# neggles/neurosis

Hardware: AMD Instinct MI355X
Metric: train images/sec (node) SDXL 1024^2 (higher is better)
Workload: dtype bf16

## Files before the change

### include/neurosis_hip.h

```cpp
#ifndef NEUROSIS_HIP_H
#define NEUROSIS_HIP_H

#ifdef __cplusplus
extern "C" {
#endif

const char* nk_last_error(void);
int nk_abi_version(void);

int nk_linear_fwd(const void* x, const void* w, const float* bias, const void* residual, void* y,
                  int M, int N, int K, long ldx, long ldw, long ldr, long ldy, float alpha, void* stream);
int nk_linear_dgrad(const void* dy, const void* w, const void* dx_add, void* dx, int M, int N, int K,
                    long lddy, long ldw, long ldadd, long lddx, void* stream);
long nk_linear_fwd_geglu_ok(int M, int I, int K);
int nk_linear_fwd_geglu(const void* x, const void* w, const float* bias, void* u, void* h, int M, int I, int K, long ldx, long ldw, long ldu,
                        long ldh, void* stream);
int nk_linear_dgrad_geglu(const void* dy, const void* w, const void* u, void* du, int M, int N, int I, long lddy, long ldw, long ldu,
                          long lddu, void* stream);
int nk_linear_fwd_geglu_s(const void* x, const void* w, const float* bias, void* s, void* h, int M, int I, int K, long ldx, long ldw, long lds,
                          long ldh, void* stream);
int nk_linear_dgrad_geglu_s(const void* dy, const void* w, const void* s, void* du, int M, int N, int I, long lddy, long ldw, long lds,
                            long lddu, void* stream);
int nk_linear_wgrad(const void* dy, const void* x, float* dw, int M, int N, int K, long lddy, long ldx,
                    long lddw, int accumulate, void* stream);
int nk_linear_wgrad_bias(const void* dy, const void* x, float* dw, float* dbias, int M, int N, int K, long lddy, long ldx, long lddw,
                         int accumulate, void* stream);

int nk_gemm_sk_status(void);

int nk_health_status(void);
int nk_health_clear(void);
int nk_health_export(int* dst, void* stream);
int nk_health_import(const int* src, void* stream);
int nk_debug_raise_health(void* stream);
int nk_debug_stamp(unsigned long long* dst, void* stream);
int nk_debug_launch_log(int mode);
long nk_debug_launch_names(char* buf, long cap);

int nk_colsum_batched(const void* dy, float* out, float* ws, long M, int N, long ld, int nbatch, int accumulate, void* stream);

int nk_linear_fwd_batched(const void* const* x, const void* const* w, void* const* y, int count, int M, int N, int K,
                          long ldx, long ldw, long ldy, void* stream);

int nk_linear_wgrad_batched(const void* const* dy, const void* const* x, float* const* dw, float* const* dbias, int count, int M, int N,
                            int K, long lddy, long ldx, long lddw, int accumulate, void* stream);

typedef struct NkConvDesc {
  int N, H, W, Cin;
  int Cout, KH, KW;
  int stride;
  int pad_t, pad_l;
  int Ho, Wo;
  int upsample;
} NkConvDesc;
int nk_conv2d_fwd(const NkConvDesc* d, const void* x, const void* w, const float* bias, const void* rowvec,
                  const void* residual, void* y, void* stream);
long nk_conv2d_stats_tiles(const NkConvDesc* d, int stats_groups);
int nk_conv2d_fwd_stats(const NkConvDesc* d, const void* x, const void* w, const float* bias, const void* rowvec, const void* residual,
                        void* y, float* stats_part, int stats_groups, void* stream);
int nk_conv3x3_few_channels_fwd(const void* x, const void* w, const float* bias, void* y, int N, int H, int W, int Cout, int cin_real,
                                void* stream);
int nk_conv_weight_flip(const void* w, void* wt, int Cout, int Cin, int taps, void* stream);
long nk_conv2d_dgrad_flipped_ok(const NkConvDesc* d);
int nk_conv2d_dgrad_flipped(const NkConvDesc* d, const void* dy, const void* wt, void* dx, void* stream);
int nk_conv2d_dgrad(const NkConvDesc* d, const void* dy, const void* w, void* dx, void* stream);
int nk_conv2d_wgrad(const NkConvDesc* d, const void* dy, const void* x, float* dw, int accumulate, void* stream);
int nk_conv2d_wgrad_bias(const NkConvDesc* d, const void* dy, const void* x, float* dw, float* dbias, int accumulate, void* stream);

typedef struct NkAttnDesc {
  int B, H, Lq, Lk, D;
  long sq, sk, sv, so;
  long bq, bk, bv, bo;
  long sdq, sdk, sdv, sdo;
  long bdq, bdk, bdv, bdo;
  float scale;
  int causal;
} NkAttnDesc;
int nk_attention_fwd(const NkAttnDesc* d, const void* q, const void* k, const void* v, void* o, float* lse,
                     void* stream);
long nk_attention_bwd_ws_floats(const NkAttnDesc* d);
int nk_attention_bwd(const NkAttnDesc* d, const void* q, const void* k, const void* v, const void* o,
                     const float* lse, const void* d_o, void* dq, void* dk, void* dv, float* delta_ws, void* stream);
int nk_attention_bwd_causal(const NkAttnDesc* d, const void* q, const void* k, const void* v, const void* o,
                            const float* lse, const void* d_o, void* dq, void* dk, void* dv, void* stream);
int nk_softmax_rows(void* s, long M, int L, void* stream);

long nk_groupnorm_ws_floats(int N, int HW, int C, int G);
int nk_groupnorm_fwd(const void* x, const float* gamma, const float* beta, void* y, float* mean, float* rstd,
                     float* ws, int N, int HW, int C, int G, float eps, int silu, void* stream);
int nk_groupnorm_sums(const void* x, float* sums, float* ws, int N, int HW, int C, int G, void* stream);
long nk_groupnorm_sums_ws_floats(int N, int nparts, int G);
int nk_groupnorm_sums_from_parts(const float* part, float* sums, float* ws, int N, int nparts, int G, void* stream);
int nk_groupnorm_apply(const void* x, const float* sums, const float* gamma, const float* beta, void* y, float* mean, float* rstd,
                       int N, int HW, int C, int G, float eps, int silu, void* stream);
int nk_groupnorm_bwd(const void* dy, const void* x, const float* gamma, const float* beta, const float* mean,
                     const float* rstd, const void* dx_add, void* dx, float* dgamma, float* dbeta, float* ws,
                     int N, int HW, int C, int G, int silu, int accumulate, void* stream);

int nk_layernorm_fwd(const void* x, const float* gamma, const float* beta, void* y, float* mean, float* rstd,
                     int M, int C, float eps, void* stream);
long nk_layernorm_ws_floats(int M, int C);
int nk_layernorm_bwd(const void* dy, const void* x, const float* gamma, const float* mean, const float* rstd,
                     const void* dx_add, void* dx, float* dgamma, float* dbeta, float* ws, int M, int C, int accumulate, void* stream);
#define NK_COLPART_MAX 32
typedef struct NkColpartBatch {
  const float* part[NK_COLPART_MAX];
  float* dgamma[NK_COLPART_MAX];
  float* dbeta[NK_COLPART_MAX];
  int nrows[NK_COLPART_MAX];
  int C[NK_COLPART_MAX];
  int accumulate[NK_COLPART_MAX];
  int n;
} NkColpartBatch;
long nk_layernorm_part_rows(int M);
int nk_layernorm_bwd_rows(const void* dy, const void* x, const float* gamma, const float* mean, const float* rstd,
                          const void* dx_add, void* dx, float* part, int M, int C, void* stream);
int nk_colpart_reduce_batch(const NkColpartBatch* b, void* stream);
int nk_layernorm_bwd_dx(const void* dy, const void* x, const float* gamma, const float* mean, const float* rstd,
                        const void* dx_add, void* dx, int M, int C, void* stream);
int nk_layernorm_bwd_params(const void* dy, const void* x, const float* mean, const float* rstd, float* dgamma,
                            float* dbeta, float* ws, int M, int C, int accumulate, void* stream);

int nk_geglu_fwd(const void* u, void* y, long M, int I, void* stream);
int nk_geglu_bwd(const void* dy, const void* u, void* du, long M, int I, void* stream);
int nk_geglu_fwd_s(const void* u, void* y, void* s, long M, int I, void* stream);
int nk_geglu_bwd_s(const void* dy, const void* s, void* du, long M, int I, void* stream);

int nk_silu_fwd(const void* x, void* y, long n, void* stream);
int nk_silu_bwd(const void* dy, const void* x, void* dx, long n, void* stream);

int nk_add(const void* a, const void* b, void* out, long n, void* stream);

int nk_cat_channels(const void* a, const void* b, void* out, long rows, int Ca, int Cb, void* stream);
int nk_split_channels(const void* src, void* a, void* b, long rows, int Ca, int Cb, void* stream);

int nk_upsample2x_bwd(const void* dup, void* dx, int N, int H, int W, int C, void* stream);

int nk_nchw_to_nhwc(const void* src, int src_is_f32, void* dst, int N, int C, int HW, int Cpad, float scale,
                    void* stream);
int nk_nhwc_to_nchw(const void* src, void* dst, int dst_is_f32, int N, int C, int HW, int Cpad, void* stream);
int nk_cast_f32_to_bf16(const float* src, void* dst, long n, void* stream);
int nk_cast_bf16_to_f32(const void* src, float* dst, long n, void* stream);

long nk_colsum_ws_floats(long M, int N);
int nk_colsum(const void* dy, float* out, float* ws, long M, int N, long ld, int accumulate, void* stream);

int nk_softmax_rows_bwd(const void* p, void* dp, long M, int L, float scale, void* stream);

int nk_leaky_relu_fwd(const void* x, void* y, long n, float slope, void* stream);
int nk_leaky_relu_bwd(const void* dy, const void* y, void* dx, long n, float slope, void* stream);
long nk_batchnorm_ws_floats(long M, int C);
int nk_batchnorm_fwd(const void* x, const float* gamma, const float* beta, void* y, float* mean, float* rstd, float* running_mean,
                     float* running_var, float* ws, long M, int C, float eps, float momentum, float slope, void* stream);
int nk_batchnorm_bwd(const void* dy, const void* x, const void* y, const float* gamma, const float* mean, const float* rstd, void* dx,
                     float* dgamma, float* dbeta, float* ws, long M, int C, float slope, int accumulate, void* stream);
int nk_batchnorm_eval(const void* x, const float* gamma, const float* beta, const float* running_mean, const float* running_var, void* y,
                      float* ws, long M, int C, float eps, float slope, void* stream);

int nk_maxpool2x2_fwd(const void* x, void* y, int N, int H, int W, int C, void* stream);
int nk_maxpool2x2_bwd(const void* dy, const void* x, void* dx, int N, int H, int W, int C, void* stream);
int nk_maxpool_fwd(const void* x, void* y, int N, int H, int W, int C, int k, int s, void* stream);
int nk_maxpool_bwd(const void* dy, const void* x, void* dx, int N, int H, int W, int C, int k, int s, void* stream);
long nk_lpips_layer_ws_floats(int N, int HW);
int nk_lpips_layer_fwd(const void* f0, const void* f1, const float* w, float* out, float* ws, int N, int HW, int C, float eps,
                       int accumulate, void* stream);
int nk_lpips_layer_bwd(const void* f0, const void* f1, const float* w, const float* upstream, void* df1, int N, int HW, int C,
                       float eps, void* stream);

int nk_gelu_fwd(const void* x, void* y, long n, int mode, void* stream);
int nk_gelu_bwd(const void* dy, const void* x, void* dx, long n, int mode, void* stream);
#define NK_EMBEDDING_BWD_MAX_TOKENS 8192
int nk_embedding_bwd(const long long* ids, const void* dx, long ldx, float* dtable, float* dpos, int B, int L, int V, int P, int C,
                     int accumulate, void* stream);
int nk_gather_rows_bwd(const void* dsel, long ldsel, const long long* idx, void* dx, int B, int L, int C, void* stream);
int nk_wgrad_few_rows(const void* x, long ldx, const void* dy, long lddy, float* dw, long lddw, int M, int K, int N, int accumulate, void* stream);

int nk_timestep_embedding(const float* t, void* out, int B, int dim, float max_period, void* stream);

int nk_edm_prepare(const float* x, const float* eps, const float* sigma, const float* c_in, float* zt, void* net_in,
                   int B, int C, int HW, int Cpad, void* stream);
int nk_edm_loss(const void* net_out, const float* zt, const float* target, const float* c_out, const float* c_skip,
                const float* w, float* loss, void* dnet, int B, int C, int HW, int Cpad, float upstream, void* stream);

int nk_sample_prepare(const float* x, const float* c_in, void* net_in, int B, int C, int HW, int Cpad, int rep, void* stream);
int nk_sample_denoise(const void* net_out, const float* x, const float* c_skip, const float* c_out, float scale,
                      float* denoised, int B, int C, int HW, int Cpad, int rep, void* stream);
int nk_sample_euler_step(const void* net_out, const float* x, const float* c_skip, const float* c_out, const float* sigma_hat,
                         const float* sigma_next, float scale, float* x_next, float* denoised, int B, int C, int HW, int Cpad,
                         int rep, void* stream);

int nk_adamw_flat(float* p, const float* g, float* m, float* v, void* shadow, long n, float lr, float beta1,
                  float beta2, float eps, float weight_decay, int step, float grad_scale, void* stream);

typedef struct NkAdafactorArgs {
  float* master; const float* grad; void* shadow; float* state; float* ws;
  const void* tensors; const void* items;
  float* u2_part; float* p2_part; float* mean_row; float* scale; float* lr_t;
  int item_lo, item_hi, tensor_lo, tensor_hi;
  float beta2t, eps1, eps2, clip_threshold, rel_step, weight_decay, grad_scale;
  int scale_parameter;
  unsigned* counters;
  int has_matrix;
  int reserved;
} NkAdafactorArgs;
long nk_adafactor_tensor_bytes(void);
int nk_adafactor_init(const NkAdafactorArgs* args, void* stream);
int nk_adafactor_chunk(const NkAdafactorArgs* args, void* stream);

typedef struct NkCameArgs {
  float* master; const float* grad; void* shadow; float* state; float* ws;
  const void* tensors; const void* items;
  float* u2_part;
  float* mean_row;
  float* denom;
  unsigned* counters;
  int item_lo, item_hi, tensor_lo, tensor_hi;
  float beta1, beta2, beta3;
  float one_minus_beta1, one_minus_beta2, one_minus_beta3;
  float eps1, eps2, clip_threshold, lr, decay, grad_scale;
  int has_matrix;
// ... 23 lines not shown
```

### neurosis_amd/csrc/conv_wgrad_halo.h

```cpp
#pragma once

#define WH_TH 4
#define WH_TW 32
#define WH_HS 48
#define WH_X_BYTES ((WH_TH + 2) * WH_HS * 128)
#define WH_DY_BYTES (WH_TH * WH_TW * 256)
#define WH_STAGE (WH_X_BYTES + WH_DY_BYTES)
#define WH_SMEM (2 * WH_STAGE)
#define WH_BCO 128
#define WH_BCI 64

typedef __attribute__((address_space(3))) char* wh_lds;
typedef __attribute__((address_space(3))) short4_t* wh_lds4;

__device__ __forceinline__ int wh_swz_x(int slot) { return (((slot >> 1) & 1) << 2) | ((slot >> 2) & 3); }
__device__ __forceinline__ int wh_swz_dy(int px) { return ((px & 3) << 2) | ((px >> 2) & 3); }

__device__ __forceinline__ bf16x8_t wh_read(wh_lds lo, wh_lds hi) {
  const short4_t a = __builtin_amdgcn_ds_read_tr16_b64_v4i16((wh_lds4)lo);
  const short4_t b = __builtin_amdgcn_ds_read_tr16_b64_v4i16((wh_lds4)hi);
  short8_t r;
  r[0] = a[0]; r[1] = a[1]; r[2] = a[2]; r[3] = a[3];
  r[4] = b[0]; r[5] = b[1]; r[6] = b[2]; r[7] = b[3];
  return __builtin_bit_cast(bf16x8_t, r);
}

struct WhStager {
  int xd, xe, dd, de;
  int n, ty, tx;

  __device__ __forceinline__ void init(const NkGemmParams& p, int t, int txn, int tyn, int lane) {
    const int per_img = txn * tyn;
    n = t / per_img;
    const int rem = t - n * per_img;
    ty = rem / txn;
    tx = rem - ty * txn;
    const int l8 = lane >> 3, l16 = lane >> 4;
    xd = (lane & 7) ^ ((((l8 >> 1) & 1) << 2) | (l8 >> 2));
    xe = l8 * p.gb.C;
    dd = (lane & 15) ^ (l16 << 2);
    de = l16 * (int)p.lda;
  }
  __device__ __forceinline__ void issue(const NkGemmParams& p, char* stage, int txn, int tyn, int cb, int ib, int wave, int lane) {
    const NkGather& g = p.gb;
    const int h0 = ty * WH_TH, w0 = tx * WH_TW;
    const bf16_t* xo = p.B + (((long)n * g.H + h0 - 1) * g.W + (w0 - 1)) * g.C + ib * WH_BCI;
    const bf16_t* dyo = p.A + (((long)n * g.H + h0) * g.W + w0) * p.lda + cb * WH_BCO;
    const bf16_t* zp = (const bf16_t*)nk_zero_page;
    int l8 = lane >> 3, l16 = lane >> 4, xd_ = xd, xe_ = xe, dd_ = dd, de_ = de;
    asm volatile("" : "+v"(l8), "+v"(l16), "+v"(xd_), "+v"(xe_), "+v"(dd_), "+v"(de_));
#pragma unroll
    for (int i = 0; i < 8; ++i) {
      const int pc = wave + 8 * i;
      if (pc < 30) {
        const int hr = pc / 5, pg = pc - hr * 5;
        const bool row_ok = (unsigned)(h0 - 1 + hr) < (unsigned)g.H;
        const int slot = pg * 8 + l8;
        const bool v = row_ok && slot < WH_TW + 2 && (unsigned)(w0 - 1 + slot) < (unsigned)g.W;
        const int off = (hr * g.W + pg * 8) * g.C + xe_ + ((xd_ ^ ((pg & 1) << 1)) << 3);
        __builtin_amdgcn_global_load_lds((nk_gptr)(v ? xo + off : zp), (nk_lptr)(stage + (hr * WH_HS + pg * 8) * 128), 16, 0, 0);
      } else if (pc < 62) {
        const int q = pc - 30;
        const bool row_ok = h0 + (q >> 3) < g.H;
        const int chunk = dd_ ^ (q & 3);
        const bool v = row_ok && w0 + (q & 7) * 4 + l16 < g.W && cb * WH_BCO + chunk * 8 < p.M;
        const int off = ((q >> 3) * g.W + (q & 7) * 4) * (int)p.lda + de_ + (chunk << 3);
        __builtin_amdgcn_global_load_lds((nk_gptr)(v ? dyo + off : zp), (nk_lptr)(stage + WH_X_BYTES + q * 1024), 16, 0, 0);
      }
    }
    if (++tx == txn) { tx = 0; if (++ty == tyn) { ty = 0; ++n; } }
  }
};

template <int BIAS>
__global__ __launch_bounds__(512, 2) void nk_conv3x3_wgrad_halo_kernel(const NkGemmParams p) {
  extern __shared__ __attribute__((aligned(16))) char smem[];
  const int tid = threadIdx.x, lane = tid & 63;
  const int wave = __builtin_amdgcn_readfirstlane(tid >> 6);
  const int cs = wave & 3, is = wave >> 2;
  const NkGather& g = p.gb;
  const int Cin = g.C, Cout = p.M;
  const int nci = Cin / WH_BCI;
  const int nblk = ((Cout + WH_BCO - 1) / WH_BCO) * nci;
  const int blk = blockIdx.x % nblk, split = blockIdx.x / nblk;
  const int cb = blk / nci, ib = blk - cb * nci;
  const int txn = (g.W + WH_TW - 1) / WH_TW, tyn = (g.H + WH_TH - 1) / WH_TH;
  const int T = p.halo_nb * txn * tyn;
  const int t0 = split * p.ksplit_len, t1 = min(T, t0 + p.ksplit_len);

  float16_t acc[9];
#pragma unroll
  for (int t = 0; t < 9; ++t)
#pragma unroll
    for (int r = 0; r < 16; ++r) acc[t][r] = 0.f;
  float bsum = 0.f;

  const int h = lane >> 5, g1 = (lane >> 4) & 1, q4 = (lane & 15) >> 2, pp = lane & 3;
  unsigned xo[3][2], dyo[2];
#pragma unroll
  for (int j = 0; j < 2; ++j) {
#pragma unroll
    for (int a = 0; a < 3; ++a) {
      const int row = a + 4 * h + q4 + 8 * j;
      xo[a][j] = (unsigned)(row * 128 + (((4 * is + 2 * g1 + (pp >> 1)) ^ wh_swz_x(row)) << 4) + 8 * (pp & 1));
    }
    const int row = 4 * h + q4 + 8 * j;
    dyo[j] = (unsigned)(WH_X_BYTES + row * 256 + (((4 * cs + 2 * g1 + (pp >> 1)) ^ wh_swz_dy(row)) << 4) + 8 * (pp & 1));
  }
  const wh_lds sm = (wh_lds)smem;

  WhStager stg;
  stg.init(p, t0 < t1 ? t0 : 0, txn, tyn, lane);
  if (t0 < t1) stg.issue(p, smem, txn, tyn, cb, ib, wave, lane);
  for (int t = t0; t < t1; ++t) {
    const int st = (t - t0) & 1;
    asm volatile("s_waitcnt vmcnt(0)" ::: "memory");
    __syncthreads();
    if (t + 1 < t1) stg.issue(p, smem + (st ^ 1) * WH_STAGE, txn, tyn, cb, ib, wave, lane);
    const wh_lds base = sm + st * WH_STAGE;
#pragma unroll
    for (int kg = 0; kg < 8; ++kg) {
      const int r = kg >> 1, c = (kg & 1) * 16;
      const bf16x8_t af = wh_read(base + dyo[0] + kg * 4096, base + dyo[1] + kg * 4096);
      if constexpr (BIAS) {
        const short8_t raw = __builtin_bit_cast(short8_t, af);
#pragma unroll
        for (int e = 0; e < 8; ++e) bsum += bf2f((bf16_t)raw[e]);
      }
#pragma unroll
      for (int kh = 0; kh < 3; ++kh)
#pragma unroll
        for (int kw = 0; kw < 3; ++kw) {
          const int off = ((r + kh) * WH_HS + c) * 128;
          const bf16x8_t xf = wh_read(base + xo[kw][0] + off, base + xo[kw][1] + off);
          acc[kh * 3 + kw] = __builtin_amdgcn_mfma_f32_32x32x16_bf16(af, xf, acc[kh * 3 + kw], 0, 0, 0);
        }
    }
  }

  float* dw = (float*)p.C;
  const int ci = ib * WH_BCI + is * 32 + (lane & 31);
  const int co_base = cb * WH_BCO + cs * 32 + 4 * h;
  const bool atomic = gridDim.x > (unsigned)nblk || p.accumulate == 1;
#pragma unroll
  for (int t = 0; t < 9; ++t)
#pragma unroll
    for (int r = 0; r < 16; ++r) {
      const int co = co_base + (r & 3) + 8 * (r >> 2);
      if (co < Cout) {
        float* dst = dw + (long)co * p.ldc + t * Cin + ci;
        const float v = acc[t][r] * p.alpha;
        if (atomic) unsafeAtomicAdd(dst, v);
        else *dst = v;
      }
    }
  if constexpr (BIAS) {
    if (ib == 0 && is == 0) {
      bsum += __shfl_xor(bsum, 32);
      const int co = cb * WH_BCO + cs * 32 + (lane & 31);
      if (lane < 32 && co < Cout) {
        if (atomic) unsafeAtomicAdd(p.dbias + co, bsum * p.alpha);
        else p.dbias[co] = bsum * p.alpha;
      }
    }
  }
}

static bool wgrad_halo_shape_ok(const NkGemmParams& p) {
  const NkGather& g = p.gb;
  if (!p.halo_nb || g.KW != 3 || p.N != 9 * g.C || g.rs != 1 || g.ks != 1 || g.div != 1 || g.off_h != -1 || g.off_w != -1) return false;
  if (g.Ho != g.H || g.Wo != g.W || (g.C % WH_BCI) || (p.M & 7) || p.nbatch || p.ldc != p.N || p.lda != p.M) return false;
  if (p.K != (long)p.halo_nb * g.H * g.W) return false;
  const long cover = (long)((g.W + WH_TW - 1) / WH_TW) * WH_TW * ((g.H + WH_TH - 1) / WH_TH) * WH_TH;
  return cover * 100 <= (long)g.H * g.W * 125;
}
static int wgrad_halo_splits(const NkGemmParams& p, int& per) {
  const NkGather& g = p.gb;
  const long T = (long)p.halo_nb * ((g.W + WH_TW - 1) / WH_TW) * ((g.H + WH_TH - 1) / WH_TH);
  const long nblk = (long)((p.M + WH_BCO - 1) / WH_BCO) * (g.C / WH_BCI);
  const double dw_bytes = (double)p.M * p.N * 4.0;
  double best = 1e30;
  int best_s = 1;
  for (int s = 1; s <= 64 && s <= T; ++s) {
    const long tiles = (T + s - 1) / s;
    const long rounds = (nblk * s + 255) / 256;
    const double cost = (double)rounds * (tiles * 3.0e-6 + 4.0e-6) + (s > 1 ? s * dw_bytes / 1.3e12 : dw_bytes / 4.0e12);
    if (cost < best * 0.97) { best = cost; best_s = s; }
  }
  per = (int)((T + best_s - 1) / best_s);
  return (int)((T + per - 1) / per);
}
static bool use_wgrad_halo(const NkGemmParams& p, int amode, int bmode, int out_f32) {
  if (amode != OP_MC || bmode != OP_MCG || !out_f32) return false;
  int mode = 1;
  if (const char* e = getenv("NK_CONV_WGRAD_HALO")) mode = atoi(e);
  if (!mode || !wgrad_halo_shape_ok(p)) return false;
  if (mode == 2) return true;
  if (p.M < 64) return false;
  const long nblk = (long)((p.M + WH_BCO - 1) / WH_BCO) * (p.gb.C / WH_BCI);
  return p.K >= 16384 || nblk >= 180;
}
static int launch_wgrad_halo(NkGemmParams& p, hipStream_t stream) {
  int per = 0;
  const int S = wgrad_halo_splits(p, per);
  const long nblk = (long)((p.M + WH_BCO - 1) / WH_BCO) * (p.gb.C / WH_BCI);
  if (S > 1 && p.accumulate == 0) {
    const size_t n = (size_t)p.M * p.N;
    const unsigned blocks = (unsigned)((n / 4 + 255) / 256 > 2048 ? 2048 : (n / 4 + 255) / 256);
    hipLaunchKernelGGL(nk_zero_f32_kernel, dim3(blocks ? blocks : 1), dim3(256), 0, stream, (float*)p.C, n);
    if (p.dbias) hipLaunchKernelGGL(nk_zero_f32_kernel, dim3(1), dim3(256), 0, stream, p.dbias, (size_t)p.M);
    if (hipGetLastError() != hipSuccess) return NK_ERR_LAUNCH;
  }
  p.accumulate = p.accumulate == 1 ? 1 : 0;
  p.ksplit_len = per;
  auto kern = p.dbias ? nk_conv3x3_wgrad_halo_kernel<1> : nk_conv3x3_wgrad_halo_kernel<0>;
  nk_optin_lds((const void*)kern, WH_SMEM);
  hipLaunchKernelGGL(kern, dim3((unsigned)(nblk * S)), dim3(512), WH_SMEM, stream, p);
  return nk_check_launch(p.dbias ? "nk_conv3x3_wgrad_halo_kernel<bias=1>" : "nk_conv3x3_wgrad_halo_kernel<bias=0>");
}
```

### neurosis_amd/csrc/gemm.hip

```cpp
#include "nk_common.h"
#include "nk_gemm.h"
#include <stdlib.h>

#define BM 128
#define BN 128
#define BK 64
#define NTHREADS 256
#define GROUP_M 8
#define KC_IMAGE_BYTES (128 * 128)
#define MC_ROW_BYTES (128 * 2 + 16)
#define MC_IMAGE_BYTES (BK * MC_ROW_BYTES)
#define OPND_BYTES MC_IMAGE_BYTES
#define STAGE_BYTES (2 * OPND_BYTES)
#define CS_LD 132
#define SMEM_BYTES (2 * STAGE_BYTES)

static_assert(SMEM_BYTES >= BM * CS_LD * 4, "epilogue staging must fit");

enum { OP_KC = 0, OP_KCG = 1, OP_MC = 2, OP_MCT = 3, OP_MCG = 4 };

__device__ __forceinline__ bool is_kc(int mode) { return mode == OP_KC || mode == OP_KCG; }

__device__ __forceinline__ long gather_offset(const NkGather& g, int n, int bh, int bw, int kh, int kw,
                                              int c, bool& valid) {
  int hn = bh + kh * g.ks;
  int wn = bw + kw * g.ks;
  bool ok = (hn >= 0) & (wn >= 0);
  ok &= (((hn | wn) & g.need_even) == 0);
  const int sh = g.div >> 1;
  int h = hn >> sh, w = wn >> sh;
  ok &= (h < g.H) & (w < g.W);
  valid = valid && ok;
  return (((long)n * g.H + h) * g.W + w) * g.C + c;
}

template <int OUT_F32, int TBM = BM, int TNT = NTHREADS, int NJ = 4>
__device__ __forceinline__ void nk_gemm_epilogue(const NkGemmParams& p, char* smem, float4_t (&acc)[4][NJ], int m0, int n0, int tid,
                                                 int lane, int wm, int wn) {
  float* cs = (float*)smem;
  constexpr int GIT = OUT_F32 ? 1 : (TBM * BN / 8) / TNT;
  uint4_t gu_a[GIT], gu_g[GIT];
  const bool geglu = !OUT_F32 && p.geglu_u != nullptr && (p.N & 7) == 0;
  if constexpr (!OUT_F32) {
    if (geglu) {
#pragma unroll
      for (int it = 0; it < GIT; ++it) {
        const int idx = tid + it * TNT;
        const int m = m0 + (idx >> 4), n = n0 + (idx & 15) * 8;
        const bool ok = m < p.M && n < p.N;
        const bf16_t* up = p.geglu_u + (long)(ok ? m : 0) * p.ld_u + (ok ? n : 0);
        gu_a[it] = *(const uint4_t*)up;
        gu_g[it] = *(const uint4_t*)(up + p.N);
      }
    }
  }
#pragma unroll
  for (int i = 0; i < 4; ++i)
#pragma unroll
    for (int j = 0; j < NJ; ++j)
#pragma unroll
      for (int r = 0; r < 4; ++r) {
        int row = wm * 64 + i * 16 + (lane >> 4) * 4 + r;
        int col = wn * (NJ * 16) + j * 16 + (lane & 15);
        cs[row * CS_LD + col] = acc[i][j][r];
      }
  __syncthreads();

  if constexpr (!OUT_F32) {
    if (geglu) {
      bf16_t* C = (bf16_t*)p.C;
#pragma unroll
      for (int it = 0; it < GIT; ++it) {
        const int idx = tid + it * TNT;
        const int row = idx >> 4, cc = idx & 15;
        const int m = m0 + row, n = n0 + cc * 8;
        if (m >= p.M || n >= p.N) continue;
        const float4_t c0 = *(const float4_t*)(cs + row * CS_LD + cc * 8);
        const float4_t c1 = *(const float4_t*)(cs + row * CS_LD + cc * 8 + 4);
        float v[8] = {c0[0], c0[1], c0[2], c0[3], c1[0], c1[1], c1[2], c1[3]};
        if (p.alpha != 1.0f) {
#pragma unroll
          for (int e = 0; e < 8; ++e) v[e] *= p.alpha;
        }
        float a[8], g[8], da[8], dg[8];
        unpack8(gu_a[it], a);
        unpack8(gu_g[it], g);
        if (p.geglu_save) {
#pragma unroll
          for (int e = 0; e < 8; ++e) { da[e] = v[e] * a[e]; dg[e] = v[e] * g[e]; }
        } else {
#pragma unroll
          for (int e = 0; e < 8; ++e) {
            float cdf, pdf;
            normal_cdf_pdf(g[e], cdf, pdf);
            da[e] = v[e] * (g[e] * cdf);
            dg[e] = v[e] * a[e] * (cdf + g[e] * pdf);
          }
        }
        *(uint4_t*)(C + (long)m * p.ldc + n) = pack8(da);
        *(uint4_t*)(C + (long)m * p.ldc + p.N + n) = pack8(dg);
      }
      return;
    }
  }

  if constexpr (OUT_F32) {
    float* C = (float*)(p.nbatch ? p.Cb[blockIdx.z] : p.C);
    if (!p.accumulate && (p.N & 3) == 0 && (p.ldc & 3) == 0) {
      for (int it = 0; it < (TBM * BN / 4) / TNT; ++it) {
        int idx = tid + it * TNT;
        int row = idx >> 5, c4 = (idx & 31) * 4;
        int m = m0 + row, n = n0 + c4;
        if (m < p.M && n < p.N) {
          float4_t v = *(const float4_t*)(cs + row * CS_LD + c4);
          v *= p.alpha;
          *(float4_t*)(C + (long)m * p.ldc + n) = v;
        }
      }
      return;
    }
    for (int it = 0; it < (TBM * BN) / TNT; ++it) {
      int idx = tid + it * TNT;
      int row = idx >> 7, col = idx & 127;
      int m = m0 + row, n = n0 + col;
      if (m < p.M && n < p.N) {
        float v = cs[row * CS_LD + col] * p.alpha;
        float* dst = C + (long)m * p.ldc + n;
        if (p.accumulate) unsafeAtomicAdd(dst, v);
        else *dst = v;
      }
    }
  } else {
    bf16_t* C = (bf16_t*)(p.nbatch ? p.Cb[blockIdx.z] : p.C);
    const bool vec = (p.N & 7) == 0;
#pragma unroll 2
    for (int it = 0; it < (TBM * BN / 8) / TNT; ++it) {
      int idx = tid + it * TNT;
      int row = idx >> 4, cc = idx & 15;
      int m = m0 + row, n = n0 + cc * 8;
      if (m >= p.M || n >= p.N) continue;
      float v[8];
      const float4_t c0 = *(const float4_t*)(cs + row * CS_LD + cc * 8);
      const float4_t c1 = *(const float4_t*)(cs + row * CS_LD + cc * 8 + 4);
      v[0] = c0[0]; v[1] = c0[1]; v[2] = c0[2]; v[3] = c0[3];
      v[4] = c1[0]; v[5] = c1[1]; v[6] = c1[2]; v[7] = c1[3];
      if (p.alpha != 1.0f) {
#pragma unroll
        for (int e = 0; e < 8; ++e) v[e] *= p.alpha;
      }
      if (vec) {
        if (p.bias) {
          const float4_t b0 = *(const float4_t*)(p.bias + n);
          const float4_t b1 = *(const float4_t*)(p.bias + n + 4);
          v[0] += b0[0]; v[1] += b0[1]; v[2] += b0[2]; v[3] += b0[3];
          v[4] += b1[0]; v[5] += b1[1]; v[6] += b1[2]; v[7] += b1[3];
        }
        if (p.rowvec) {
          unsigned b = fdiv((unsigned)m, p.fRowsPerBatch);
          float t[8];
          unpack8(*(const uint4_t*)(p.rowvec + (long)b * p.ld_rowvec + n), t);
#pragma unroll
          for (int e = 0; e < 8; ++e) v[e] += t[e];
        }
        if (p.residual) {
          float t[8];
          unpack8(*(const uint4_t*)(p.residual + (long)m * p.ldr + n), t);
#pragma unroll
          for (int e = 0; e < 8; ++e) v[e] += t[e];
        }
        *(uint4_t*)(C + (long)m * p.ldc + n) = pack8(v);
      } else {
        for (int e = 0; e < 8 && n + e < p.N; ++e) {
          float x = v[e];
          if (p.bias) x += p.bias[n + e];
          if (p.rowvec) x += bf2f(p.rowvec[(long)fdiv((unsigned)m, p.fRowsPerBatch) * p.ld_rowvec + n + e]);
          if (p.residual) x += bf2f(p.residual[(long)m * p.ldr + n + e]);
          C[(long)m * p.ldc + n + e] = f2bf(x);
        }
      }
    }
  }
}

__device__ __attribute__((aligned(64))) unsigned int nk_zero_page[16];

typedef __attribute__((address_space(1))) const void* nk_gptr;
typedef __attribute__((address_space(3))) void* nk_lptr;

#define V2_OPND_BYTES 16384
#define V2_STAGE_BYTES (2 * V2_OPND_BYTES)
#define V2_SMEM_BYTES (BM * CS_LD * 4)

__device__ __forceinline__ int mc_swz(int k) { return ((k & 3) | (((k >> 3) & 1) << 2)) << 1; }

template <int MODE, int NP = 4>
struct OperandDMA {
  const bf16_t* P;
  long ld;
  int R, r0, wave, lane;
  int pn[NP], pbh[NP], pbw[NP];
  int tkh0, tkh1, tkw0, tkw1, tc0, tc1;
  bool rvalid[NP < 2 ? 2 : NP];

  __device__ __forceinline__ int kc_row(int i) const { return wave * (NP * 8) + i * 8 + (lane >> 3); }
  __device__ __forceinline__ int kc_chunk() const { return (lane & 7) ^ (lane >> 3); }
  __device__ __forceinline__ int mc_k(int i) const { return (wave * NP + i) * 4 + (lane >> 4); }
  __device__ __forceinline__ int mc_var(int i) const { return (((wave * NP + i) * 4) >> 3) & 1; }
  __device__ __forceinline__ bool mc_valid(int v) const { return v ? rvalid[1] : rvalid[0]; }
  __device__ __forceinline__ int sel(int a0, int a1, int v) const { return v ? a1 : a0; }
  __device__ __forceinline__ int mc_chunk(int v) const { return (lane & 15) ^ (((lane >> 4) | (v << 2)) << 1); }

  __device__ __forceinline__ void init(const bf16_t* p, long ld_, int R_, int r0_, int tid, const NkGather& g) {
    P = p; ld = ld_; R = R_; r0 = r0_; wave = tid >> 6; lane = tid & 63;
    if constexpr (MODE == OP_KC || MODE == OP_KCG) {
#pragma unroll
      for (int i = 0; i < NP; ++i) {
        int r = r0 + kc_row(i);
        rvalid[i] = r < R;
        if constexpr (MODE == OP_KCG) {
          unsigned p_ = rvalid[i] ? (unsigned)r : 0u;
          unsigned n = fdiv(p_, g.fHoWo);
          unsigned rem = p_ - n * g.fHoWo.d;
          unsigned ph = fdiv(rem, g.fWo);
          unsigned pw = rem - ph * g.fWo.d;
          pn[i] = (int)n;
          pbh[i] = (int)ph * g.rs + g.off_h;
          pbw[i] = (int)pw * g.rs + g.off_w;
          if (g.div == 1 && (g.C & 63) == 0) pn[i] = ((pn[i] * g.H + pbh[i]) * g.W + pbw[i]) * g.C + kc_chunk() * 8;
        }
      }
    } else {
#pragma unroll
      for (int v = 0; v < 2; ++v) {
        int r = r0 + mc_chunk(v) * 8;
        rvalid[v] = r < R;
        if constexpr (MODE == OP_MCG) {
          unsigned rr = rvalid[v] ? (unsigned)r : 0u;
          unsigned tap = fdiv(rr, g.fC);
          const int c_ = (int)(rr - tap * g.fC.d);
          unsigned kh = fdiv(tap, g.fKW);
          const int kw_ = (int)(tap - kh * g.fKW.d);
          if (v == 0) { tc0 = c_; tkh0 = (int)kh; tkw0 = kw_; }
          else { tc1 = c_; tkh1 = (int)kh; tkw1 = kw_; }
        }
      }
    }
  }

  __device__ __forceinline__ void issue(int k0, int kend, char* img, const NkGather& g, const NkTapW& tw) const {
    const bf16_t* src[NP];
    sources(k0, kend, src, g, tw);
#pragma unroll
    for (int i = 0; i < NP; ++i) fire(i, src[i], img);
  }
  __device__ __forceinline__ void fire(int i, const bf16_t* s, char* img) const {
    __builtin_amdgcn_global_load_lds((nk_gptr)s, (nk_lptr)(img + (wave * NP + i) * 1024), 16, 0, 0);
  }
  __device__ __forceinline__ void sources(int k0, int kend, const bf16_t* (&src)[NP], const NkGather& g, const NkTapW& tw) const {
    const bf16_t* zp = (const bf16_t*)nk_zero_page;
    if constexpr (MODE == OP_KC) {
      int k = k0 + kc_chunk() * 8;
      bool kv = k < kend;
#pragma unroll
      for (int i = 0; i < NP; ++i) src[i] = (kv && rvalid[i]) ? P + (long)(r0 + kc_row(i)) * ld + k : zp;
    } else if constexpr (MODE == OP_KCG) {
      int k = k0 + kc_chunk() * 8;
      bool kv = k < kend;
      unsigned tap, kh;
      int c, kw;
      if (((g.C | k0) & 63) == 0) {
        const unsigned k0u = (unsigned)k0;
        tap = fdiv(k0u, g.fC);
        const int c0 = (int)(k0u - tap * g.fC.d);
        c = c0 + kc_chunk() * 8;
        kh = fdiv(tap, g.fKW);
        kw = (int)(tap - kh * g.fKW.d);
        if (g.div == 1) {
          const int dh = (int)kh * g.ks, dw = kw * g.ks;
          const int tapoff = (dh * g.W + dw) * g.C + c0;
#pragma unroll
          for (int i = 0; i < NP; ++i) {
            const bool ok = kv && rvalid[i] && (unsigned)(pbh[i] + dh) < (unsigned)g.H && (unsigned)(pbw[i] + dw) < (unsigned)g.W;
// ... 34 lines not shown
    } else if constexpr (MODE == OP_MCT) {
      if (((tw.fCout.d | (unsigned)k0) & 63) == 0) {
        const unsigned k0u = (unsigned)k0;
        const unsigned tap = fdiv(k0u, tw.fCout);
        const unsigned co0 = k0u - tap * tw.fCout.d;
        const bf16_t* base = P + (long)co0 * tw.co_stride + (long)tap * tw.tap_stride + r0;
#pragma unroll
        for (int i = 0; i < NP; ++i) {
          const int v = mc_var(i);
          const bool ok = k0 + mc_k(i) < kend && mc_valid(v);
          src[i] = ok ? base + (long)mc_k(i) * tw.co_stride + mc_chunk(v) * 8 : zp;
        }
      } else {
#pragma unroll
        for (int i = 0; i < NP; ++i) {
          int k = k0 + mc_k(i);
          const int v = mc_var(i);
          bool ok = k < kend && mc_valid(v);
          unsigned kk = ok ? (unsigned)k : 0u;
          unsigned tap = fdiv(kk, tw.fCout);
          unsigned co = kk - tap * tw.fCout.d;
          src[i] = ok ? P + (long)co * tw.co_stride + (long)tap * tw.tap_stride + r0 + mc_chunk(v) * 8 : zp;
        }
      }
    } else {
#pragma unroll
      for (int i = 0; i < NP; ++i) {
        int k = k0 + mc_k(i);
        const int v = mc_var(i);
        bool ok = (k < kend) && mc_valid(v);
        unsigned p_ = ok ? (unsigned)k : 0u;
        unsigned n = fdiv(p_, g.fHoWo);
        unsigned rem = p_ - n * g.fHoWo.d;
        unsigned ph = fdiv(rem, g.fWo);
        unsigned pw = rem - ph * g.fWo.d;
        long off = gather_offset(g, (int)n, (int)ph * g.rs + g.off_h, (int)pw * g.rs + g.off_w, sel(tkh0, tkh1, v), sel(tkw0, tkw1, v), sel(tc0, tc1, v), ok);
        src[i] = ok ? P + off : zp;
      }
    }
  }

  int kcur;
  const bf16_t* rp[NP];
  int mh[NP], mw[NP], moff[NP];
  bool mplain;
  __device__ __forceinline__ void start(int k_begin, const NkGather& g) {
    start(k_begin);
    if constexpr (MODE == OP_MCG) {
      const int q = (int)fdiv(64u, g.fWo);
      mplain = g.div == 1 && q + 1 < g.Ho;
      if (mplain) {
#pragma unroll
        for (int i = 0; i < NP; ++i) {
          const int v = mc_var(i);
          const unsigned p_ = (unsigned)(k_begin + mc_k(i));
          const unsigned n = fdiv(p_, g.fHoWo);
          const unsigned rem = p_ - n * g.fHoWo.d;
          const unsigned ph = fdiv(rem, g.fWo);
          const unsigned pw = rem - ph * g.fWo.d;
          mh[i] = (int)ph * g.rs + g.off_h + sel(tkh0, tkh1, v) * g.ks;
          mw[i] = (int)pw * g.rs + g.off_w + sel(tkw0, tkw1, v) * g.ks;
          moff[i] = (((int)n * g.H + mh[i]) * g.W + mw[i]) * g.C + sel(tc0, tc1, v);
        }
      }
    }
  }
  __device__ __forceinline__ void start(int k_begin) {
    kcur = k_begin;
    if constexpr (MODE == OP_KC) {
#pragma unroll
      for (int i = 0; i < NP; ++i) rp[i] = P + (long)(r0 + kc_row(i)) * ld + (k_begin + kc_chunk() * 8);
    } else if constexpr (MODE == OP_MC) {
#pragma unroll
      for (int i = 0; i < NP; ++i) rp[i] = P + (long)(k_begin + mc_k(i)) * ld + r0 + mc_chunk(mc_var(i)) * 8;
    }
  }
  __device__ __forceinline__ void next_sources(int kend, const bf16_t* (&src)[NP], const NkGather& g, const NkTapW& tw) {
    if constexpr (MODE == OP_KC || MODE == OP_MC) {
      const bf16_t* zp = (const bf16_t*)nk_zero_page;
#pragma unroll
      for (int i = 0; i < NP; ++i) {
        bool ok;
        if constexpr (MODE == OP_KC) ok = (kcur + kc_chunk() * 8 < kend) && rvalid[i];
        else ok = (kcur + mc_k(i) < kend) && mc_valid(mc_var(i));
        src[i] = ok ? rp[i] : zp;
        rp[i] += MODE == OP_KC ? (long)BK : (long)BK * ld;
      }
    } else if constexpr (MODE == OP_MCG) {
      if (mplain) {
        const bf16_t* zp = (const bf16_t*)nk_zero_page;
        const int q = (int)fdiv(64u, g.fWo);
        const int rm = 64 - q * g.Wo;
        const int wspan = g.Wo * g.rs, hspan = g.Ho * g.rs;
        const int A = (q * g.rs * g.W + rm * g.rs) * g.C, Bc = (g.rs * g.W - wspan) * g.C, Ci = (g.H - hspan) * g.W * g.C;
#pragma unroll
        for (int i = 0; i < NP; ++i) {
          const int v = mc_var(i);
          const bool ok = (kcur + mc_k(i) < kend) && mc_valid(v) && (unsigned)mh[i] < (unsigned)g.H && (unsigned)mw[i] < (unsigned)g.W;
          src[i] = ok ? P + (long)moff[i] : zp;
          const int dw = sel(tkw0, tkw1, v) * g.ks + g.off_w, dh = sel(tkh0, tkh1, v) * g.ks + g.off_h;
          int w = mw[i] + rm * g.rs;
          const bool c1 = w - dw >= wspan;
          w -= c1 ? wspan : 0;
          int h = mh[i] + (q + (c1 ? 1 : 0)) * g.rs;
          const bool c2 = h - dh >= hspan;
          h -= c2 ? hspan : 0;
          mw[i] = w; mh[i] = h;
          moff[i] += A + (c1 ? Bc : 0) + (c2 ? Ci : 0);
        }
      } else {
        sources(kcur, kend, src, g, tw);
      }
    } else {
      sources(kcur, kend, src, g, tw);
    }
    kcur += BK;
  }
  __device__ __forceinline__ void issue_next(int kend, char* img, const NkGather& g, const NkTapW& tw) {
    const bf16_t* src[NP];
    next_sources(kend, src, g, tw);
#pragma unroll
    for (int i = 0; i < NP; ++i) fire(i, src[i], img);
  }

  static __device__ __forceinline__ bf16x8_t frag(const char* img, int sub, int ks, int lane) {
    if constexpr (MODE == OP_KC || MODE == OP_KCG) {
      int row = sub + (lane & 15);
      int chunk = ks * 4 + (lane >> 4);
      int byte = row * 128 + ((chunk ^ (row & 7)) << 4);
      return *(const bf16x8_t*)(img + byte);
    } else {
      int g = lane >> 4, i = lane & 15;
      int q = i >> 2, p = i & 3;
      int k = ks * 32 + 8 * g + q;
      int col = sub + 4 * p;
      int byte_lo = k * 256 + (((col >> 3) ^ mc_swz(k)) << 4) + (col & 7) * 2;
      int k2 = k + 4;
      int byte_hi = k2 * 256 + (((col >> 3) ^ mc_swz(k2)) << 4) + (col & 7) * 2;
      typedef __attribute__((address_space(3))) short4_t* lds_p;
      short4_t lo = __builtin_amdgcn_ds_read_tr16_b64_v4i16((lds_p)(img + byte_lo));
      short4_t hi = __builtin_amdgcn_ds_read_tr16_b64_v4i16((lds_p)(img + byte_hi));
      short8_t r;
      r[0] = lo[0]; r[1] = lo[1]; r[2] = lo[2]; r[3] = lo[3];
      r[4] = hi[0]; r[5] = hi[1]; r[6] = hi[2]; r[7] = hi[3];
      return __builtin_bit_cast(bf16x8_t, r);
    }
  }
};

__device__ __forceinline__ bf16x8_t nk_ones_frag() {
  const short8_t o = {0x3F80, 0x3F80, 0x3F80, 0x3F80, 0x3F80, 0x3F80, 0x3F80, 0x3F80};
  return __builtin_bit_cast(bf16x8_t, o);
}
__device__ __forceinline__ void nk_store_bias_rows(float* db, const float4_t& a, int row0, int M, float alpha, int mode, int lane) {
  if (lane & 15) return;
#pragma unroll
  for (int r = 0; r < 4; ++r) {
    const int m = row0 + (lane >> 4) * 4 + r;
    if (m < M) {
      const float v = a[r] * alpha;
      if (mode == 2) unsafeAtomicAdd(db + m, v);
      else db[m] = mode == 1 ? db[m] + v : v;
    }
  }
}

template <int AMODE, int BMODE, int OUT_F32, int NW>
__global__ __launch_bounds__(NW * 64, NW / 2) void nk_gemm_dma_kernel(const NkGemmParams p) {
  extern __shared__ __attribute__((aligned(16))) char smem[];
  constexpr int NJ = NW == 4 ? 4 : 2;
  constexpr int NP = 16 / NW;
  const int tid = threadIdx.x;
  const int lane = tid & 63;
  const int wave = tid >> 6;
  const int wm = NW == 4 ? (wave >> 1) : (wave >> 2), wn = NW == 4 ? (wave & 1) : (wave & 3);

  const int nwg = gridDim.x;
  const int bid = blockIdx.x;
  const int q8 = nwg >> 3, r8 = nwg & 7, xcd = bid & 7;
  const int wg = (xcd < r8 ? xcd * (q8 + 1) : r8 * (q8 + 1) + (xcd - r8) * q8) + (bid >> 3);
  const int ntn = (p.N + BN - 1) / BN;
  const int ntm = (p.M + BM - 1) / BM;
  const int GMv = p.group_m;
  const int per_group = GMv * ntn;
  const int group = wg / per_group;
  const int first_m = group * GMv;
  const int gm = min(GMv, ntm - first_m);
  const int in_group = wg - group * per_group;
  const int nt = in_group / gm;
  const int mt = first_m + (in_group - nt * gm);
  const int m0 = mt * BM, n0 = nt * BN;

  const int kbeg = blockIdx.y * p.ksplit_len;
  const int kend = min(p.K, kbeg + p.ksplit_len);
  const int nk = (kend - kbeg + BK - 1) / BK;

  OperandDMA<AMODE, NP> opa;
  OperandDMA<BMODE, NP> opb;
  opa.init(p.nbatch ? p.Ab[blockIdx.z] : p.A, p.lda, p.M, m0, tid, p.ga);
  opb.init(p.nbatch ? p.Bb[blockIdx.z] : p.B, p.ldb, p.N, n0, tid, p.gb);

  float4_t acc[4][NJ];
#pragma unroll
  for (int i = 0; i < 4; ++i)
#pragma unroll
    for (int j = 0; j < NJ; ++j) acc[i][j] = (float4_t){0.f, 0.f, 0.f, 0.f};
  constexpr bool CAN_BIAS = AMODE == OP_MC && OUT_F32 == 1;
  constexpr int NWN = NW == 4 ? 2 : 4, BPW = 4 / NWN;
  float* const dbias = CAN_BIAS ? (p.nbatch ? p.dbias_b[blockIdx.z] : p.dbias) : nullptr;
  const bool do_bias = CAN_BIAS && dbias != nullptr && nt == 0;
  const int wn_s = __builtin_amdgcn_readfirstlane(wn);
  float4_t accb[BPW];
#pragma unroll
  for (int u = 0; u < BPW; ++u) accb[u] = (float4_t){0.f, 0.f, 0.f, 0.f};

  constexpr bool CAN_ROT = AMODE == OP_KC || AMODE == OP_KCG || (AMODE == OP_MC && BMODE == OP_MC);
  const int s0 = CAN_ROT && p.k_rotate ? (xcd * nk) >> 3 : 0;
  opa.start(kbeg + s0 * BK, p.ga);
  opb.start(kbeg + s0 * BK, p.gb);
  if (nk > 0) {
    opa.issue_next(kend, smem, p.ga, p.tw);
    opb.issue_next(kend, smem + V2_OPND_BYTES, p.gb, p.tw);
  }
  for (int kt = 0; kt < nk; ++kt) {
    asm volatile("s_waitcnt vmcnt(0)" ::: "memory");
    __syncthreads();
    const char* cur = smem + (kt & 1) * V2_STAGE_BYTES;
    bf16x8_t af[2][4], bfr[2][NJ];
#pragma unroll
    for (int ks = 0; ks < 2; ++ks) {
#pragma unroll
      for (int i = 0; i < 4; ++i) af[ks][i] = OperandDMA<AMODE>::frag(cur, wm * 64 + i * 16, ks, lane);
#pragma unroll
      for (int j = 0; j < NJ; ++j) bfr[ks][j] = OperandDMA<BMODE>::frag(cur + V2_OPND_BYTES, wn * (NJ * 16) + j * 16, ks, lane);
    }
    __builtin_amdgcn_sched_barrier(0);
    if (kt + 1 < nk) {
      char* nxt = smem + ((kt + 1) & 1) * V2_STAGE_BYTES;
      if constexpr (CAN_ROT) {
        if (kt + 1 == nk - s0) {
          opa.start(kbeg, p.ga);
          opb.start(kbeg, p.gb);
        }
      }
      opa.issue_next(kend, nxt, p.ga, p.tw);
      opb.issue_next(kend, nxt + V2_OPND_BYTES, p.gb, p.tw);
    }
    __builtin_amdgcn_sched_barrier(0);
#pragma unroll
    for (int ks = 0; ks < 2; ++ks)
#pragma unroll
      for (int i = 0; i < 4; ++i)
#pragma unroll
        for (int j = 0; j < NJ; ++j)
          acc[i][j] = __builtin_amdgcn_mfma_f32_16x16x32_bf16(af[ks][i], bfr[ks][j], acc[i][j], 0, 0, 0);
    if constexpr (CAN_BIAS) {
      if (do_bias) {
        const bf16x8_t ones = nk_ones_frag();
#pragma unroll
        for (int u = 0; u < BPW; ++u) {
          switch (wn_s * BPW + u) {
            case 0: accb[u] = __builtin_amdgcn_mfma_f32_16x16x32_bf16(af[0][0], ones, accb[u], 0, 0, 0); accb[u] = __builtin_amdgcn_mfma_f32_16x16x32_bf16(af[1][0], ones, accb[u], 0, 0, 0); break;
            case 1: accb[u] = __builtin_amdgcn_mfma_f32_16x16x32_bf16(af[0][1], ones, accb[u], 0, 0, 0); accb[u] = __builtin_amdgcn_mfma_f32_16x16x32_bf16(af[1][1], ones, accb[u], 0, 0, 0); break;
            case 2: accb[u] = __builtin_amdgcn_mfma_f32_16x16x32_bf16(af[0][2], ones, accb[u], 0, 0, 0); accb[u] = __builtin_amdgcn_mfma_f32_16x16x32_bf16(af[1][2], ones, accb[u], 0, 0, 0); break;
            default: accb[u] = __builtin_amdgcn_mfma_f32_16x16x32_bf16(af[0][3], ones, accb[u], 0, 0, 0); accb[u] = __builtin_amdgcn_mfma_f32_16x16x32_bf16(af[1][3], ones, accb[u], 0, 0, 0); break;
          }
        }
      }
    }
  }
  if constexpr (CAN_BIAS) {
    if (do_bias) {
      const int mode = gridDim.y > 1 ? 2 : (p.accumulate ? 1 : 0);
#pragma unroll
      for (int u = 0; u < BPW; ++u) nk_store_bias_rows(dbias, accb[u], m0 + wm * 64 + (wn * BPW + u) * 16, p.M, p.alpha, mode, lane);
    }
  }
  __syncthreads();
  nk_gemm_epilogue<OUT_F32, BM, NW * 64, NJ>(p, smem, acc, m0, n0, tid, lane, wm, wn);
}

#define RING_NS 4
#define RING_SMEM_BYTES (RING_NS * V2_STAGE_BYTES)

template <int MODE>
__device__ __forceinline__ bf16x8_t ring_frag(const char* img, int sub, int ks, int lane) {
  if constexpr (MODE == OP_KC || MODE == OP_KCG) {
    return OperandDMA<MODE>::frag(img, sub, ks, lane);
  } else {
    int g = lane >> 4, i = lane & 15;
    int q = i >> 2, p = i & 3;
    int k = ks * 32 + 8 * g + q;
    int col = sub + 4 * p;
    int byte_lo = k * 256 + (((col >> 3) ^ mc_swz(k)) << 4) + (col & 7) * 2;
    int k2 = k + 4;
    int byte_hi = k2 * 256 + (((col >> 3) ^ mc_swz(k2)) << 4) + (col & 7) * 2;
    typedef __attribute__((address_space(3))) const char* lds_c;
    const unsigned a_lo = (unsigned)(size_t)(lds_c)(img + byte_lo), a_hi = (unsigned)(size_t)(lds_c)(img + byte_hi);
    short4_t lo, hi;
    asm volatile("ds_read_b64_tr_b16 %0, %1" : "=v"(lo) : "v"(a_lo));
    asm volatile("ds_read_b64_tr_b16 %0, %1" : "=v"(hi) : "v"(a_hi));
    short8_t r;
    r[0] = lo[0]; r[1] = lo[1]; r[2] = lo[2]; r[3] = lo[3];
    r[4] = hi[0]; r[5] = hi[1]; r[6] = hi[2]; r[7] = hi[3];
    return __builtin_bit_cast(bf16x8_t, r);
  }
}

template <int AMODE, int BMODE, int OUT_F32>
__global__ __launch_bounds__(512, 2) void nk_gemm_ring_kernel(const NkGemmParams p) {
  extern __shared__ __attribute__((aligned(16))) char smem[];
  constexpr int NJ = 2, NP = 2;
  const int tid = threadIdx.x;
  const int lane = tid & 63;
  const int wave = tid >> 6;
  const int wm = wave >> 2, wn = wave & 3;

  const int nwg = gridDim.x;
  const int bid = blockIdx.x;
  const int q8 = nwg >> 3, r8 = nwg & 7, xcd = bid & 7;
  const int wg = (xcd < r8 ? xcd * (q8 + 1) : r8 * (q8 + 1) + (xcd - r8) * q8) + (bid >> 3);
  const int ntn = (p.N + BN - 1) / BN;
  const int ntm = (p.M + BM - 1) / BM;
  const int GMv = p.group_m;
  const int per_group = GMv * ntn;
  const int group = wg / per_group;
  const int first_m = group * GMv;
  const int gm = min(GMv, ntm - first_m);
  const int in_group = wg - group * per_group;
  const int nt = in_group / gm;
  const int mt = first_m + (in_group - nt * gm);
  const int m0 = mt * BM, n0 = nt * BN;

  const int kbeg = blockIdx.y * p.ksplit_len;
  const int kend = min(p.K, kbeg + p.ksplit_len);
  const int nk = (kend - kbeg + BK - 1) / BK;

  OperandDMA<AMODE, NP> opa;
  OperandDMA<BMODE, NP> opb;
  opa.init(p.A, p.lda, p.M, m0, tid, p.ga);
  opb.init(p.B, p.ldb, p.N, n0, tid, p.gb);

  float4_t acc[4][NJ];
#pragma unroll
  for (int i = 0; i < 4; ++i)
#pragma unroll
    for (int j = 0; j < NJ; ++j) acc[i][j] = (float4_t){0.f, 0.f, 0.f, 0.f};

  constexpr bool CAN_BIAS = AMODE == OP_MC && OUT_F32 == 1;
  const bool do_bias = CAN_BIAS && p.dbias != nullptr && nt == 0;
  float4_t accb = (float4_t){0.f, 0.f, 0.f, 0.f};

  opa.start(kbeg, p.ga);
  opb.start(kbeg, p.gb);
#pragma unroll
  for (int t = 0; t < RING_NS - 1; ++t)
    if (t < nk) {
      opa.issue_next(kend, smem + t * V2_STAGE_BYTES, p.ga, p.tw);
      opb.issue_next(kend, smem + t * V2_STAGE_BYTES + V2_OPND_BYTES, p.gb, p.tw);
    }
  int cur_stage = 0;
  for (int kt = 0; kt < nk; ++kt) {
    const int later = min(nk - 1 - kt, RING_NS - 2);
    if (later >= 2) asm volatile("s_waitcnt vmcnt(8)" ::: "memory");
    else if (later == 1) asm volatile("s_waitcnt vmcnt(4)" ::: "memory");
    else asm volatile("s_waitcnt vmcnt(0)" ::: "memory");
    __builtin_amdgcn_s_barrier();
    const char* cur = smem + cur_stage * V2_STAGE_BYTES;
    bf16x8_t af[2][4], bfr[2][NJ];
#pragma unroll
    for (int ks = 0; ks < 2; ++ks) {
#pragma unroll
      for (int i = 0; i < 4; ++i) af[ks][i] = ring_frag<AMODE>(cur, wm * 64 + i * 16, ks, lane);
#pragma unroll
      for (int j = 0; j < NJ; ++j) bfr[ks][j] = ring_frag<BMODE>(cur + V2_OPND_BYTES, wn * (NJ * 16) + j * 16, ks, lane);
    }
    __builtin_amdgcn_sched_barrier(0);
    if (kt + RING_NS - 1 < nk) {
      int ns = cur_stage + RING_NS - 1; if (ns >= RING_NS) ns -= RING_NS;
      opa.issue_next(kend, smem + ns * V2_STAGE_BYTES, p.ga, p.tw);
      opb.issue_next(kend, smem + ns * V2_STAGE_BYTES + V2_OPND_BYTES, p.gb, p.tw);
    }
    asm volatile("s_waitcnt lgkmcnt(0)"
                 : "+v"(af[0][0]), "+v"(af[0][1]), "+v"(af[0][2]), "+v"(af[0][3]), "+v"(af[1][0]), "+v"(af[1][1]), "+v"(af[1][2]),
                   "+v"(af[1][3]), "+v"(bfr[0][0]), "+v"(bfr[0][1]), "+v"(bfr[1][0]), "+v"(bfr[1][1]));
    __builtin_amdgcn_sched_barrier(0);
#pragma unroll
    for (int ks = 0; ks < 2; ++ks)
#pragma unroll
      for (int i = 0; i < 4; ++i)
#pragma unroll
        for (int j = 0; j < NJ; ++j)
          acc[i][j] = __builtin_amdgcn_mfma_f32_16x16x32_bf16(af[ks][i], bfr[ks][j], acc[i][j], 0, 0, 0);
    if constexpr (CAN_BIAS) {
      if (do_bias) {
        const bf16x8_t ones = nk_ones_frag();
        switch (__builtin_amdgcn_readfirstlane(wn)) {
          case 0: accb = __builtin_amdgcn_mfma_f32_16x16x32_bf16(af[0][0], ones, accb, 0, 0, 0); accb = __builtin_amdgcn_mfma_f32_16x16x32_bf16(af[1][0], ones, accb, 0, 0, 0); break;
          case 1: accb = __builtin_amdgcn_mfma_f32_16x16x32_bf16(af[0][1], ones, accb, 0, 0, 0); accb = __builtin_amdgcn_mfma_f32_16x16x32_bf16(af[1][1], ones, accb, 0, 0, 0); break;
          case 2: accb = __builtin_amdgcn_mfma_f32_16x16x32_bf16(af[0][2], ones, accb, 0, 0, 0); accb = __builtin_amdgcn_mfma_f32_16x16x32_bf16(af[1][2], ones, accb, 0, 0, 0); break;
          default: accb = __builtin_amdgcn_mfma_f32_16x16x32_bf16(af[0][3], ones, accb, 0, 0, 0); accb = __builtin_amdgcn_mfma_f32_16x16x32_bf16(af[1][3], ones, accb, 0, 0, 0); break;
        }
      }
    }
    if (++cur_stage == RING_NS) cur_stage = 0;
  }
  if constexpr (CAN_BIAS) {
    if (do_bias) nk_store_bias_rows(p.dbias, accb, m0 + wm * 64 + wn * 16, p.M, p.alpha, gridDim.y > 1 ? 2 : (p.accumulate ? 1 : 0), lane);
  }
  __syncthreads();
  nk_gemm_epilogue<OUT_F32, BM, 512, NJ>(p, smem, acc, m0, n0, tid, lane, wm, wn);
}

#define R64_NS 8
#define R64_OPND 8192
#define R64_STAGE (2 * R64_OPND)
#define R64_SMEM (R64_NS * R64_STAGE)
#define R64_CS_LD 68
__global__ __launch_bounds__(512, 2) void nk_gemm_ring64_kernel(const NkGemmParams p) {
  extern __shared__ __attribute__((aligned(16))) char smem[];
  const int tid = threadIdx.x, lane = tid & 63, wave = tid >> 6;
  const int wm = wave >> 2, wn = wave & 3;
  const int nwg = gridDim.x, bid = blockIdx.x;
  const int q8 = nwg >> 3, r8 = nwg & 7, xcd = bid & 7;
  const int wg = (xcd < r8 ? xcd * (q8 + 1) : r8 * (q8 + 1) + (xcd - r8) * q8) + (bid >> 3);
  const int ntm = (p.M + 63) >> 6;
  const int nt = wg / ntm, mt = wg - nt * ntm;
  const int m0 = mt * 64, n0 = nt * 64;
  const int kend = p.K, nk = (p.K + BK - 1) / BK;

  OperandDMA<OP_KC, 1> opa, opb;
  opa.init(p.A, p.lda, p.M, m0, tid, p.ga);
  opb.init(p.B, p.ldb, p.N, n0, tid, p.gb);
  float4_t acc[2] = {(float4_t){0.f, 0.f, 0.f, 0.f}, (float4_t){0.f, 0.f, 0.f, 0.f}};
  opa.start(0);
  opb.start(0);
#pragma unroll
  for (int t = 0; t < R64_NS - 1; ++t)
    if (t < nk) {
      opa.issue_next(kend, smem + t * R64_STAGE, p.ga, p.tw);
      opb.issue_next(kend, smem + t * R64_STAGE + R64_OPND, p.gb, p.tw);
    }
  int cur_stage = 0;
  for (int kt = 0; kt < nk; ++kt) {
    switch (min(nk - 1 - kt, R64_NS - 2)) {
      case 6: asm volatile("s_waitcnt vmcnt(12)" ::: "memory"); break;
      case 5: asm volatile("s_waitcnt vmcnt(10)" ::: "memory"); break;
      case 4: asm volatile("s_waitcnt vmcnt(8)" ::: "memory"); break;
      case 3: asm volatile("s_waitcnt vmcnt(6)" ::: "memory"); break;
      case 2: asm volatile("s_waitcnt vmcnt(4)" ::: "memory"); break;
      case 1: asm volatile("s_waitcnt vmcnt(2)" ::: "memory"); break;
      default: asm volatile("s_waitcnt vmcnt(0)" ::: "memory"); break;
    }
    __builtin_amdgcn_s_barrier();
    const char* cur = smem + cur_stage * R64_STAGE;
    bf16x8_t af[2][2], bfr[2];
#pragma unroll
    for (int ks = 0; ks < 2; ++ks) {
#pragma unroll
      for (int i = 0; i < 2; ++i) af[ks][i] = ring_frag<OP_KC>(cur, wm * 32 + i * 16, ks, lane);
      bfr[ks] = ring_frag<OP_KC>(cur + R64_OPND, wn * 16, ks, lane);
    }
    __builtin_amdgcn_sched_barrier(0);
    if (kt + R64_NS - 1 < nk) {
      int ns = cur_stage + R64_NS - 1; if (ns >= R64_NS) ns -= R64_NS;
      opa.issue_next(kend, smem + ns * R64_STAGE, p.ga, p.tw);
      opb.issue_next(kend, smem + ns * R64_STAGE + R64_OPND, p.gb, p.tw);
    }
    asm volatile("s_waitcnt lgkmcnt(0)" : "+v"(af[0][0]), "+v"(af[0][1]), "+v"(af[1][0]), "+v"(af[1][1]), "+v"(bfr[0]), "+v"(bfr[1]));
    __builtin_amdgcn_sched_barrier(0);
#pragma unroll
    for (int ks = 0; ks < 2; ++ks)
#pragma unroll
      for (int i = 0; i < 2; ++i) acc[i] = __builtin_amdgcn_mfma_f32_16x16x32_bf16(af[ks][i], bfr[ks], acc[i], 0, 0, 0);
    if (++cur_stage == R64_NS) cur_stage = 0;
  }
  __syncthreads();
  float* cs = (float*)smem;
#pragma unroll
  for (int i = 0; i < 2; ++i)
#pragma unroll
    for (int r = 0; r < 4; ++r) cs[(wm * 32 + i * 16 + (lane >> 4) * 4 + r) * R64_CS_LD + wn * 16 + (lane & 15)] = acc[i][r];
  __syncthreads();
  const int row = tid >> 3, cc = tid & 7;
  const int m = m0 + row, n = n0 + cc * 8;
  if (m >= p.M || n >= p.N) return;
  bf16_t* C = (bf16_t*)p.C;
  const float4_t c0 = *(const float4_t*)(cs + row * R64_CS_LD + cc * 8), c1 = *(const float4_t*)(cs + row * R64_CS_LD + cc * 8 + 4);
  float v[8] = {c0[0] * p.alpha, c0[1] * p.alpha, c0[2] * p.alpha, c0[3] * p.alpha, c1[0] * p.alpha, c1[1] * p.alpha, c1[2] * p.alpha, c1[3] * p.alpha};
  if ((p.N & 7) == 0) {
    if (p.bias) {
      const float4_t b0 = *(const float4_t*)(p.bias + n), b1 = *(const float4_t*)(p.bias + n + 4);
      v[0] += b0[0]; v[1] += b0[1]; v[2] += b0[2]; v[3] += b0[3];
      v[4] += b1[0]; v[5] += b1[1]; v[6] += b1[2]; v[7] += b1[3];
    }
    if (p.rowvec) {
      float t[8];
      unpack8(*(const uint4_t*)(p.rowvec + (long)fdiv((unsigned)m, p.fRowsPerBatch) * p.ld_rowvec + n), t);
#pragma unroll
      for (int e = 0; e < 8; ++e) v[e] += t[e];
    }
    if (p.residual) {
      float t[8];
      unpack8(*(const uint4_t*)(p.residual + (long)m * p.ldr + n), t);
#pragma unroll
      for (int e = 0; e < 8; ++e) v[e] += t[e];
    }
    *(uint4_t*)(C + (long)m * p.ldc + n) = pack8(v);
  } else {
    for (int e = 0; e < 8 && n + e < p.N; ++e) {
      float x = v[e];
      if (p.bias) x += p.bias[n + e];
      if (p.rowvec) x += bf2f(p.rowvec[(long)fdiv((unsigned)m, p.fRowsPerBatch) * p.ld_rowvec + n + e]);
      if (p.residual) x += bf2f(p.residual[(long)m * p.ldr + n + e]);
      C[(long)m * p.ldc + n + e] = f2bf(x);
    }
  }
}
static bool use_ring64(const NkGemmParams& p, int amode, int bmode, int out_f32) {
  if (amode != OP_KC || bmode != OP_KC || out_f32 || p.nbatch || p.geglu_u || p.geglu_h || p.stats_part) return false;
  if (const char* e = getenv("NK_GEMM_R64")) if (e[0] == '0') return false;
  if (p.M > 512 || p.K < 4 * BK) return false;
  const long t64 = (long)((p.M + 63) / 64) * ((p.N + 63) / 64);
  return t64 <= 256;
}
static int launch_ring64(const NkGemmParams& p, hipStream_t stream) {
  nk_optin_lds((const void*)nk_gemm_ring64_kernel, R64_SMEM);
  const unsigned tiles = (unsigned)(((p.M + 63) >> 6) * ((p.N + 63) >> 6));
  hipLaunchKernelGGL(nk_gemm_ring64_kernel, dim3(tiles), dim3(512), R64_SMEM, stream, p);
  return nk_check_launch("nk_gemm_ring64_kernel");
}

#define SK_NT 512
#define SK_SMEM_BYTES (2 * V2_STAGE_BYTES)
#define SK_MAX_GRID 512
#define SK_TILE_FLOATS (BM * BN)

__device__ __forceinline__ void sk_decode(const NkGemmParams& p, int t, int ntm, int ntn, int& m0, int& n0, int& z) {
  const int per = ntm * ntn;
  z = p.nbatch ? t / per : 0;
  const int wg = t - z * per;
  const int per_group = GROUP_M * ntn;
  const int group = wg / per_group;
  const int first_m = group * GROUP_M;
  const int gm = min(GROUP_M, ntm - first_m);
  const int in_group = wg - group * per_group;
  const int nt = in_group / gm;
  m0 = (first_m + (in_group - nt * gm)) * BM;
  n0 = nt * BN;
}

template <int MI>
__device__ __forceinline__ void residual_prefetch_64x32(const NkGemmParams& p, uint4_t (&r)[MI], int mbase, int nbase, int lane) {
  const int g = lane >> 4;
  const int n = nbase + (g & 1) * 16 + (g >> 1) * 8;
  const int mrow = mbase + (lane & 15);
#pragma unroll
  for (int i = 0; i < MI; ++i) {
    const int m = mrow + i * 16;
    r[i] = (n < p.N && m < p.M) ? *(const uint4_t*)(p.residual + (long)m * p.ldr + n) : (uint4_t){0u, 0u, 0u, 0u};
  }
// ... 391 lines not shown
    X2_NEXT(op, s_, g, cnt, ke);                            \
    op.fire(0, s_[0], img); op.fire(1, s_[1], img);         \
  } while (0)
  float4_t acc[8][4];
#pragma unroll
  for (int i = 0; i < 8; ++i)
#pragma unroll
    for (int j = 0; j < 4; ++j) acc[i][j] = (float4_t){0.f, 0.f, 0.f, 0.f};

  bf16x8_t ar[8], bc0[4], bc1[4];
  typedef __attribute__((address_space(3))) const char* lds_c;
  const unsigned lds0 = (unsigned)(size_t)(lds_c)smem;
  const unsigned x0 = (unsigned)(((lane >> 4) ^ (lane & 7)) << 4);
  const unsigned arow = lds0 + (unsigned)(wm * 128 + (lane & 15)) * 128u;
  const unsigned brow = lds0 + 32768u + (unsigned)(wn * 64 + (lane & 15)) * 128u;
  const unsigned a_k0 = arow + x0, a_k1 = arow + (x0 ^ 64u), b_k0 = brow + x0, b_k1 = brow + (x0 ^ 64u);
#define X2_RD1(f, addr, OFF) asm volatile("ds_read_b128 %0, %1 offset:%2" : "=v"(f) : "v"(addr), "n"((OFF)))
#define X2_RDA(half)                                                                                             \
  X2_RD1(ar[0], ca0, (half) * 8192); X2_RD1(ar[1], ca0, (half) * 8192 + 2048); X2_RD1(ar[2], ca0, (half) * 8192 + 4096);    \
  X2_RD1(ar[3], ca0, (half) * 8192 + 6144); X2_RD1(ar[4], ca1, (half) * 8192); X2_RD1(ar[5], ca1, (half) * 8192 + 2048);    \
  X2_RD1(ar[6], ca1, (half) * 8192 + 4096); X2_RD1(ar[7], ca1, (half) * 8192 + 6144)
#define X2_RDB(f, half)                                                                                          \
  X2_RD1(f[0], cb0, (half) * 4096); X2_RD1(f[1], cb0, (half) * 4096 + 2048); X2_RD1(f[2], cb1, (half) * 4096);              \
  X2_RD1(f[3], cb1, (half) * 4096 + 2048)
#define X2_BAR() __builtin_amdgcn_sched_barrier(0); __builtin_amdgcn_s_barrier(); __builtin_amdgcn_sched_barrier(0)
#define X2_MM(rb, cb, bf, PREP)                                                                                  \
  asm volatile("s_waitcnt lgkmcnt(0)" ::: "memory");                                                             \
  __builtin_amdgcn_sched_barrier(0);                                                                             \
  __builtin_amdgcn_s_setprio(1);                                                                                 \
  PREP;               \
  _Pragma("unroll") for (int ks = 0; ks < 2; ++ks)                                                               \
    _Pragma("unroll") for (int i = 0; i < 4; ++i)                                                                \
      _Pragma("unroll") for (int j = 0; j < 2; ++j)                                                              \
        acc[(rb) + i][(cb) + j] = __builtin_amdgcn_mfma_f32_16x16x32_bf16(bf[ks * 2 + j], ar[ks * 4 + i], acc[(rb) + i][(cb) + j], 0, 0, 0); \
  __builtin_amdgcn_s_setprio(0)

  const bf16_t* sa0[2];
  const bf16_t* sa1[2];
  const bf16_t* sb0[2];
  const bf16_t* sb1[2];
  if (nk > 0) {
    X2_ISSUE(a0, smem, p.ga, na0, ka0);
    X2_ISSUE(a1, smem + 16384, p.ga, na1, ka1);
    X2_ISSUE(b0, smem + 32768, p.gb, nb0, kb0);
    X2_ISSUE(b1, smem + 49152, p.gb, nb1, kb1);
    X2_ISSUE(b0, smem + XL_STAGE_BYTES + 32768, p.gb, nb0, kb0);
    X2_ISSUE(b1, smem + XL_STAGE_BYTES + 49152, p.gb, nb1, kb1);
    asm volatile("s_waitcnt vmcnt(4)" ::: "memory");
  }
  X2_NEXT(a1, sa1, p.ga, na1, ka1);
  X2_BAR();
  if (wm == 1) { X2_BAR(); }
  for (int t = 0; t < nk; ++t) {
    const unsigned so = (unsigned)(t & 1) * XL_STAGE_BYTES;
    char* cur = smem + so;
    char* oth = smem + (so ^ XL_STAGE_BYTES);
    const unsigned ca0 = a_k0 + so, ca1 = a_k1 + so, cb0 = b_k0 + so, cb1 = b_k1 + so;
    __builtin_amdgcn_sched_barrier(0);
    X2_RDB(bc0, 0);
    X2_RDA(0);
    a1.fire(0, sa1[0], oth + 16384);
    a1.fire(1, sa1[1], oth + 16384);
    X2_BAR();
    X2_MM(0, 0, bc0, X2_NEXT(a0, sa0, p.ga, na0, ka0));
    X2_BAR();
    X2_RDB(bc1, 1);
    a0.fire(0, sa0[0], oth);
    a0.fire(1, sa0[1], oth);
    X2_BAR();
    X2_MM(0, 2, bc1, (void)0);
    X2_BAR();
    X2_RDA(1);
    X2_BAR();
    X2_MM(4, 2, bc1, X2_NEXT(b0, sb0, p.gb, nb0, kb0); X2_NEXT(b1, sb1, p.gb, nb1, kb1));
    X2_BAR();
    b0.fire(0, sb0[0], cur + 32768);
    b0.fire(1, sb0[1], cur + 32768);
    b1.fire(0, sb1[0], cur + 49152);
    b1.fire(1, sb1[1], cur + 49152);
    asm volatile("s_waitcnt vmcnt(4)" ::: "memory");
    X2_BAR();
    X2_MM(4, 0, bc0, X2_NEXT(a1, sa1, p.ga, na1, ka1));
    X2_BAR();
  }
  if (wm == 0) { X2_BAR(); }
  asm volatile("s_waitcnt vmcnt(0)" ::: "memory");
#undef X2_NEXT
#undef X2_ISSUE
#undef X2_RD1
#undef X2_RDA
#undef X2_RDB
#undef X2_BAR
#undef X2_MM
  if constexpr (GEGLU) {
    const int I = p.N >> 1;
    const int abase = (n0 >> 1) + wn * 32;
    const int cl = (lane >> 4) * 4;
    float4_t ba[2], bg[2];
#pragma unroll
    for (int q = 0; q < 2; ++q) {
      ba[q] = p.bias ? *(const float4_t*)(p.bias + abase + q * 16 + cl) : (float4_t){0.f, 0.f, 0.f, 0.f};
      bg[q] = p.bias ? *(const float4_t*)(p.bias + I + abase + q * 16 + cl) : (float4_t){0.f, 0.f, 0.f, 0.f};
    }
    NkGemmParams ph = p;
    ph.N = I; ph.ldc = p.ld_h; ph.bias = nullptr;
    NkGemmParams ps = p;
    ps.bias = nullptr;
#pragma unroll
    for (int ib = 0; ib < 2; ++ib) {
      float4_t pa[4][2], pg[4][2], phh[4][2];
#pragma unroll
      for (int i = 0; i < 4; ++i)
#pragma unroll
        for (int q = 0; q < 2; ++q) {
          pa[i][q] = acc[ib * 4 + i][2 * q];
          pg[i][q] = acc[ib * 4 + i][2 * q + 1];
#pragma unroll
          for (int r = 0; r < 4; ++r) {
            const float av = bf2f(f2bf(pa[i][q][r] + ba[q][r])), gv = bf2f(f2bf(pg[i][q][r] + bg[q][r]));
            float cdf, pdf;
            normal_cdf_pdf(gv, cdf, pdf);
            const float ge = gv * cdf;
            phh[i][q][r] = av * ge;
            if (p.geglu_save) {
              pa[i][q][r] = ge;
              pg[i][q][r] = av * (cdf + gv * pdf);
            }
          }
        }
      const int mb = m0 + wm * 128 + ib * 64;
      if (p.geglu_save) {
        reg_epilogue_64x32<0>(ps, p.C, pa, mb, abase, lane);
        reg_epilogue_64x32<0>(ps, p.C, pg, mb, I + abase, lane);
      } else {
        reg_epilogue_64x32<0>(p, p.C, pa, mb, abase, lane);
        reg_epilogue_64x32<0>(p, p.C, pg, mb, I + abase, lane);
      }
      reg_epilogue_64x32<0>(ph, p.geglu_h, phh, mb, abase, lane);
    }
    return;
  }
#pragma unroll
  for (int ib = 0; ib < 2; ++ib)
#pragma unroll
    for (int half = 0; half < 2; ++half) {
      float4_t pair[4][2];
#pragma unroll
      for (int i = 0; i < 4; ++i) { pair[i][0] = acc[ib * 4 + i][2 * half]; pair[i][1] = acc[ib * 4 + i][2 * half + 1]; }
      reg_epilogue_64x32<0>(p, p.C, pair, m0 + wm * 128 + ib * 64, n0 + wn * 64 + half * 32, lane);
    }
}

static bool use_xl(const NkGemmParams& p, int amode, int bmode, int out_f32, int splitk);
__global__ void nk_zero_f32_kernel(float* __restrict__ dst, size_t n);
#include "gemm_g2.h"
#include "gemm_w160.h"
#include "conv_halo.h"
#include "conv_wgrad_halo.h"

static bool use_xl(const NkGemmParams& p, int amode, int bmode, int out_f32, int splitk) {
  static int on = -1;
  if (on < 0) { const char* e = getenv("NK_GEMM_XL"); on = (e && e[0] == '0') ? 0 : 1; }
  if (!on || p.nbatch || out_f32 || splitk != 1 || bmode != OP_KC || !(amode == OP_KC || amode == OP_KCG)) return false;
  const long ntn = (p.N + XL_BN - 1) / XL_BN;
  const long tiles = (long)((p.M + XL_BM - 1) / XL_BM) * ntn;
  const long rounds = (tiles + 255) / 256;
  return tiles >= 224 && tiles * 10 >= rounds * 256 * 8 && ntn * XL_BN * 100 <= (long)p.N * 112 && p.K >= 4 * BK;
}
template <int AMODE, int WM, int WN>
static int launch_xl_as(const NkGemmParams& p, hipStream_t stream) {
  auto kern = nk_gemm_xl_kernel<AMODE, WM, WN>;
  nk_optin_lds((const void*)kern, XL_SMEM_BYTES);
  dim3 grid(((p.M + XL_BM - 1) / XL_BM) * ((p.N + XL_BN - 1) / XL_BN), 1, 1);
  hipLaunchKernelGGL(kern, grid, dim3((XL_BM / WM) * (XL_BN / WN) * 64), XL_SMEM_BYTES, stream, p);
  return nk_check_launch("nk_gemm_xl_kernel");
}
template <int AMODE>
static int launch_xl(const NkGemmParams& p_in, hipStream_t stream) {
  if (AMODE == OP_KC) {
    auto kern = nk_gemm_xl2g_kernel<OP_KC, 0>;
    auto kerng = nk_gemm_xl2g_kernel<OP_KC, 1>;
    nk_optin_lds((const void*)kern, XL_SMEM_BYTES);
    nk_optin_lds((const void*)kerng, XL_SMEM_BYTES);
    NkGemmParams p = p_in;
    p.k_rotate = k_rotate_on(p.K) ? 1 : 0;
    dim3 grid(((p.M + XL_BM - 1) / XL_BM) * ((p.N + XL_BN - 1) / XL_BN), 1, 1);
    if (p.geglu_h) hipLaunchKernelGGL(kerng, grid, dim3(512), XL_SMEM_BYTES, stream, p);
    else hipLaunchKernelGGL(kern, grid, dim3(512), XL_SMEM_BYTES, stream, p);
    return nk_check_launch(p.geglu_h ? "nk_gemm_xl2g_kernel<geglu=1>" : "nk_gemm_xl2g_kernel<geglu=0>");
  }
  return launch_xl_as<AMODE, 64, 64>(p_in, stream);
}

template <int AMODE, int BMODE, int OUT_F32>
static int launch(const NkGemmParams& p_in, int splitk, hipStream_t stream) {
  NkGemmParams p2 = p_in;
  const NkGemmParams& p = p2;
  auto kern8 = nk_gemm_dma_kernel<AMODE, BMODE, OUT_F32, 8>;
  auto kernr = nk_gemm_ring_kernel<AMODE, BMODE, OUT_F32>;
  nk_optin_lds((const void*)kern8, V2_SMEM_BYTES);
  nk_optin_lds((const void*)kernr, RING_SMEM_BYTES);
  int ntm = (p.M + BM - 1) / BM, ntn = (p.N + BN - 1) / BN;
  dim3 grid(ntm * ntn, splitk, p.nbatch ? p.nbatch : 1);
  {
    int per_xcd = (ntm * ntn + 7) / 8, g = 1;
    while ((g + 1) * (g + 1) <= per_xcd) ++g;
    p2.group_m = g > GROUP_M ? GROUP_M : g;
  }
  p2.k_rotate = k_rotate_on(splitk > 1 ? p.ksplit_len : p.K) ? 1 : 0;
  if (!p.nbatch && (long)ntm * ntn * splitk <= 256) {
    hipLaunchKernelGGL(kernr, grid, dim3(512), RING_SMEM_BYTES, stream, p);
    return nk_check_launch("nk_gemm_ring_kernel");
  }
  hipLaunchKernelGGL(kern8, grid, dim3(512), V2_SMEM_BYTES, stream, p);
  return nk_check_launch("nk_gemm_dma_kernel");
}


#include <mutex>
#include <unordered_map>
struct SkWorkspace {
  unsigned* counter = nullptr;
  unsigned* flags = nullptr;
  float* ws = nullptr;
};
static std::mutex sk_mutex;
static std::unordered_map<void*, SkWorkspace> sk_spaces;

static bool use_sk(const NkGemmParams& p, int out_f32) {
  int mode = 4;
  if (const char* e = getenv("NK_GEMM_SK")) mode = atoi(e);
  if (mode == 0) return false;
  if (mode == 1) return true;
  if (mode == 2) return out_f32 != 0;
  if (mode == 4 && out_f32) return false;
  const long tiles = (long)((p.M + BM - 1) / BM) * ((p.N + BN - 1) / BN) * (p.nbatch ? p.nbatch : 1);
  const long nk = (p.K + BK - 1) / BK;
  const long rounds = (tiles + 511) / 512;
  const double fill = (double)tiles / (double)(rounds * 512);
  if (tiles >= 1024 && fill >= 0.8) return false;
  if (tiles >= 512 && fill >= 0.95) return false;
  return nk >= 24;
}

static int sk_prepare(NkGemmParams& p, int grid, hipStream_t stream) {
  std::lock_guard<std::mutex> lock(sk_mutex);
  SkWorkspace& w = sk_spaces[(void*)stream];
  if (!w.ws) {
    hipStreamCaptureStatus capturing = hipStreamCaptureStatusNone;
    if (hipStreamIsCapturing(stream, &capturing) == hipSuccess && capturing != hipStreamCaptureStatusNone) {
      nk_set_error(__FILE__, __LINE__, "stream-K workspace requested while the stream is capturing: run the launch once on this stream before capturing it");
      return NK_ERR_LAUNCH;
    }
    char* raw = nullptr;
    const size_t ws_bytes = (size_t)SK_MAX_GRID * SK_TILE_FLOATS * sizeof(float);
    if (hipMalloc((void**)&raw, ws_bytes + (SK_MAX_GRID + 64) * sizeof(unsigned)) != hipSuccess) {
      nk_set_error(__FILE__, __LINE__, "hipMalloc of the stream-K workspace failed");
      return NK_ERR_LAUNCH;
    }
    w.ws = (float*)raw;
    w.flags = (unsigned*)(raw + ws_bytes);
    w.counter = w.flags + SK_MAX_GRID;
    if (hipMemsetAsync(w.flags, 0, (SK_MAX_GRID + 64) * sizeof(unsigned), stream) != hipSuccess) return NK_ERR_LAUNCH;
  }
  p.sk_health = nk_health_word();
  if (!p.sk_health) { nk_set_error(__FILE__, __LINE__, "health word allocation failed"); return NK_ERR_LAUNCH; }
  p.sk_counter = w.counter;
  p.sk_flags = w.flags;
  p.sk_ws = w.ws;
  p.sk_base = 0;
  p.sk_epoch = 0;
  return NK_OK;
}

int nk_gemm_sk_reset(void) {
  std::lock_guard<std::mutex> lock(sk_mutex);
  for (auto& kv : sk_spaces)
    if (kv.second.flags && hipMemset(kv.second.flags, 0, (SK_MAX_GRID + 64) * sizeof(unsigned)) != hipSuccess) return NK_ERR_LAUNCH;
  return NK_OK;
}

extern "C" int nk_gemm_sk_status(void) {
  std::lock_guard<std::mutex> lock(sk_mutex);
  if (hipDeviceSynchronize() != hipSuccess) return -1;
  int bad = 0;
  for (auto& kv : sk_spaces) {
    unsigned v = 0;
    if (kv.second.flags && hipMemcpy(&v, kv.second.flags + SK_MAX_GRID + 1, sizeof(v), hipMemcpyDeviceToHost) == hipSuccess && v) bad = 1;
  }
  return bad;
}

template <int AMODE, int BMODE, int OUT_F32>
static int launch_sk(NkGemmParams& p, hipStream_t stream) {
  auto kern = nk_gemm_sk_kernel<AMODE, BMODE, OUT_F32>;
  nk_optin_lds((const void*)kern, SK_SMEM_BYTES);
  const long ntm = (p.M + BM - 1) / BM, ntn = (p.N + BN - 1) / BN, nk = (p.K + BK - 1) / BK;
  const long T = ntm * ntn * (p.nbatch ? p.nbatch : 1), W = T * nk;
  const int max_grid = SK_MAX_GRID & ~7, min_iters = 4;
  long grid = (W / min_iters) & ~7l;
  if (grid > max_grid) grid = max_grid;
  if (grid < 8) grid = 8;
  p.sk_chunked = T >= 64;
  { const char* d = getenv("NK_SK_DEBUG"); p.sk_debug = d ? atoi(d) & 2 : 0; }
  if (int e = sk_prepare(p, (int)grid, stream)) return e;
  hipLaunchKernelGGL(kern, dim3((unsigned)grid), dim3(SK_NT), SK_SMEM_BYTES, stream, p);
  return nk_check_launch("nk_gemm_sk_kernel");
}

__global__ __launch_bounds__(256) void nk_zero_f32_kernel(float* __restrict__ dst, size_t n) {
  const size_t n4 = n / 4, stride = (size_t)gridDim.x * 256;
  float4_t* d4 = (float4_t*)dst;
  for (size_t i = (size_t)blockIdx.x * 256 + threadIdx.x; i < n4; i += stride) d4[i] = (float4_t){0.f, 0.f, 0.f, 0.f};
  if (blockIdx.x == 0 && threadIdx.x < (n & 3)) dst[n4 * 4 + threadIdx.x] = 0.f;
}

static int pick_splitk(int M, int N, int K, int max_split) {
  int tiles = ((M + BM - 1) / BM) * ((N + BN - 1) / BN);
  int nk = (K + BK - 1) / BK;
  const int lo = 96, hi = 192;
  if (tiles >= lo && tiles * 2 <= 512 && nk >= 256 && max_split >= 2) return 2;
  if (tiles >= lo) return 1;
  int s = 1;
  while (s < max_split && tiles * s < hi && nk / (s * 2) >= 8) s *= 2;
  return s;
}

static void set_split(NkGemmParams& p, int splitk) {
  int nk = (p.K + BK - 1) / BK;
  int per = (nk + splitk - 1) / splitk;
  p.ksplit_len = per * BK;
}

static int zero_split_outputs(const NkGemmParams& p, hipStream_t stream) {
  for (int z = 0; z < (p.nbatch ? p.nbatch : 1); ++z) {
    const size_t n = (size_t)p.M * p.N;
    float* dst = (float*)(p.nbatch ? p.Cb[z] : p.C);
    const unsigned blocks = (unsigned)((n / 4 + 255) / 256 > 2048 ? 2048 : (n / 4 + 255) / 256);
    hipLaunchKernelGGL(nk_zero_f32_kernel, dim3(blocks ? blocks : 1), dim3(256), 0, stream, dst, n);
    float* db = p.nbatch ? p.dbias_b[z] : p.dbias;
    if (db) hipLaunchKernelGGL(nk_zero_f32_kernel, dim3(1), dim3(256), 0, stream, db, (size_t)p.M);
  }
  return hipGetLastError() != hipSuccess ? NK_ERR_LAUNCH : NK_OK;
}

int nk_gemm_dispatch(NkGemmParams& p, int amode, int bmode, int out_f32, int allow_splitk,
                     hipStream_t stream) {
  NK_CHECK_ARG(p.M > 0 && p.N > 0 && p.K > 0);
  if (!p.nbatch) NK_CHECK_ARG(((uintptr_t)p.A & 15) == 0 && ((uintptr_t)p.B & 15) == 0 && ((uintptr_t)p.C & 15) == 0);
  for (int z = 0; z < p.nbatch; ++z) NK_CHECK_ARG(((uintptr_t)p.Ab[z] & 15) == 0 && ((uintptr_t)p.Bb[z] & 15) == 0 && ((uintptr_t)p.Cb[z] & 15) == 0);
  if (amode == OP_KC) NK_CHECK_ARG((p.K & 7) == 0 && (p.lda & 7) == 0);
  if (bmode == OP_KC) NK_CHECK_ARG((p.K & 7) == 0 && (p.ldb & 7) == 0);
  if (amode == OP_KCG) NK_CHECK_ARG((p.ga.C & 7) == 0);
  if (amode == OP_MC) NK_CHECK_ARG((p.M & 7) == 0 && (p.lda & 7) == 0);
  if (bmode == OP_MC) NK_CHECK_ARG((p.N & 7) == 0 && (p.ldb & 7) == 0);
  if (bmode == OP_MCT) NK_CHECK_ARG((p.N & 7) == 0 && (p.tw.co_stride & 7) == 0 && (p.tw.tap_stride & 7) == 0);
  if (bmode == OP_MCG) NK_CHECK_ARG((p.gb.C & 7) == 0);
  if (p.residual) NK_CHECK_ARG(((uintptr_t)p.residual & 15) == 0 && ((p.ldr & 7) == 0 || (p.N & 7) != 0));
  if (!out_f32) NK_CHECK_ARG((p.ldc & 7) == 0 || (p.N & 7) != 0);
  if (p.fRowsPerBatch.d == 0) p.fRowsPerBatch = make_fastdiv(1);

  if (p.dbias || (p.nbatch && p.dbias_b[0])) NK_CHECK_ARG(amode == OP_MC && out_f32);
  if (p.geglu_h) {
    NK_CHECK_ARG(amode == OP_KC && bmode == OP_KC && !out_f32 && !p.nbatch && (p.N & 255) == 0 && (p.ld_h & 7) == 0 && !p.rowvec && !p.residual && p.alpha == 1.0f);
    NK_CHECK_ARG(((uintptr_t)p.geglu_h & 15) == 0 && (!p.bias || ((uintptr_t)p.bias & 15) == 0));
    if (!use_xl(p, amode, bmode, out_f32, 1)) {
      nk_set_error(__FILE__, __LINE__, "fused GEGLU forward on a shape the 256 x 256 kernel does not take (ask nk_linear_fwd_geglu_ok first)");
      return NK_ERR_ARG;
    }
    set_split(p, 1);
    return launch_xl<OP_KC>(p, stream);
  }
  if (p.geglu_u) {
    NK_CHECK_ARG(amode == OP_KC && bmode == OP_MC && !out_f32 && !p.nbatch && (p.N & 7) == 0 && (p.ld_u & 7) == 0 && !p.bias && !p.rowvec && !p.residual);
    set_split(p, 1);
    return launch<OP_KC, OP_MC, 0>(p, 1, stream);
  }
  if (use_halo(p, amode, bmode, out_f32)) return launch_halo(p, stream);
  if (use_wgrad_halo(p, amode, bmode, out_f32)) return launch_wgrad_halo(p, stream);
  if (p.stats_part) {
    nk_set_error(__FILE__, __LINE__, "statistics epilogue on a convolution the halo-tile kernel does not take (ask nk_conv2d_stats_tiles first)");
    return NK_ERR_ARG;
  }

  {
    const W160Plan wp = w160_plan(p, amode, bmode, out_f32, allow_splitk);
    if (wp.bn) {
      set_split(p, wp.splitk);
      if (wp.splitk > 1 && p.accumulate == 0) {
        NK_CHECK_ARG(p.ldc == p.N);
        if (int rc = zero_split_outputs(p, stream)) return rc;
        p.accumulate = 1;
      } else if (p.accumulate == 2) {
        p.accumulate = wp.splitk > 1 ? 1 : 0;
      }
      p.k_rotate = k_rotate_on(wp.splitk > 1 ? p.ksplit_len : p.K) ? 1 : 0;
      return wp.bn == 160 ? launch_w160_as<160>(p, wp.splitk, stream) : launch_w160_as<128>(p, wp.splitk, stream);
    }
  }
  if (use_ring64(p, amode, bmode, out_f32)) return launch_ring64(p, stream);
  if ((!p.nbatch || p.nbatch <= NK_MAX_BATCH) && use_g2(p, amode, bmode, out_f32, 1) && (g2_mode() == 2 || !use_xl(p, amode, bmode, out_f32, 1))) {
    if (p.accumulate == 2) p.accumulate = 0;
    if (amode == OP_KC && bmode == OP_KC) return out_f32 ? launch_g2<OP_KC, OP_KC, 1>(p, stream) : launch_g2<OP_KC, OP_KC, 0>(p, stream);
    if (amode == OP_KC && bmode == OP_MC) return out_f32 ? launch_g2<OP_KC, OP_MC, 1>(p, stream) : launch_g2<OP_KC, OP_MC, 0>(p, stream);
    if (amode == OP_KCG && bmode == OP_KC) return out_f32 ? launch_g2<OP_KCG, OP_KC, 1>(p, stream) : launch_g2<OP_KCG, OP_KC, 0>(p, stream);
    if (amode == OP_KCG && bmode == OP_MCT) return out_f32 ? launch_g2<OP_KCG, OP_MCT, 1>(p, stream) : launch_g2<OP_KCG, OP_MCT, 0>(p, stream);
    return out_f32 ? launch_g2<OP_MC, OP_MC, 1>(p, stream) : launch_g2<OP_MC, OP_MC, 0>(p, stream);
  }

  bool has_dbias = p.dbias != nullptr;
  for (int z = 0; z < p.nbatch && z < NK_MAX_BATCH; ++z) has_dbias = has_dbias || p.dbias_b[z] != nullptr;
  if (!has_dbias && use_sk(p, out_f32)) {
    const long ntm_ = (p.M + BM - 1) / BM, ntn_ = (p.N + BN - 1) / BN, nk_ = (p.K + BK - 1) / BK;
    if (ntm_ * ntn_ * (p.nbatch ? p.nbatch : 1) * nk_ < (1l << 22)) {
      if (p.accumulate == 2) p.accumulate = 0;
#define NK_SK_CASE(A_, B_)                                                        \
      if (amode == A_ && bmode == B_) return out_f32 ? launch_sk<A_, B_, 1>(p, stream) : launch_sk<A_, B_, 0>(p, stream);
      NK_SK_CASE(OP_KC, OP_KC)
      NK_SK_CASE(OP_KC, OP_MC)
      NK_SK_CASE(OP_MC, OP_MC)
      NK_SK_CASE(OP_KCG, OP_KC)
      NK_SK_CASE(OP_KCG, OP_MCT)
      NK_SK_CASE(OP_MC, OP_MCG)
#undef NK_SK_CASE
    }
  }
  int splitk = 1;
  if (out_f32 && allow_splitk) splitk = pick_splitk(p.M * (p.nbatch ? p.nbatch : 1), p.N, p.K, 32);
  if (p.nbatch) NK_CHECK_ARG(p.nbatch <= NK_MAX_BATCH);
  set_split(p, splitk);
  if (out_f32 && splitk > 1 && p.accumulate == 0) {
    NK_CHECK_ARG(p.ldc == p.N);
    if (int rc = zero_split_outputs(p, stream)) return rc;
    p.accumulate = 1;
  } else if (p.accumulate == 2) {
    p.accumulate = splitk > 1 ? 1 : 0;
  }

  if (use_xl(p, amode, bmode, out_f32, splitk))
    return amode == OP_KC ? launch_xl<OP_KC>(p, stream) : launch_xl<OP_KCG>(p, stream);

#define NK_CASE(A_, B_)                                                          \
  if (amode == A_ && bmode == B_) {                                              \
    return out_f32 ? launch<A_, B_, 1>(p, splitk, stream) : launch<A_, B_, 0>(p, splitk, stream); \
  }
  NK_CASE(OP_KC, OP_KC)
  NK_CASE(OP_KC, OP_MC)
  NK_CASE(OP_MC, OP_MC)
  NK_CASE(OP_KCG, OP_KC)
  NK_CASE(OP_KCG, OP_MCT)
  NK_CASE(OP_MC, OP_MCG)
#undef NK_CASE
  nk_set_error(__FILE__, __LINE__, "unsupported operand mode combination");
  return NK_ERR_ARG;
}

int nk_halo_bn(int N) { return halo_bn(N); }
int nk_halo_tiles_per_image(const NkGemmParams& p) {
  if (!use_halo(p, OP_KCG, OP_KC, 0)) return 0;
  return halo_tiles_per_image(p);
}


int nk_geglu_fwd_fusable(const NkGemmParams& p) {
  return (p.N & 255) == 0 && use_xl(p, OP_KC, OP_KC, 0, 1) ? 1 : 0;
}
```

### neurosis_amd/csrc/gemm_w160.h

```cpp
#pragma once

#define W160_BM 160
#define W160_NS 3
#ifdef NK_W160_STAMPS
__device__ unsigned long long nk_w160_stamp_buf[12 * 4096];
#define W160_STAMP(slot) do { if (tid == 0 && blockIdx.x < 4096 && blockIdx.z == 0 && blockIdx.y == 0) nk_w160_stamp_buf[blockIdx.x * 12 + (slot)] = __builtin_amdgcn_s_memtime(); } while (0)
#define W160_STAMP_RT(slot) do { if (tid == 0 && blockIdx.x < 4096 && blockIdx.z == 0 && blockIdx.y == 0) nk_w160_stamp_buf[blockIdx.x * 12 + (slot)] = __builtin_amdgcn_s_memrealtime(); } while (0)
#define W160_PSTAMP_DECL unsigned long long ps_fire = 0, ps_wait = 0, ps_bar = 0, ps_t = 0
#define W160_PSTAMP_T() (ps_t = __builtin_amdgcn_s_memtime())
#define W160_PSTAMP_ADD(acc) do { const unsigned long long n_ = __builtin_amdgcn_s_memtime(); acc += n_ - ps_t; ps_t = n_; } while (0)
#define W160_PSTAMP_OUT() do { if (tid == 256 && blockIdx.x < 4096 && blockIdx.z == 0 && blockIdx.y == 0) { nk_w160_stamp_buf[blockIdx.x * 12 + 6] = ps_fire; nk_w160_stamp_buf[blockIdx.x * 12 + 7] = ps_wait; nk_w160_stamp_buf[blockIdx.x * 12 + 8] = ps_bar; } } while (0)
#else
#define W160_STAMP(slot)
#define W160_STAMP_RT(slot)
#define W160_PSTAMP_DECL
#define W160_PSTAMP_T()
#define W160_PSTAMP_ADD(acc)
#define W160_PSTAMP_OUT()
#endif

template <int BN_>
struct W160Cfg {
  static constexpr int NJ = BN_ / 32;
  static constexpr int A_BYTES = W160_BM * 128;
// ... 115 lines not shown
      oa.advance(); ob.advance();
      if (kslab == nk) { kslab = 0; oa.rewind(nk); ob.rewind(nk); }
    };
    fire_next(smem);
    fire_next(smem + Cfg::STAGE);
    asm volatile("s_waitcnt vmcnt(%0)" ::"n"(PPS) : "memory");
    W160_BAR();
    unsigned sn = 2 * Cfg::STAGE;
    W160_PSTAMP_DECL;
    W160_PSTAMP_T();
    for (int t = 0; t < nk; ++t) {
      fire_next(smem + sn);
      W160_PSTAMP_ADD(ps_fire);
      asm volatile("s_waitcnt vmcnt(%0)" ::"n"(PPS) : "memory");
      W160_PSTAMP_ADD(ps_wait);
      W160_BAR();
      W160_PSTAMP_ADD(ps_bar);
      sn += Cfg::STAGE; if (sn == W160_NS * Cfg::STAGE) sn = 0;
    }
    W160_PSTAMP_OUT();
    asm volatile("s_waitcnt vmcnt(0)" ::: "memory");
    if (gridDim.y > 1) { W160_BAR(); }
    return;
  }

  __builtin_amdgcn_s_setprio(1);
  const int wr = wave >> 1, wc = wave & 1;
  typedef __attribute__((address_space(3))) const char* lds_c;
  const unsigned lds0 = (unsigned)(size_t)(lds_c)smem;
  FragG2<OP_MC, W160_BM, 5> fa;
  FragG2<OP_MC, BN_, NJ> fb;
  fa.init(lds0, wr * 80, lane);
  fb.init(lds0 + Cfg::A_BYTES, wc * (BN_ / 2), lane);

  float4_t acc[5][NJ];
#pragma unroll
  for (int i = 0; i < 5; ++i)
#pragma unroll
    for (int j = 0; j < NJ; ++j) acc[i][j] = (float4_t){0.f, 0.f, 0.f, 0.f};
  float* const dbias = p.nbatch ? p.dbias_b[blockIdx.z] : p.dbias;
  unsigned bmask = 0;
  if (dbias != nullptr && wc == 0) {
    for (int rb = nt; rb < 10; rb += ntn) bmask |= 1u << rb;
    bmask = (bmask >> (5 * wr)) & 31u;
  }
  bmask = __builtin_amdgcn_readfirstlane(bmask);
  float4_t accb[5];
#pragma unroll
  for (int i = 0; i < 5; ++i) accb[i] = (float4_t){0.f, 0.f, 0.f, 0.f};

  short4_t alo[2][5], ahi[2][5], blo[2][NJ], bhi[2][NJ];
  unsigned aa[5], ba[NJ];
  auto set_stage = [&](unsigned so) {
#pragma unroll
    for (int i = 0; i < 5; ++i) aa[i] = fa.a[i] + so;
#pragma unroll
    for (int j = 0; j < NJ; ++j) ba[j] = fb.a[j] + so;
  };
  auto frag = [](const short4_t& lo, const short4_t& hi) {
    short8_t r;
    r[0] = lo[0]; r[1] = lo[1]; r[2] = lo[2]; r[3] = lo[3]; r[4] = hi[0]; r[5] = hi[1]; r[6] = hi[2]; r[7] = hi[3];
    return __builtin_bit_cast(bf16x8_t, r);
  };

  auto substep = [&](auto cur_tag, auto nks_tag, auto barrier_tag, auto bias_tag, unsigned so_next) {
    constexpr int CUR = decltype(cur_tag)::value, NKS = decltype(nks_tag)::value;
    constexpr bool BARRIER = decltype(barrier_tag)::value, BIAS = decltype(bias_tag)::value;
    constexpr int NXT = 1 - CUR;
    if constexpr (NJ == 5)
      asm volatile("s_waitcnt lgkmcnt(8)" : "+v"(blo[CUR][0]), "+v"(bhi[CUR][0]), "+v"(blo[CUR][1]), "+v"(bhi[CUR][1]), "+v"(blo[CUR][2]), "+v"(bhi[CUR][2]),
                   "+v"(blo[CUR][3]), "+v"(bhi[CUR][3]), "+v"(blo[CUR][4]), "+v"(bhi[CUR][4]), "+v"(alo[CUR][0]), "+v"(ahi[CUR][0]));
    else
      asm volatile("s_waitcnt lgkmcnt(8)" : "+v"(blo[CUR][0]), "+v"(bhi[CUR][0]), "+v"(blo[CUR][1]), "+v"(bhi[CUR][1]), "+v"(blo[CUR][2]), "+v"(bhi[CUR][2]),
                   "+v"(blo[CUR][3]), "+v"(bhi[CUR][3]), "+v"(alo[CUR][0]), "+v"(ahi[CUR][0]));
    __builtin_amdgcn_sched_barrier(0);
    bf16x8_t bf[NJ];
#pragma unroll
    for (int j = 0; j < NJ; ++j) bf[j] = frag(blo[CUR][j], bhi[CUR][j]);
    {
      const bf16x8_t a0 = frag(alo[CUR][0], ahi[CUR][0]);
#pragma unroll
      for (int j = 0; j < NJ; ++j) acc[0][j] = __builtin_amdgcn_mfma_f32_16x16x32_bf16(bf[j], a0, acc[0][j], 0, 0, 0);
      if constexpr (BIAS) {
        if (bmask & 1u) accb[0] = __builtin_amdgcn_mfma_f32_16x16x32_bf16(nk_ones_frag(), a0, accb[0], 0, 0, 0);
      }
    }
    if constexpr (BARRIER) {
      W160_BAR();
      set_stage(so_next);
    }
    __builtin_amdgcn_sched_barrier(0);
    constexpr int GAPS = 4 * NJ;
    auto row = [&](auto i_tag) {
      constexpr int i = decltype(i_tag)::value;
      constexpr int issued = ((i - 1) * NJ * NRD + GAPS - 1) / GAPS;
      constexpr int allow = 2 * (4 - i) + issued;
      asm volatile("s_waitcnt lgkmcnt(%2)" : "+v"(alo[CUR][i]), "+v"(ahi[CUR][i]) : "n"(allow > 15 ? 15 : allow));
      __builtin_amdgcn_sched_barrier(0);
      const bf16x8_t ai = frag(alo[CUR][i], ahi[CUR][i]);
      auto gap = [&](auto j_tag) {
        constexpr int j = decltype(j_tag)::value;
        constexpr int g = (i - 1) * NJ + j;
        constexpr int r0 = (g * NRD + GAPS - 1) / GAPS, r1 = ((g + 1) * NRD + GAPS - 1) / GAPS;
        acc[i][j] = __builtin_amdgcn_mfma_f32_16x16x32_bf16(bf[j], ai, acc[i][j], 0, 0, 0);
        if constexpr (r1 > r0) w160_issue_read<BN_, NKS, r0>(alo[NXT], ahi[NXT], blo[NXT], bhi[NXT], aa, ba);
        if constexpr (r1 > r0 + 1) w160_issue_read<BN_, NKS, r0 + 1>(alo[NXT], ahi[NXT], blo[NXT], bhi[NXT], aa, ba);
        __builtin_amdgcn_sched_barrier(0);
      };
      gap(std::integral_constant<int, 0>{}); gap(std::integral_constant<int, 1>{}); gap(std::integral_constant<int, 2>{}); gap(std::integral_constant<int, 3>{});
      if constexpr (NJ == 5) gap(std::integral_constant<int, 4>{});
      if constexpr (BIAS) {
        if (bmask & (1u << i)) accb[i] = __builtin_amdgcn_mfma_f32_16x16x32_bf16(nk_ones_frag(), ai, accb[i], 0, 0, 0);
      }
    };
    row(std::integral_constant<int, 1>{}); row(std::integral_constant<int, 2>{}); row(std::integral_constant<int, 3>{}); row(std::integral_constant<int, 4>{});
  };

  W160_BAR();
  W160_STAMP(1); W160_STAMP_RT(4);
  set_stage(0);
  {
    auto rd = [&](auto r_tag) { w160_issue_read<BN_, 0, decltype(r_tag)::value>(alo[0], ahi[0], blo[0], bhi[0], aa, ba); };
    rd(std::integral_constant<int, 0>{}); rd(std::integral_constant<int, 1>{}); rd(std::integral_constant<int, 2>{}); rd(std::integral_constant<int, 3>{});
    rd(std::integral_constant<int, 4>{}); rd(std::integral_constant<int, 5>{}); rd(std::integral_constant<int, 6>{}); rd(std::integral_constant<int, 7>{});
    rd(std::integral_constant<int, 8>{}); rd(std::integral_constant<int, 9>{}); rd(std::integral_constant<int, 10>{}); rd(std::integral_constant<int, 11>{});
    rd(std::integral_constant<int, 12>{}); rd(std::integral_constant<int, 13>{}); rd(std::integral_constant<int, 14>{}); rd(std::integral_constant<int, 15>{});
    rd(std::integral_constant<int, 16>{}); rd(std::integral_constant<int, 17>{});
    if constexpr (NRD == 20) { rd(std::integral_constant<int, 18>{}); rd(std::integral_constant<int, 19>{}); }
  }
  if constexpr (NJ == 5)
    asm volatile("s_waitcnt lgkmcnt(0)" : "+v"(blo[0][0]), "+v"(bhi[0][0]), "+v"(blo[0][1]), "+v"(bhi[0][1]), "+v"(blo[0][2]), "+v"(bhi[0][2]), "+v"(blo[0][3]),
                 "+v"(bhi[0][3]), "+v"(blo[0][4]), "+v"(bhi[0][4]), "+v"(alo[0][0]), "+v"(ahi[0][0]), "+v"(alo[0][1]), "+v"(ahi[0][1]), "+v"(alo[0][2]),
                 "+v"(ahi[0][2]), "+v"(alo[0][3]), "+v"(ahi[0][3]), "+v"(alo[0][4]), "+v"(ahi[0][4]));
  else
    asm volatile("s_waitcnt lgkmcnt(0)" : "+v"(blo[0][0]), "+v"(bhi[0][0]), "+v"(blo[0][1]), "+v"(bhi[0][1]), "+v"(blo[0][2]), "+v"(bhi[0][2]), "+v"(blo[0][3]),
                 "+v"(bhi[0][3]), "+v"(alo[0][0]), "+v"(ahi[0][0]), "+v"(alo[0][1]), "+v"(ahi[0][1]), "+v"(alo[0][2]), "+v"(ahi[0][2]), "+v"(alo[0][3]),
                 "+v"(ahi[0][3]), "+v"(alo[0][4]), "+v"(ahi[0][4]));
  __builtin_amdgcn_sched_barrier(0);
  auto k_loop = [&](auto bias_tag) {
    unsigned so = 0;
    for (int t = 0; t < nk; ++t) {
      unsigned son = so + Cfg::STAGE; if (son == W160_NS * Cfg::STAGE) son = 0;
      substep(std::integral_constant<int, 0>{}, std::integral_constant<int, 1>{}, std::false_type{}, bias_tag, 0u);
      substep(std::integral_constant<int, 1>{}, std::integral_constant<int, 0>{}, std::true_type{}, bias_tag, son);
      so = son;
    }
  };
  if (bmask) k_loop(std::true_type{}); else k_loop(std::false_type{});
  asm volatile("s_waitcnt lgkmcnt(0)" ::: "memory");
  __builtin_amdgcn_s_setprio(0);
  W160_STAMP(2); W160_STAMP_RT(5);

  const int mb = m0 + wr * 80, nb = n0 + wc * (BN_ / 2);
  const int mode = gridDim.y > 1 ? 2 : (p.accumulate ? 1 : 0);
  if (dbias != nullptr && bmask) {
#pragma unroll
    for (int i = 0; i < 5; ++i) {
      if ((bmask & (1u << i)) && lane < 16) {
        const int m = mb + i * 16 + lane;
        if (m < p.M) {
          const float v = accb[i][0] * p.alpha;
          if (mode == 2) unsafeAtomicAdd(dbias + m, v);
          else dbias[m] = mode == 1 ? dbias[m] + v : v;
        }
      }
    }
  }
  float* const Cp = (float*)(p.nbatch ? p.Cb[blockIdx.z] : p.C);
  if (mode == 2) {
    W160_BAR();
    constexpr int BW = BN_ / 2, LDW = BW + 4;
    static_assert(4 * 80 * LDW * 4 <= Cfg::SMEM, "the four waves' staging images fit the ring");
    float* img = (float*)smem + wave * (80 * LDW);
#pragma unroll
    for (int i = 0; i < 5; ++i)
#pragma unroll
      for (int j = 0; j < NJ; ++j) {
        float4_t v = acc[i][j];
        v *= p.alpha;
        *(float4_t*)(img + (i * 16 + (lane & 15)) * LDW + j * 16 + (lane >> 4) * 4) = v;
      }
    for (int e = lane; e < 80 * BW; e += 64) {
      const int m = e / BW, n = e - m * BW;
      if (mb + m < p.M && nb + n < p.N) unsafeAtomicAdd(Cp + (long)(mb + m) * p.ldc + nb + n, img[m * LDW + n]);
    }
    return;
  }
#pragma unroll
  for (int half = 0; half < NJ / 2; ++half) {
    float4_t pair[5][2];
#pragma unroll
    for (int i = 0; i < 5; ++i) { pair[i][0] = acc[i][2 * half]; pair[i][1] = acc[i][2 * half + 1]; }
    reg_epilogue_64x32<1, 5>(p, Cp, pair, mb, nb + half * 32, lane);
  }
  if constexpr (NJ & 1) {
    float4_t last[5];
#pragma unroll
    for (int i = 0; i < 5; ++i) last[i] = acc[i][NJ - 1];
    reg_epilogue_col16<1, 5>(p, Cp, last, mb, nb + (NJ - 1) * 16, lane);
  }
#ifdef NK_W160_STAMPS
  asm volatile("s_waitcnt vmcnt(0)" ::: "memory");
  W160_STAMP(3);
#endif
}
#ifdef NK_W160_STAMPS
extern "C" int nk_debug_w160_stamps(unsigned long long* host_out, int nwg) {
  return hipMemcpyFromSymbol(host_out, HIP_SYMBOL(nk_w160_stamp_buf), (size_t)nwg * 12 * sizeof(unsigned long long)) == hipSuccess ? 0 : 1;
}
#endif

static int w160_mode() {
  int mode = 1;
  if (const char* e = getenv("NK_GEMM_W160")) mode = atoi(e);
  return mode;
}
struct W160Plan { int bn, splitk; };
static W160Plan w160_plan(const NkGemmParams& p, int amode, int bmode, int out_f32, int allow_splitk) {
  const int mode = w160_mode();
  if (!mode || amode != OP_MC || bmode != OP_MC || !out_f32) return {0, 0};
  if (p.nbatch > NK_MAX_BATCH) return {0, 0};
  const int nb = p.nbatch ? p.nbatch : 1;
  const long nk = (p.K + BK - 1) / BK;
  if (mode == 2) {
    int sk = 1;
    if (const char* e = getenv("NK_GEMM_W160_SPLIT")) sk = atoi(e);
    if (sk < 1 || !allow_splitk || nk < 2 * sk) sk = 1;
    return {p.N % 160 == 0 || p.N % 128 != 0 ? 160 : 128, sk};
  }
  if (p.M % W160_BM) return {0, 0};
  if (nk < 32) return {0, 0};
  W160Plan best = {0, 0};
  double best_us = 1e30;
  for (int bn = 160; bn >= 128; bn -= 32) {
    const long ntn = (p.N + bn - 1) / bn;
    if (ntn * bn * 100 > (long)p.N * 104) continue;
    const long tiles = (long)(p.M / W160_BM) * ntn * nb;
    for (int sk = 1; sk <= 8; ++sk) {
      if (sk > 1 && (!allow_splitk || nk / sk < 32)) break;
      const long wgs = tiles * sk, rounds = (wgs + 255) / 256;
      if ((double)wgs < 0.85 * (double)(rounds * 256)) continue;
      const double us = (double)rounds * (double)((nk + sk - 1) / sk) * 0.66 * bn / 160.0 + (sk > 1 ? sk * (double)p.M * p.N * nb * 4.0 / 0.6e6 : 0.0);
      if (us < best_us) { best_us = us; best = {bn, sk}; }
    }
  }
  return best;
}
template <int BN_>
static int launch_w160_as(NkGemmParams& p, int splitk, hipStream_t stream) {
  auto kern = nk_gemm_w160_kernel<BN_>;
  nk_optin_lds((const void*)kern, W160Cfg<BN_>::SMEM);
  dim3 grid(((p.M + W160_BM - 1) / W160_BM) * ((p.N + BN_ - 1) / BN_), splitk, p.nbatch ? p.nbatch : 1);
  hipLaunchKernelGGL(kern, grid, dim3(512), W160Cfg<BN_>::SMEM, stream, p);
  return nk_check_launch(BN_ == 160 ? "nk_gemm_w160_kernel<160>" : "nk_gemm_w160_kernel<128>");
}
```

### neurosis_amd/csrc/nk_gemm.h

```cpp
#pragma once
#include "nk_common.h"

struct NkGather {
  int H, W, C;
  int Ho, Wo;
  int KW;
  int rs, ks;
  int off_h, off_w;
  int div;
  int need_even;
  FastDiv fWo, fHoWo, fC, fKW;
};

struct NkTapW {
  long co_stride, tap_stride;
  FastDiv fCout;
};

struct NkGemmParams {
  const bf16_t* A;
  const bf16_t* B;
  long lda, ldb;
  int M, N, K;
  NkGather ga, gb;
  NkTapW tw;
  void* C;
  long ldc;
  float alpha;
  const float* bias;
  const bf16_t* residual;
  long ldr;
  const bf16_t* rowvec;
  long ld_rowvec;
  FastDiv fRowsPerBatch;
  int ksplit_len;
  int group_m;
  int accumulate;
  int lean_src;
  int k_rotate;
  int nbatch;
  const bf16_t* Ab[8];
  const bf16_t* Bb[8];
  void* Cb[8];
  unsigned* sk_counter;
  unsigned sk_base;
  unsigned* sk_flags;
  unsigned sk_epoch;
  float* sk_ws;
  int sk_chunked;
  int sk_debug;
  unsigned* sk_health;
  float* dbias;
  float* dbias_b[8];
  const bf16_t* geglu_u;
  long ld_u;
  bf16_t* geglu_h;
  long ld_h;
  int geglu_save;
  int halo_nb;
  float* stats_part;
  int stats_groups;
};
#define NK_MAX_BATCH 8

enum { NK_OP_KC = 0, NK_OP_KCG = 1, NK_OP_MC = 2, NK_OP_MCT = 3, NK_OP_MCG = 4 };

int nk_gemm_dispatch(NkGemmParams& p, int amode, int bmode, int out_f32, int allow_splitk, hipStream_t stream);
int nk_halo_tiles_per_image(const NkGemmParams& p);
int nk_halo_bn(int N);
int nk_geglu_fwd_fusable(const NkGemmParams& p);
```

### neurosis_amd/csrc/ops_gemm.hip

```cpp
#include "../../include/neurosis_hip.h"
#include "nk_gemm.h"
#include <string.h>

static NkGemmParams zero_params() {
  NkGemmParams p;
  memset(&p, 0, sizeof(p));
  p.alpha = 1.0f;
  p.fRowsPerBatch = make_fastdiv(1);
  p.ga.fWo = p.ga.fHoWo = p.ga.fC = p.ga.fKW = make_fastdiv(1);
  p.gb.fWo = p.gb.fHoWo = p.gb.fC = p.gb.fKW = make_fastdiv(1);
  p.tw.fCout = make_fastdiv(1);
  return p;
}

extern "C" int nk_linear_fwd(const void* x, const void* w, const float* bias, const void* residual, void* y,
                             int M, int N, int K, long ldx, long ldw, long ldr, long ldy, float alpha,
                             void* stream) {
  NkGemmParams p = zero_params();
  p.A = (const bf16_t*)x; p.lda = ldx;
  p.B = (const bf16_t*)w; p.ldb = ldw;
  p.M = M; p.N = N; p.K = K;
  p.C = y; p.ldc = ldy;
  p.bias = bias;
  p.residual = (const bf16_t*)residual; p.ldr = ldr;
  p.alpha = alpha;
  return nk_gemm_dispatch(p, NK_OP_KC, NK_OP_KC, 0, 0, (hipStream_t)stream);
}

extern "C" int nk_linear_fwd_batched(const void* const* x, const void* const* w, void* const* y, int count, int M, int N, int K,
                                     long ldx, long ldw, long ldy, void* stream) {
  NK_CHECK_ARG(x && w && y && count >= 1 && count <= NK_MAX_BATCH);
  NkGemmParams p = zero_params();
  p.lda = ldx; p.ldb = ldw;
  p.M = M; p.N = N; p.K = K;
  p.ldc = ldy;
  p.nbatch = count;
  for (int i = 0; i < count; ++i) {
    p.Ab[i] = (const bf16_t*)x[i];
    p.Bb[i] = (const bf16_t*)w[i];
    p.Cb[i] = y[i];
  }
  p.A = p.Ab[0]; p.B = p.Bb[0]; p.C = p.Cb[0];
  return nk_gemm_dispatch(p, NK_OP_KC, NK_OP_KC, 0, 0, (hipStream_t)stream);
}

extern "C" int nk_linear_dgrad(const void* dy, const void* w, const void* dx_add, void* dx, int M, int N, int K,
                               long lddy, long ldw, long ldadd, long lddx, void* stream) {
  NkGemmParams p = zero_params();
  p.A = (const bf16_t*)dy; p.lda = lddy;
  p.B = (const bf16_t*)w; p.ldb = ldw;
  p.M = M; p.N = K; p.K = N;
  p.C = dx; p.ldc = lddx;
  p.residual = (const bf16_t*)dx_add; p.ldr = ldadd;
  return nk_gemm_dispatch(p, NK_OP_KC, NK_OP_MC, 0, 0, (hipStream_t)stream);
}

static NkGemmParams geglu_fwd_params(const void* x, const void* w, const float* bias, void* u, void* h, int M, int I, int K, long ldx, long ldw,
                                      long ldu, long ldh) {
  NkGemmParams p = zero_params();
  p.A = (const bf16_t*)x; p.lda = ldx;
  p.B = (const bf16_t*)w; p.ldb = ldw;
  p.M = M; p.N = 2 * I; p.K = K;
  p.C = u; p.ldc = ldu;
  p.bias = bias;
  p.geglu_h = (bf16_t*)h; p.ld_h = ldh;
  return p;
}
extern "C" long nk_linear_fwd_geglu_ok(int M, int I, int K) {
  if (M <= 0 || I <= 0 || K <= 0 || (I & 127) || (K & 7)) return 0;
  NkGemmParams p = geglu_fwd_params(nullptr, nullptr, nullptr, nullptr, (void*)16, M, I, K, K, K, 2l * I, I);
  return nk_geglu_fwd_fusable(p);
}
extern "C" int nk_linear_fwd_geglu(const void* x, const void* w, const float* bias, void* u, void* h, int M, int I, int K, long ldx, long ldw,
                                   long ldu, long ldh, void* stream) {
  NK_CHECK_ARG(x && w && u && h && M > 0 && I > 0 && K > 0);
  NkGemmParams p = geglu_fwd_params(x, w, bias, u, h, M, I, K, ldx, ldw, ldu, ldh);
  return nk_gemm_dispatch(p, NK_OP_KC, NK_OP_KC, 0, 0, (hipStream_t)stream);
}

extern "C" int nk_linear_fwd_geglu_s(const void* x, const void* w, const float* bias, void* s, void* h, int M, int I, int K, long ldx, long ldw,
                                     long lds, long ldh, void* stream) {
  NK_CHECK_ARG(x && w && s && h && M > 0 && I > 0 && K > 0);
  NkGemmParams p = geglu_fwd_params(x, w, bias, s, h, M, I, K, ldx, ldw, lds, ldh);
  p.geglu_save = 1;
  return nk_gemm_dispatch(p, NK_OP_KC, NK_OP_KC, 0, 0, (hipStream_t)stream);
}

static int dgrad_geglu(const void* dy, const void* w, const void* u, void* du, int M, int N, int I, long lddy, long ldw, long ldu, long lddu, int save,
                       void* stream) {
  NK_CHECK_ARG(dy && w && u && du && I > 0 && (I & 7) == 0);
  NkGemmParams p = zero_params();
  p.A = (const bf16_t*)dy; p.lda = lddy;
  p.B = (const bf16_t*)w; p.ldb = ldw;
  p.M = M; p.N = I; p.K = N;
  p.C = du; p.ldc = lddu;
  p.geglu_u = (const bf16_t*)u; p.ld_u = ldu;
  p.geglu_save = save;
  return nk_gemm_dispatch(p, NK_OP_KC, NK_OP_MC, 0, 0, (hipStream_t)stream);
}
extern "C" int nk_linear_dgrad_geglu_s(const void* dy, const void* w, const void* s, void* du, int M, int N, int I, long lddy, long ldw,
                                       long lds, long lddu, void* stream) {
  return dgrad_geglu(dy, w, s, du, M, N, I, lddy, ldw, lds, lddu, 1, stream);
}

extern "C" int nk_linear_dgrad_geglu(const void* dy, const void* w, const void* u, void* du, int M, int N, int I, long lddy, long ldw,
                                     long ldu, long lddu, void* stream) {
  return dgrad_geglu(dy, w, u, du, M, N, I, lddy, ldw, ldu, lddu, 0, stream);
}

static int linear_wgrad(const void* dy, const void* x, float* dw, float* dbias, int M, int N, int K, long lddy, long ldx, long lddw,
                        int accumulate, void* stream) {
  NkGemmParams p = zero_params();
  p.A = (const bf16_t*)dy; p.lda = lddy;
  p.B = (const bf16_t*)x; p.ldb = ldx;
  p.M = N; p.N = K; p.K = M;
  p.C = dw; p.ldc = lddw;
  p.accumulate = accumulate;
  p.dbias = dbias;
  return nk_gemm_dispatch(p, NK_OP_MC, NK_OP_MC, 1, lddw == K, (hipStream_t)stream);
}
extern "C" int nk_linear_wgrad(const void* dy, const void* x, float* dw, int M, int N, int K, long lddy,
                               long ldx, long lddw, int accumulate, void* stream) {
  return linear_wgrad(dy, x, dw, nullptr, M, N, K, lddy, ldx, lddw, accumulate, stream);
}
extern "C" int nk_linear_wgrad_bias(const void* dy, const void* x, float* dw, float* dbias, int M, int N, int K, long lddy,
                                    long ldx, long lddw, int accumulate, void* stream) {
  NK_CHECK_ARG(dbias != nullptr);
  return linear_wgrad(dy, x, dw, dbias, M, N, K, lddy, ldx, lddw, accumulate, stream);
}

extern "C" int nk_linear_wgrad_batched(const void* const* dy, const void* const* x, float* const* dw, float* const* dbias, int count, int M,
                                       int N, int K, long lddy, long ldx, long lddw, int accumulate, void* stream) {
  NK_CHECK_ARG(dy && x && dw && count >= 1 && count <= NK_MAX_BATCH);
  NkGemmParams p = zero_params();
  p.lda = lddy; p.ldb = ldx;
  p.M = N; p.N = K; p.K = M;
  p.ldc = lddw;
  p.accumulate = accumulate;
  p.nbatch = count;
  for (int i = 0; i < count; ++i) {
    p.Ab[i] = (const bf16_t*)dy[i];
    p.Bb[i] = (const bf16_t*)x[i];
    p.Cb[i] = dw[i];
    p.dbias_b[i] = dbias ? dbias[i] : nullptr;
  }
  p.A = p.Ab[0]; p.B = p.Bb[0]; p.C = p.Cb[0];
  return nk_gemm_dispatch(p, NK_OP_MC, NK_OP_MC, 1, lddw == K, (hipStream_t)stream);
}

static int check_conv(const NkConvDesc* d) {
  NK_CHECK_ARG(d != nullptr);
  NK_CHECK_ARG(d->N > 0 && d->H > 0 && d->W > 0 && d->Cin > 0 && d->Cout > 0);
  NK_CHECK_ARG(d->KH > 0 && d->KW > 0 && (d->stride == 1 || d->stride == 2 || d->stride == 4));
  NK_CHECK_ARG((d->Cin & 7) == 0 && (d->Cout & 7) == 0);
  NK_CHECK_ARG(!(d->upsample && d->stride != 1));
  const int Hin = d->upsample ? 2 * d->H : d->H, Win = d->upsample ? 2 * d->W : d->W;
  NK_CHECK_ARG(d->Ho > 0 && d->Wo > 0);
  NK_CHECK_ARG((d->Ho - 1) * d->stride - d->pad_t < Hin && (d->Wo - 1) * d->stride - d->pad_l < Win);
  NK_CHECK_ARG((long)d->N * Hin * Win * (long)d->Cin < (1l << 31) && (long)d->N * d->Ho * d->Wo * (long)d->Cout < (1l << 31));
  return NK_OK;
}

static NkGather fwd_gather(const NkConvDesc* d) {
  NkGather g;
  memset(&g, 0, sizeof(g));
  g.H = d->H; g.W = d->W; g.C = d->Cin;
  g.Ho = d->Ho; g.Wo = d->Wo; g.KW = d->KW;
  g.rs = d->stride; g.ks = 1;
  g.off_h = -d->pad_t; g.off_w = -d->pad_l;
  g.div = d->upsample ? 2 : 1;
  g.need_even = 0;
  g.fWo = make_fastdiv(d->Wo); g.fHoWo = make_fastdiv(d->Ho * d->Wo);
  g.fC = make_fastdiv(d->Cin); g.fKW = make_fastdiv(d->KW);
  return g;
}

static NkGemmParams conv_fwd_params(const NkConvDesc* d, const void* x, const void* w, const float* bias, const void* rowvec,
                                    const void* residual, void* y) {
  NkGemmParams p = zero_params();
  p.A = (const bf16_t*)x;
  p.ga = fwd_gather(d);
  p.B = (const bf16_t*)w; p.ldb = (long)d->KH * d->KW * d->Cin;
  p.M = d->N * d->Ho * d->Wo; p.N = d->Cout; p.K = d->KH * d->KW * d->Cin;
  p.C = y; p.ldc = d->Cout;
  p.bias = bias;
  p.rowvec = (const bf16_t*)rowvec; p.ld_rowvec = d->Cout;
  p.fRowsPerBatch = make_fastdiv(d->Ho * d->Wo);
  p.residual = (const bf16_t*)residual; p.ldr = d->Cout;
  p.halo_nb = (d->KH == 3 && d->KW == 3) ? d->N : 0;
  return p;
}

extern "C" int nk_conv2d_fwd(const NkConvDesc* d, const void* x, const void* w, const float* bias,
                             const void* rowvec, const void* residual, void* y, void* stream) {
  if (int e = check_conv(d)) return e;
  NkGemmParams p = conv_fwd_params(d, x, w, bias, rowvec, residual, y);
  return nk_gemm_dispatch(p, NK_OP_KCG, NK_OP_KC, 0, 0, (hipStream_t)stream);
}

extern "C" long nk_conv2d_stats_tiles(const NkConvDesc* d, int stats_groups) {
  if (check_conv(d)) return 0;
  if (stats_groups < 0 || stats_groups > 32) return 0;
  if (stats_groups) {
    if (d->Cout % stats_groups) return 0;
    const int bn = nk_halo_bn(d->Cout), cpg = d->Cout / stats_groups;
    if (bn % cpg) return 0;
  }
  NkGemmParams p = conv_fwd_params(d, nullptr, nullptr, nullptr, nullptr, nullptr, nullptr);
  return nk_halo_tiles_per_image(p);
}

extern "C" int nk_conv2d_fwd_stats(const NkConvDesc* d, const void* x, const void* w, const float* bias, const void* rowvec,
                                   const void* residual, void* y, float* stats_part, int stats_groups, void* stream) {
  if (int e = check_conv(d)) return e;
  NK_CHECK_ARG(stats_part && stats_groups > 0);
  NK_CHECK_ARG(nk_conv2d_stats_tiles(d, stats_groups) > 0);
  NkGemmParams p = conv_fwd_params(d, x, w, bias, rowvec, residual, y);
  p.stats_part = stats_part; p.stats_groups = stats_groups;
  return nk_gemm_dispatch(p, NK_OP_KCG, NK_OP_KC, 0, 0, (hipStream_t)stream);
}

extern "C" int nk_conv2d_dgrad(const NkConvDesc* d, const void* dy, const void* w, void* dx, void* stream) {
  if (int e = check_conv(d)) return e;
  const int Hin = d->upsample ? 2 * d->H : d->H, Win = d->upsample ? 2 * d->W : d->W;
  NkGemmParams p = zero_params();
  NkGather g;
  memset(&g, 0, sizeof(g));
  g.H = d->Ho; g.W = d->Wo; g.C = d->Cout;
  g.Ho = Hin; g.Wo = Win; g.KW = d->KW;
  g.rs = 1; g.ks = -1;
  g.off_h = d->pad_t; g.off_w = d->pad_l;
  g.div = d->stride; g.need_even = d->stride - 1;
  g.fWo = make_fastdiv(Win); g.fHoWo = make_fastdiv(Hin * Win);
  g.fC = make_fastdiv(d->Cout); g.fKW = make_fastdiv(d->KW);
  p.A = (const bf16_t*)dy; p.ga = g;
  p.B = (const bf16_t*)w;
  p.tw.co_stride = (long)d->KH * d->KW * d->Cin;
  p.tw.tap_stride = d->Cin;
  p.tw.fCout = make_fastdiv(d->Cout);
  p.M = d->N * Hin * Win; p.N = d->Cin; p.K = d->KH * d->KW * d->Cout;
  p.C = dx; p.ldc = d->Cin;
  return nk_gemm_dispatch(p, NK_OP_KCG, NK_OP_MCT, 0, 0, (hipStream_t)stream);
}

extern "C" long nk_conv2d_dgrad_flipped_ok(const NkConvDesc* d) {
  if (check_conv(d) || d->KH != 3 || d->KW != 3 || d->stride != 1 || d->pad_t != 1 || d->pad_l != 1) return 0;
  const int Hin = d->upsample ? 2 * d->H : d->H, Win = d->upsample ? 2 * d->W : d->W;
  if (d->Ho != Hin || d->Wo != Win) return 0;
  NkConvDesc t = *d;
  t.H = Hin; t.W = Win; t.Cin = d->Cout; t.Cout = d->Cin; t.upsample = 0;
  NkGemmParams p = conv_fwd_params(&t, nullptr, nullptr, nullptr, nullptr, nullptr, nullptr);
  return nk_halo_tiles_per_image(p) > 0;
}

extern "C" int nk_conv2d_dgrad_flipped(const NkConvDesc* d, const void* dy, const void* wt, void* dx, void* stream) {
  NK_CHECK_ARG(nk_conv2d_dgrad_flipped_ok(d) == 1);
  const int Hin = d->upsample ? 2 * d->H : d->H, Win = d->upsample ? 2 * d->W : d->W;
  NkConvDesc t = *d;
  t.H = Hin; t.W = Win; t.Cin = d->Cout; t.Cout = d->Cin; t.upsample = 0;
  NkGemmParams p = conv_fwd_params(&t, dy, wt, nullptr, nullptr, nullptr, dx);
  return nk_gemm_dispatch(p, NK_OP_KCG, NK_OP_KC, 0, 0, (hipStream_t)stream);
}

static int conv_wgrad(const NkConvDesc* d, const void* dy, const void* x, float* dw, float* dbias, int accumulate, void* stream) {
  if (int e = check_conv(d)) return e;
  NkGemmParams p = zero_params();
  p.A = (const bf16_t*)dy; p.lda = d->Cout;
  p.B = (const bf16_t*)x; p.gb = fwd_gather(d);
  p.M = d->Cout; p.N = d->KH * d->KW * d->Cin; p.K = d->N * d->Ho * d->Wo;
  p.C = dw; p.ldc = p.N;
  p.accumulate = accumulate;
  p.dbias = dbias;
  p.halo_nb = (d->KH == 3 && d->KW == 3) ? d->N : 0;
  return nk_gemm_dispatch(p, NK_OP_MC, NK_OP_MCG, 1, 1, (hipStream_t)stream);
}
extern "C" int nk_conv2d_wgrad(const NkConvDesc* d, const void* dy, const void* x, float* dw, int accumulate,
                               void* stream) {
  return conv_wgrad(d, dy, x, dw, nullptr, accumulate, stream);
}
extern "C" int nk_conv2d_wgrad_bias(const NkConvDesc* d, const void* dy, const void* x, float* dw, float* dbias, int accumulate,
                                    void* stream) {
  NK_CHECK_ARG(dbias != nullptr);
  return conv_wgrad(d, dy, x, dw, dbias, accumulate, stream);
}
```

### neurosis_amd/lib.py

```python
from __future__ import annotations

import ctypes as C
import os
from pathlib import Path

import torch

CSRC = Path(__file__).resolve().parent / "csrc"
LIB_PATH = CSRC / "libneurosis_hip.so"

vp, i32, i64, f32 = C.c_void_p, C.c_int, C.c_long, C.c_float


class NkConvDesc(C.Structure):
    _fields_ = [(n, i32) for n in ("N", "H", "W", "Cin", "Cout", "KH", "KW", "stride", "pad_t", "pad_l", "Ho", "Wo", "upsample")]


class NkAttnDesc(C.Structure):
    _fields_ = (
        [(n, i32) for n in ("B", "H", "Lq", "Lk", "D")]
        + [(n, i64) for n in ("sq", "sk", "sv", "so", "bq", "bk", "bv", "bo", "sdq", "sdk", "sdv", "sdo", "bdq", "bdk", "bdv", "bdo")]
        + [("scale", f32), ("causal", i32)]
    )


NK_COLPART_MAX = 32


class NkColpartBatch(C.Structure):
    _fields_ = [("part", vp * NK_COLPART_MAX), ("dgamma", vp * NK_COLPART_MAX), ("dbeta", vp * NK_COLPART_MAX), ("nrows", i32 * NK_COLPART_MAX),
                ("C", i32 * NK_COLPART_MAX), ("accumulate", i32 * NK_COLPART_MAX), ("n", i32)]


cdp, adp = C.POINTER(NkConvDesc), C.POINTER(NkAttnDesc)

SIGNATURES: dict[str, list] = {
    "nk_linear_fwd": [vp, vp, vp, vp, vp, i32, i32, i32, i64, i64, i64, i64, f32, vp],
    "nk_linear_dgrad": [vp, vp, vp, vp, i32, i32, i32, i64, i64, i64, i64, vp],
    "nk_linear_dgrad_geglu": [vp, vp, vp, vp, i32, i32, i32, i64, i64, i64, i64, vp],
    "nk_linear_fwd_geglu": [vp, vp, vp, vp, vp, i32, i32, i32, i64, i64, i64, i64, vp],
    "nk_linear_fwd_geglu_s": [vp, vp, vp, vp, vp, i32, i32, i32, i64, i64, i64, i64, vp],
    "nk_linear_dgrad_geglu_s": [vp, vp, vp, vp, i32, i32, i32, i64, i64, i64, i64, vp],
    "nk_linear_wgrad": [vp, vp, vp, i32, i32, i32, i64, i64, i64, i32, vp],
    "nk_linear_fwd_batched": [C.POINTER(vp), C.POINTER(vp), C.POINTER(vp), i32, i32, i32, i32, i64, i64, i64, vp],
    "nk_linear_wgrad_batched": [C.POINTER(vp), C.POINTER(vp), C.POINTER(vp), C.POINTER(vp), i32, i32, i32, i32, i64, i64, i64, i32, vp],
    "nk_linear_wgrad_bias": [vp, vp, vp, vp, i32, i32, i32, i64, i64, i64, i32, vp],
    "nk_conv2d_wgrad_bias": [cdp, vp, vp, vp, vp, i32, vp],
    "nk_conv2d_fwd": [cdp, vp, vp, vp, vp, vp, vp, vp],
    "nk_conv2d_fwd_stats": [cdp, vp, vp, vp, vp, vp, vp, vp, i32, vp],
    "nk_conv_weight_flip": [vp, vp, i32, i32, i32, vp],
    "nk_conv3x3_few_channels_fwd": [vp, vp, vp, vp, i32, i32, i32, i32, i32, vp],
    "nk_conv2d_dgrad": [cdp, vp, vp, vp, vp],
    "nk_conv2d_dgrad_flipped": [cdp, vp, vp, vp, vp],
    "nk_conv2d_wgrad": [cdp, vp, vp, vp, i32, vp],
    "nk_attention_fwd": [adp, vp, vp, vp, vp, vp, vp],
    "nk_attention_bwd": [adp, vp, vp, vp, vp, vp, vp, vp, vp, vp, vp, vp],
    "nk_attention_bwd_causal": [adp, vp, vp, vp, vp, vp, vp, vp, vp, vp, vp],
    "nk_softmax_rows": [vp, i64, i32, vp],
    "nk_softmax_rows_bwd": [vp, vp, i64, i32, f32, vp],
    "nk_groupnorm_fwd": [vp, vp, vp, vp, vp, vp, vp, i32, i32, i32, i32, f32, i32, vp],
    "nk_groupnorm_sums": [vp, vp, vp, i32, i32, i32, i32, vp],
    "nk_groupnorm_sums_from_parts": [vp, vp, vp, i32, i32, i32, vp],
    "nk_groupnorm_apply": [vp, vp, vp, vp, vp, vp, vp, i32, i32, i32, i32, f32, i32, vp],
    "nk_groupnorm_bwd": [vp, vp, vp, vp, vp, vp, vp, vp, vp, vp, vp, i32, i32, i32, i32, i32, i32, vp],
    "nk_layernorm_fwd": [vp, vp, vp, vp, vp, vp, i32, i32, f32, vp],
    "nk_layernorm_bwd": [vp, vp, vp, vp, vp, vp, vp, vp, vp, vp, i32, i32, i32, vp],
    "nk_layernorm_bwd_dx": [vp, vp, vp, vp, vp, vp, vp, i32, i32, vp],
    "nk_layernorm_bwd_rows": [vp, vp, vp, vp, vp, vp, vp, vp, i32, i32, vp],
    "nk_colpart_reduce_batch": [C.POINTER(NkColpartBatch), vp],
    "nk_layernorm_bwd_params": [vp, vp, vp, vp, vp, vp, vp, i32, i32, i32, vp],
    "nk_geglu_fwd": [vp, vp, i64, i32, vp],
    "nk_geglu_bwd": [vp, vp, vp, i64, i32, vp],
    "nk_geglu_fwd_s": [vp, vp, vp, i64, i32, vp],
    "nk_geglu_bwd_s": [vp, vp, vp, i64, i32, vp],
    "nk_silu_fwd": [vp, vp, i64, vp],
    "nk_gelu_fwd": [vp, vp, i64, i32, vp],
    "nk_gelu_bwd": [vp, vp, vp, i64, i32, vp],
    "nk_embedding_bwd": [vp, vp, i64, vp, vp, i32, i32, i32, i32, i32, i32, vp],
    "nk_gather_rows_bwd": [vp, i64, vp, vp, i32, i32, i32, vp],
    "nk_wgrad_few_rows": [vp, i64, vp, i64, vp, i64, i32, i32, i32, i32, vp],
    "nk_leaky_relu_fwd": [vp, vp, i64, f32, vp],
    "nk_leaky_relu_bwd": [vp, vp, vp, i64, f32, vp],
    "nk_maxpool2x2_fwd": [vp, vp, i32, i32, i32, i32, vp],
    "nk_maxpool2x2_bwd": [vp, vp, vp, i32, i32, i32, i32, vp],
    "nk_maxpool_fwd": [vp, vp, i32, i32, i32, i32, i32, i32, vp],
    "nk_maxpool_bwd": [vp, vp, vp, i32, i32, i32, i32, i32, i32, vp],
    "nk_lpips_layer_fwd": [vp, vp, vp, vp, vp, i32, i32, i32, f32, i32, vp],
    "nk_lpips_layer_bwd": [vp, vp, vp, vp, vp, i32, i32, i32, f32, vp],
    "nk_batchnorm_fwd": [vp, vp, vp, vp, vp, vp, vp, vp, vp, i64, i32, f32, f32, f32, vp],
    "nk_batchnorm_bwd": [vp, vp, vp, vp, vp, vp, vp, vp, vp, vp, i64, i32, f32, i32, vp],
    "nk_batchnorm_eval": [vp, vp, vp, vp, vp, vp, vp, i64, i32, f32, f32, vp],
    "nk_silu_bwd": [vp, vp, vp, i64, vp],
    "nk_add": [vp, vp, vp, i64, vp],
    "nk_cat_channels": [vp, vp, vp, i64, i32, i32, vp],
    "nk_split_channels": [vp, vp, vp, i64, i32, i32, vp],
    "nk_upsample2x_bwd": [vp, vp, i32, i32, i32, i32, vp],
    "nk_nchw_to_nhwc": [vp, i32, vp, i32, i32, i32, i32, f32, vp],
    "nk_nhwc_to_nchw": [vp, vp, i32, i32, i32, i32, i32, vp],
    "nk_cast_f32_to_bf16": [vp, vp, i64, vp],
    "nk_cast_bf16_to_f32": [vp, vp, i64, vp],
    "nk_colsum": [vp, vp, vp, i64, i32, i64, i32, vp],
    "nk_colsum_batched": [vp, vp, vp, i64, i32, i64, i32, i32, vp],
    "nk_timestep_embedding": [vp, vp, i32, i32, f32, vp],
    "nk_edm_prepare": [vp, vp, vp, vp, vp, vp, i32, i32, i32, i32, vp],
    "nk_edm_loss": [vp, vp, vp, vp, vp, vp, vp, vp, i32, i32, i32, i32, f32, vp],
    "nk_sample_prepare": [vp, vp, vp, i32, i32, i32, i32, i32, vp],
    "nk_sample_denoise": [vp, vp, vp, vp, f32, vp, i32, i32, i32, i32, i32, vp],
    "nk_sample_euler_step": [vp, vp, vp, vp, vp, vp, f32, vp, vp, i32, i32, i32, i32, i32, vp],
    "nk_adamw_flat": [vp, vp, vp, vp, vp, i64, f32, f32, f32, f32, f32, i32, f32, vp],
    "nk_ema_flat": [vp, vp, i64, f32, vp],
    "nk_debug_raise_health": [vp],
    "nk_debug_stamp": [vp, vp],
    "nk_debug_launch_log": [i32],
    "nk_health_clear": [],
    "nk_health_export": [vp, vp],
    "nk_health_import": [vp, vp],
    "nk_adafactor_init": [vp, vp],
    "nk_adafactor_chunk": [vp, vp],
    "nk_came_chunk": [vp, vp],
    "nk_adamw8bit_step": [vp, vp],
}

SIZE_QUERIES: dict[str, list] = {
    "nk_groupnorm_ws_floats": [i32, i32, i32, i32],
    "nk_groupnorm_sums_ws_floats": [i32, i32, i32],
    "nk_conv2d_stats_tiles": [cdp, i32],
    "nk_conv2d_dgrad_flipped_ok": [cdp],
    "nk_linear_fwd_geglu_ok": [i32, i32, i32],
    "nk_layernorm_ws_floats": [i32, i32],
    "nk_layernorm_part_rows": [i32],
    "nk_colsum_ws_floats": [i64, i32],
    "nk_batchnorm_ws_floats": [i64, i32],
    "nk_lpips_layer_ws_floats": [i32, i32],
    "nk_attention_bwd_ws_floats": [adp],
    "nk_adafactor_tensor_bytes": [],
    "nk_came_tensor_bytes": [],
    "nk_adamw8bit_tensor_bytes": [],
    "nk_gemm_sk_status": [],
    "nk_health_status": [],
    "nk_debug_launch_names": [C.c_char_p, i64],
}

_lib = None


class NkError(RuntimeError):
    pass


def load() -> C.CDLL:
    global _lib
    if _lib is not None:
        return _lib
    path = Path(os.environ.get("NEUROSIS_HIP_LIB", LIB_PATH))
    if not path.exists():
        raise NkError(
            f"{path} not found: the HIP extension is not built. Run `python -c 'import __graft_entry__ as g; g.build()'` "
            "(or `make -C neurosis_amd/csrc`). There is no CPU fallback for the product path."
        )
    lib = C.CDLL(str(path))
    lib.nk_last_error.restype = C.c_char_p
    lib.nk_last_error.argtypes = []
    lib.nk_abi_version.restype = i32
    lib.nk_abi_version.argtypes = []
    for name, argtypes in SIGNATURES.items():
        fn = getattr(lib, name)
        fn.argtypes = argtypes
        fn.restype = i32
    for name, argtypes in SIZE_QUERIES.items():
        fn = getattr(lib, name)
        fn.argtypes = argtypes
        fn.restype = i64
    _lib = lib
    return lib


def launch_log(mode: int) -> None:
    call("nk_debug_launch_log", int(mode))


def launched() -> list[str]:
    buf = C.create_string_buffer(8192)
    n = query("nk_debug_launch_names", buf, len(buf))
    if n < 0:
        raise NkError("nk_debug_launch_names failed")
    return buf.value.decode().split("\n")[:-1]


def query(name: str, *args) -> int:
    return int(getattr(load(), name)(*args))


def call(name: str, *args) -> None:
    lib = load()
    rc = getattr(lib, name)(*args)
    if rc != 0:
        raise NkError(f"{name} failed (rc={rc}): {lib.nk_last_error().decode()}")
```

### neurosis_amd/ops.py

```python
from __future__ import annotations

import ctypes as C
import os
import threading
import weakref
from dataclasses import dataclass
from typing import Callable, Optional

import torch
from torch import Tensor

from . import lib
from .lib import NkAttnDesc, NkConvDesc, call, query

BF16 = torch.bfloat16


class EngineState:

    _live = weakref.WeakSet()

    def __init__(self, wgrad_stream=None):
        self.grad_accumulate = False
        self.assume_zeroed = False
        self.wgrad_stream = wgrad_stream
        self.batch_wgrads = os.environ.get("NK_BATCH_WGRADS", "1") != "0"
        self.norm_params_on_side_stream: Optional[bool] = None
        self.deferred: Optional[list] = None
        self.segment_hook: Optional[Callable] = None
        EngineState._live.add(self)

    def derived(self) -> "EngineState":
        return EngineState(self.wgrad_stream)


_capture_depth = 0


def capturing() -> bool:
    return _capture_depth > 0


class capture_scope:
    def __enter__(self):
        global _capture_depth
        _capture_depth += 1

    def __exit__(self, *exc):
        global _capture_depth
        _capture_depth -= 1


state = EngineState()
state.param_epoch = 0


def state_of(p) -> EngineState:
    if p is not None:
        st = getattr(p, "_nk_state", None)
        if st is not None:
            return st
        store = getattr(p, "_nk_store", None)
        if store is not None:
            return store.state
    return state


def wgrad_mode(p=None) -> int:
    st = state_of(p)
    if st.grad_accumulate:
        return 1
    return 2 if st.assume_zeroed else 0


_recording = threading.local()


class recording_backward:

    def __enter__(self):
        _recording.depth = getattr(_recording, "depth", 0) + 1

    def __exit__(self, *exc):
        _recording.depth -= 1


def recording() -> bool:
    return getattr(_recording, "depth", 0) > 0


def on_wgrad_stream(fn: Callable[[], None], *reads: Tensor, owner=None) -> None:
    st = state_of(owner)
    side = st.wgrad_stream
    if side is None:
        fn()
        return
    if st.deferred is not None:
        st.deferred.append((fn, reads))
        return
    side.wait_stream(torch.cuda.current_stream())
    with torch.cuda.stream(side):
        fn()
    for t in reads:
        if t is not None:
            t.record_stream(side)


class WgradQueue:

    def __init__(self, owner=None):
        self.items = []
        self.colparts = []
        self.owner = owner

    MAX_ELEMS = 2 << 20

    @classmethod
    def takes(cls, weight: Tensor) -> bool:
        return weight.numel() <= cls.MAX_ELEMS

    def add(self, dy: Tensor, x: Tensor, dw: Tensor, db: Optional[Tensor] = None) -> None:
        self.items.append((dy, x, dw, db))

    def add_colpart(self, part: Tensor, dgamma: Tensor, dbeta: Tensor, nrows: int, Cc: int, accumulate: bool) -> None:
        self.colparts.append((part, dgamma, dbeta, nrows, Cc, accumulate))

    def flush(self) -> None:
        colparts, self.colparts = self.colparts, []
        if colparts:
            on_wgrad_stream(lambda: colpart_reduce(colparts), *[c[0] for c in colparts], owner=self.owner)
        items, self.items = self.items, []
        if not items:
            return
        groups = {}
        for it in items:
            dy, x, dw, _db = it
            key = (dy.shape[0], dy.shape[1], x.shape[1], dy.stride(0), x.stride(0), dw.stride(0))
            groups.setdefault(key, []).append(it)
        mode = wgrad_mode(self.owner)

        def run():
            for (M, N, K, lddy, ldx, lddw), its in groups.items():
                for i in range(0, len(its), 8):
                    chunk = its[i:i + 8]
                    if len(chunk) == 1:
                        gemm_tn_f32(chunk[0][0], chunk[0][1], chunk[0][2], mode, dbias=chunk[0][3])
                        continue
                    n = len(chunk)
                    arr = C.c_void_p * n
                    call("nk_linear_wgrad_batched", arr(*[c[0].data_ptr() for c in chunk]), arr(*[c[1].data_ptr() for c in chunk]),
                         arr(*[c[2].data_ptr() for c in chunk]), arr(*[None if c[3] is None else c[3].data_ptr() for c in chunk]), n, M, N, K,
                         lddy, ldx, lddw, mode, _stream())

        on_wgrad_stream(run, *[t for it in items for t in it[:2]], owner=self.owner)


def colpart_reduce(entries) -> None:
    for i in range(0, len(entries), lib.NK_COLPART_MAX):
        chunk = entries[i:i + lib.NK_COLPART_MAX]
        b = lib.NkColpartBatch()
        for z, (part, dgamma, dbeta, nrows, Cc, acc) in enumerate(chunk):
            b.part[z], b.dgamma[z], b.dbeta[z] = part.data_ptr(), dgamma.data_ptr(), dbeta.data_ptr()
            b.nrows[z], b.C[z], b.accumulate[z] = nrows, Cc, int(acc)
        b.n = len(chunk)
        call("nk_colpart_reduce_batch", C.byref(b), _stream())


_wgrad_queue: Optional[WgradQueue] = None


class batched_wgrads:

    def __init__(self, owner=None):
        self.owner = owner

    def __enter__(self):
        global _wgrad_queue
        self.prev = _wgrad_queue
        _wgrad_queue = WgradQueue(self.owner) if state_of(self.owner).batch_wgrads else None
        return _wgrad_queue

    def __exit__(self, *exc):
        global _wgrad_queue
        q, _wgrad_queue = _wgrad_queue, self.prev
        if exc[0] is None and q is not None:
            q.flush()
        return False


def join_wgrad_stream(owner=None) -> None:
    if owner is not None:
        st = state_of(owner)
        side = st.wgrad_stream
        if side is not None and st.deferred is None:
            torch.cuda.current_stream().wait_stream(side)
        return
    seen = set()
    for st in list(EngineState._live):
        side = st.wgrad_stream
        if side is not None and st.deferred is None and id(side) not in seen:
            seen.add(id(side))
            torch.cuda.current_stream().wait_stream(side)


def _ws(n_floats: int, device) -> Tensor:
    return torch.empty(n_floats, dtype=torch.float32, device=device)


def _p(t: Optional[Tensor]):
    return None if t is None else t.data_ptr()


def _stream():
    return torch.cuda.current_stream().cuda_stream


def _check2d(t: Tensor, name: str):
    if t.dim() != 2 or t.stride(1) != 1 or t.dtype != BF16 or not t.is_cuda:
        raise ValueError(f"{name}: expected a 2-D bf16 CUDA tensor with unit inner stride, got {tuple(t.shape)} {t.dtype} {t.stride()} {t.device}")


@dataclass
class Img:

    t: Tensor
    N: int
    H: int
    W: int
    sums: Optional[Tensor] = None

    @property
    def C(self) -> int:
        return self.t.shape[1]

    @staticmethod
    def from_nchw(x: Tensor) -> "Img":
        N, Cc, H, W = x.shape
        if x.dtype == BF16 and x.permute(0, 2, 3, 1).is_contiguous():
            return Img(x.permute(0, 2, 3, 1).reshape(N * H * W, Cc), N, H, W)
        return Img(nchw_to_tokens(x, Cc), N, H, W)

    def to_nchw(self) -> Tensor:
        return self.t.view(self.N, self.H, self.W, self.C).permute(0, 3, 1, 2)


def _param_stamp(p: Tensor):
    st = getattr(p, "_nk_store", None)
    if st is not None:
        return ("epoch", id(st), st.epoch)
    return ("version", p._version, p.data_ptr())


def shadow(p: Tensor) -> Tensor:
    if getattr(p, "_nk_store", None) is not None:
        return p._nk_shadow
    s = getattr(p, "_nk_shadow", None)
    stamp = _param_stamp(p)
    if s is not None and getattr(p, "_nk_shadow_stamp", None) == stamp:
        return s
    flat = _phys_flat(p)
    n = flat.numel()
    if s is not None and n % 8 == 0 and s.numel() == n and s.device == p.device:
        call("nk_cast_f32_to_bf16", flat.data_ptr(), s.data_ptr(), n, _stream())
        p._nk_shadow_stamp = stamp
        return s
    s = torch.empty(flat.numel(), dtype=BF16, device=p.device)
    if n % 8 == 0:
        call("nk_cast_f32_to_bf16", flat.data_ptr(), s.data_ptr(), n, _stream())
    else:
        pad = torch.zeros((n + 7) // 8 * 8, dtype=torch.float32, device=p.device)
        pad[:n] = flat
        s8 = torch.empty(pad.numel(), dtype=BF16, device=p.device)
        call("nk_cast_f32_to_bf16", pad.data_ptr(), s8.data_ptr(), pad.numel(), _stream())
        s = s8[:n]
    p._nk_shadow = s
    p._nk_shadow_stamp = stamp
    return s


def _phys_flat(p: Tensor) -> Tensor:
    d = p.detach()
    if d.dim() == 4:
        d = d.permute(0, 2, 3, 1)
    if not d.is_contiguous():
        raise ValueError("parameter storage must be dense (conv weights in channels_last memory format)")
    return d.reshape(-1)


def grad_flat(p: Tensor) -> Tensor:
    if p.grad is None:
        g = torch.zeros_like(p, memory_format=torch.preserve_format)
        p.grad = g
    g = p.grad
    if g.dim() == 4:
        g = g.permute(0, 2, 3, 1)
    if not g.is_contiguous():
        raise ValueError("parameter .grad must share the parameter's physical layout")
    return g.reshape(-1)


def w2d(p: Tensor) -> Tensor:
    return shadow(p).view(p.shape[0], -1)


def g2d(p: Tensor) -> Tensor:
    return grad_flat(p).view(p.shape[0], -1)


def conv_weight_param(out_ch: int, in_ch: int, kh: int, kw: int) -> torch.nn.Parameter:
    base = torch.empty(out_ch, kh, kw, in_ch)
    return torch.nn.Parameter(base.permute(0, 3, 1, 2))


def nchw_to_tokens(x: Tensor, cpad: int, scale: float = 1.0) -> Tensor:
    N, Cc, H, W = x.shape
    x = x.contiguous()
    if x.dtype not in (torch.float32, BF16):
        raise ValueError(f"unsupported dtype {x.dtype}")
    out = torch.empty(N * H * W, cpad, dtype=BF16, device=x.device)
    call("nk_nchw_to_nhwc", x.data_ptr(), int(x.dtype == torch.float32), out.data_ptr(), N, Cc, H * W, cpad, scale, _stream())
    return out


def tokens_to_nchw(t: Tensor, N: int, Cc: int, H: int, W: int, dtype=torch.float32) -> Tensor:
    _check2d(t, "t")
    out = torch.empty(N, Cc, H, W, dtype=dtype, device=t.device)
    call("nk_nhwc_to_nchw", t.data_ptr(), out.data_ptr(), int(dtype == torch.float32), N, Cc, H * W, t.shape[1], _stream())
    return out


def cast_bf16(x: Tensor) -> Tensor:
    if x.dtype == BF16:
        return x
    x = x.contiguous()
    out = torch.empty(x.shape, dtype=BF16, device=x.device)
    n = x.numel()
    if n % 8:
        raise ValueError("cast_bf16 needs numel % 8 == 0")
    call("nk_cast_f32_to_bf16", x.data_ptr(), out.data_ptr(), n, _stream())
    return out


def add(a: Tensor, b: Tensor) -> Tensor:
    if a.shape != b.shape or not a.is_contiguous() or not b.is_contiguous():
        raise ValueError("add: contiguous tensors of equal shape expected")
    out = torch.empty_like(a)
    call("nk_add", a.data_ptr(), b.data_ptr(), out.data_ptr(), a.numel(), _stream())
    return out


def gemm_nt(x: Tensor, w: Tensor, bias: Optional[Tensor] = None, residual: Optional[Tensor] = None, alpha: float = 1.0, out: Optional[Tensor] = None) -> Tensor:
    _check2d(x, "x")
    _check2d(w, "w")
    M, K = x.shape
    N = w.shape[0]
    if w.shape[1] != K:
        raise ValueError(f"gemm_nt: K mismatch {x.shape} vs {w.shape}")
    if out is None:
        out = torch.empty(M, N, dtype=BF16, device=x.device)
    if residual is not None:
        _check2d(residual, "residual")
    call("nk_linear_fwd", x.data_ptr(), w.data_ptr(), _p(bias), _p(residual), out.data_ptr(), M, N, K, x.stride(0), w.stride(0),
         residual.stride(0) if residual is not None else 0, out.stride(0), float(alpha), _stream())
    return out


def gemm_nt_batched(xs, ws, outs=None):
    M, K = xs[0].shape
    N = ws[0].shape[0]
    for x, w in zip(xs, ws):
        _check2d(x, "x")
        _check2d(w, "w")
        if x.shape != (M, K) or w.shape != (N, K) or x.stride(0) != xs[0].stride(0) or w.stride(0) != ws[0].stride(0):
            raise ValueError("gemm_nt_batched: every problem must have the same shape and strides")
    if outs is None:
        outs = [torch.empty(M, N, dtype=BF16, device=xs[0].device) for _ in xs]
    for i in range(0, len(xs), 8):
        n = min(8, len(xs) - i)
        arr = C.c_void_p * n
        call("nk_linear_fwd_batched", arr(*[t.data_ptr() for t in xs[i:i + n]]), arr(*[t.data_ptr() for t in ws[i:i + n]]),
             arr(*[t.data_ptr() for t in outs[i:i + n]]), n, M, N, K, xs[0].stride(0), ws[0].stride(0), outs[0].stride(0), _stream())
    return outs


def gemm_nn(dy: Tensor, w: Tensor, dx_add: Optional[Tensor] = None, out: Optional[Tensor] = None) -> Tensor:
    _check2d(dy, "dy")
    _check2d(w, "w")
    M, N = dy.shape
    K = w.shape[1]
    if w.shape[0] != N:
        raise ValueError(f"gemm_nn: N mismatch {dy.shape} vs {w.shape}")
    if out is None:
        out = torch.empty(M, K, dtype=BF16, device=dy.device)
    if dx_add is not None:
        _check2d(dx_add, "dx_add")
    call("nk_linear_dgrad", dy.data_ptr(), w.data_ptr(), _p(dx_add), out.data_ptr(), M, N, K, dy.stride(0), w.stride(0),
         dx_add.stride(0) if dx_add is not None else 0, out.stride(0), _stream())
    return out


def gemm_tn_f32(dy: Tensor, x: Tensor, dw: Tensor, accumulate, dbias: Optional[Tensor] = None) -> None:
    _check2d(dy, "dy")
    _check2d(x, "x")
    M, N = dy.shape
    K = x.shape[1]
    if x.shape[0] != M or dw.shape != (N, K) or dw.dtype != torch.float32 or dw.stride(1) != 1:
        raise ValueError(f"gemm_tn_f32: bad shapes {dy.shape} {x.shape} {dw.shape}")
    if dbias is None:
        call("nk_linear_wgrad", dy.data_ptr(), x.data_ptr(), dw.data_ptr(), M, N, K, dy.stride(0), x.stride(0), dw.stride(0), int(accumulate), _stream())
        return
    if dbias.shape != (N,) or dbias.dtype != torch.float32 or not dbias.is_contiguous():
        raise ValueError(f"gemm_tn_f32: dbias must be a dense fp32 [{N}] tensor")
    call("nk_linear_wgrad_bias", dy.data_ptr(), x.data_ptr(), dw.data_ptr(), dbias.data_ptr(), M, N, K, dy.stride(0), x.stride(0), dw.stride(0),
         int(accumulate), _stream())


def colsum(dy: Tensor, out: Tensor, accumulate: bool) -> None:
    _check2d(dy, "dy")
    M, N = dy.shape
    ws = _ws(query("nk_colsum_ws_floats", M, N), dy.device)
    call("nk_colsum", dy.data_ptr(), out.data_ptr(), ws.data_ptr(), M, N, dy.stride(0), int(accumulate), _stream())


def linear_fwd(x: Tensor, weight: Tensor, bias: Optional[Tensor], residual: Optional[Tensor] = None, need_dx: bool = True, x_saved=None):
    y = gemm_nt(x, w2d(weight), bias, residual)
    return y, _linear_bwd(x if x_saved is None else x_saved, weight, bias, need_dx)


def geglu_save_enabled() -> bool:
    return os.environ.get("NK_GEGLU_SAVE", "1") != "0"


def linear_geglu_fwd(x: Tensor, weight: Tensor, bias: Optional[Tensor], x_saved=None, save_derivative: bool = False):
    _check2d(x, "x")
    M, K = x.shape
    I2 = weight.shape[0]
    I = I2 // 2
    wq = w2d(weight)
    if I2 % 2 == 0 and x.is_contiguous() and query("nk_linear_fwd_geglu_ok", M, I, K):
        u = torch.empty(M, I2, dtype=BF16, device=x.device)
        h = torch.empty(M, I, dtype=BF16, device=x.device)
        call("nk_linear_fwd_geglu_s" if save_derivative else "nk_linear_fwd_geglu", x.data_ptr(), wq.data_ptr(), _p(bias), u.data_ptr(), h.data_ptr(), M, I, K,
             x.stride(0), wq.stride(0), u.stride(0), h.stride(0), _stream())
    else:
        u = gemm_nt(x, wq, bias, None)
        if save_derivative:
            h = torch.empty(M, I, dtype=BF16, device=x.device)
            call("nk_geglu_fwd_s", u.data_ptr(), h.data_ptr(), u.data_ptr(), M, I, _stream())
        else:
            h = geglu_fwd(u)[0]
    return u, h, _linear_bwd(x if x_saved is None else x_saved, weight, bias, True)


def _linear_bwd(x_in, weight: Tensor, bias: Optional[Tensor], need_dx: bool):
    def bwd(dy: Tensor, dx_add: Optional[Tensor] = None, geglu_u: Optional[Tensor] = None, geglu_s: Optional[Tensor] = None):
        entry = "nk_linear_dgrad_geglu"
        if geglu_s is not None:
            if geglu_u is not None:
                raise ValueError("linear bwd: geglu_u and geglu_s are exclusive")
            geglu_u, entry = geglu_s, "nk_linear_dgrad_geglu_s"
        x = x_in() if callable(x_in) else x_in
        queued = _wgrad_queue is not None and _wgrad_queue.takes(weight) and dy.is_contiguous() and x.is_contiguous()
        db = grad_flat(bias) if bias is not None else None
        if queued:
            _wgrad_queue.add(dy, x, g2d(weight), db)
        else:
            on_wgrad_stream(lambda: gemm_tn_f32(dy, x, g2d(weight), wgrad_mode(weight), dbias=db), dy, x, owner=weight)
        if not need_dx:
            return None
        if geglu_u is not None:
            if dx_add is not None:
                raise ValueError("linear bwd: geglu_u and dx_add are exclusive")
            M, N = dy.shape
            K = weight.shape[1]
            _check2d(geglu_u, "geglu_u")
            if geglu_u.shape != (M, 2 * K):
                raise ValueError(f"linear bwd: geglu_u must be [{M}, {2 * K}], got {tuple(geglu_u.shape)}")
            du = torch.empty(M, 2 * K, dtype=BF16, device=dy.device)
            wq = w2d(weight)
            call(entry, dy.data_ptr(), wq.data_ptr(), geglu_u.data_ptr(), du.data_ptr(), M, N, K, dy.stride(0), wq.stride(0),
                 geglu_u.stride(0), du.stride(0), _stream())
            return du
        return gemm_nn(dy, w2d(weight), dx_add)

    return bwd


def _conv_desc(N, H, W, Cin, Cout, KH, KW, stride, pad_t, pad_l, Ho, Wo, upsample) -> NkConvDesc:
    return NkConvDesc(N, H, W, Cin, Cout, KH, KW, stride, pad_t, pad_l, Ho, Wo, int(upsample))


def groupnorm_sums(x: Img, groups: int) -> Tensor:
    if x.sums is not None and x.sums.shape == (x.N, 2 * groups):
        return x.sums
    sums = torch.empty(x.N, 2 * groups, dtype=torch.float32, device=x.t.device)
    ws = _ws(query("nk_groupnorm_ws_floats", x.N, x.H * x.W, x.C, groups), x.t.device)
    call("nk_groupnorm_sums", x.t.data_ptr(), sums.data_ptr(), ws.data_ptr(), x.N, x.H * x.W, x.C, groups, _stream())
    return sums


def conv2d_fwd(x: Img, weight: Tensor, bias: Optional[Tensor], stride: int = 1, padding=1, upsample: bool = False,
               rowvec: Optional[Tensor] = None, residual: Optional[Tensor] = None, need_dx: bool = True,
               asym_pad: bool = False, stats_groups: Optional[int] = None, cin_real: Optional[int] = None):
    Cout, Cin, KH, KW = weight.shape
    if x.C != Cin:
        raise ValueError(f"conv2d: input has {x.C} channels, weight expects {Cin}")
    Hin, Win = (2 * x.H, 2 * x.W) if upsample else (x.H, x.W)
    if asym_pad:
        pad_t = pad_l = 0
        Ho = (Hin + 1 - KH) // stride + 1
        Wo = (Win + 1 - KW) // stride + 1
    else:
        pad_t = pad_l = int(padding)
        Ho = (Hin + 2 * pad_t - KH) // stride + 1
        Wo = (Win + 2 * pad_l - KW) // stride + 1
    d = _conv_desc(x.N, x.H, x.W, Cin, Cout, KH, KW, stride, pad_t, pad_l, Ho, Wo, upsample)
    y = torch.empty(x.N * Ho * Wo, Cout, dtype=BF16, device=x.t.device)
    _check2d(x.t, "x")
    if not x.t.is_contiguous():
        raise ValueError("conv2d: x must be dense channels-last")
    tiles = query("nk_conv2d_stats_tiles", C.byref(d), stats_groups) if stats_groups else 0
    sums_out = None
    if tiles:
        dev = x.t.device
        part = torch.empty(x.N, tiles, 2 * stats_groups, dtype=torch.float32, device=dev)
        call("nk_conv2d_fwd_stats", C.byref(d), x.t.data_ptr(), w2d(weight).data_ptr(), _p(bias), _p(rowvec), _p(residual), y.data_ptr(),
             part.data_ptr(), stats_groups, _stream())
        sums_out = torch.empty(x.N, 2 * stats_groups, dtype=torch.float32, device=dev)
        ws = _ws(query("nk_groupnorm_sums_ws_floats", x.N, tiles, stats_groups), dev)
        call("nk_groupnorm_sums_from_parts", part.data_ptr(), sums_out.data_ptr(), ws.data_ptr(), x.N, tiles, stats_groups, _stream())
    elif (cin_real in (3, 4) and Cin == 8 and KH == 3 and KW == 3 and stride == 1 and pad_t == 1 and not asym_pad and not upsample and rowvec is None
          and residual is None and Cout % 8 == 0):
        call("nk_conv3x3_few_channels_fwd", x.t.data_ptr(), w2d(weight).data_ptr(), _p(bias), y.data_ptr(), x.N, x.H, x.W, Cout, cin_real, _stream())
    else:
        call("nk_conv2d_fwd", C.byref(d), x.t.data_ptr(), w2d(weight).data_ptr(), _p(bias), _p(rowvec), _p(residual), y.data_ptr(), _stream())
    out = Img(y, x.N, Ho, Wo, sums_out)

    def bwd(dy: Tensor):
        _check2d(dy, "dy")
        if not dy.is_contiguous():
            raise ValueError("conv2d bwd: dy must be dense")
        acc = state_of(weight).grad_accumulate

        if weight.requires_grad:
            if bias is not None:
                on_wgrad_stream(lambda: call("nk_conv2d_wgrad_bias", C.byref(d), dy.data_ptr(), x.t.data_ptr(), g2d(weight).data_ptr(), grad_flat(bias).data_ptr(),
                                             wgrad_mode(weight), _stream()), dy, x.t, owner=weight)
            else:
                on_wgrad_stream(lambda: call("nk_conv2d_wgrad", C.byref(d), dy.data_ptr(), x.t.data_ptr(), g2d(weight).data_ptr(), wgrad_mode(weight), _stream()),
                                dy, x.t, owner=weight)
        drow = None
        if rowvec is not None:
            drow32 = torch.empty(x.N, Cout, dtype=torch.float32, device=dy.device)
            ws = _ws(x.N * query("nk_colsum_ws_floats", Ho * Wo, Cout), dy.device)
            call("nk_colsum_batched", dy.data_ptr(), drow32.data_ptr(), ws.data_ptr(), Ho * Wo, Cout, dy.stride(0), x.N, 0, _stream())
            drow = cast_bf16(drow32)
        dx = None
        if need_dx:
            dxt = torch.empty(x.N * Hin * Win, Cin, dtype=BF16, device=dy.device)
            if query("nk_conv2d_dgrad_flipped_ok", C.byref(d)):
                wt = torch.empty(Cin * 9 * Cout, dtype=BF16, device=dy.device)
                call("nk_conv_weight_flip", w2d(weight).data_ptr(), wt.data_ptr(), Cout, Cin, 9, _stream())
                call("nk_conv2d_dgrad_flipped", C.byref(d), dy.data_ptr(), wt.data_ptr(), dxt.data_ptr(), _stream())
            else:
                call("nk_conv2d_dgrad", C.byref(d), dy.data_ptr(), w2d(weight).data_ptr(), dxt.data_ptr(), _stream())
            if upsample:
                dsm = torch.empty(x.N * x.H * x.W, Cin, dtype=BF16, device=dy.device)
                call("nk_upsample2x_bwd", dxt.data_ptr(), dsm.data_ptr(), x.N, x.H, x.W, Cin, _stream())
                dxt = dsm
            dx = Img(dxt, x.N, x.H, x.W)
        return dx, drow

    return out, bwd


def groupnorm_fwd(x: Img, weight: Tensor, bias: Tensor, groups: int, eps: float, silu: bool):
    if not x.t.is_contiguous():
        raise ValueError("groupnorm: x must be dense channels-last")
    N, HW, Cc = x.N, x.H * x.W, x.C
    y = torch.empty_like(x.t)
    mean = torch.empty(N, groups, dtype=torch.float32, device=x.t.device)
    rstd = torch.empty_like(mean)
    nws = query("nk_groupnorm_ws_floats", N, HW, Cc, groups)
    if x.sums is not None and x.sums.shape == (N, 2 * groups):
        call("nk_groupnorm_apply", x.t.data_ptr(), x.sums.data_ptr(), weight.data_ptr(), bias.data_ptr(), y.data_ptr(), mean.data_ptr(),
             rstd.data_ptr(), N, HW, Cc, groups, float(eps), int(silu), _stream())
    else:
        ws = _ws(nws, x.t.device)
        call("nk_groupnorm_fwd", x.t.data_ptr(), weight.data_ptr(), bias.data_ptr(), y.data_ptr(), mean.data_ptr(), rstd.data_ptr(),
             ws.data_ptr(), N, HW, Cc, groups, float(eps), int(silu), _stream())

    def bwd(dy: Tensor, dx_add: Optional[Tensor] = None):
        dx = torch.empty_like(x.t)
        ws2 = _ws(nws, dy.device)
        call("nk_groupnorm_bwd", dy.data_ptr(), x.t.data_ptr(), weight.data_ptr(), bias.data_ptr(), mean.data_ptr(), rstd.data_ptr(),
             _p(dx_add), dx.data_ptr(), grad_flat(weight).data_ptr(), grad_flat(bias).data_ptr(), ws2.data_ptr(), N, HW, Cc, groups,
             int(silu), int(state_of(weight).grad_accumulate), _stream())
        return dx

    return Img(y, x.N, x.H, x.W), bwd


def layernorm_fwd(x: Tensor, weight: Tensor, bias: Tensor, eps: float = 1e-5):
    _check2d(x, "x")
    if not x.is_contiguous():
        raise ValueError("layernorm: x must be dense")
    M, Cc = x.shape
    y = torch.empty_like(x)
    mean = torch.empty(M, dtype=torch.float32, device=x.device)
    rstd = torch.empty_like(mean)
    call("nk_layernorm_fwd", x.data_ptr(), weight.data_ptr(), bias.data_ptr(), y.data_ptr(), mean.data_ptr(), rstd.data_ptr(), M, Cc, float(eps), _stream())

    def bwd(dy: Tensor, dx_add: Optional[Tensor] = None):
        dx = torch.empty_like(x)
        acc = state_of(weight).grad_accumulate
        if os.environ.get("NK_LN_FUSED", "1") != "0":
            rows = query("nk_layernorm_part_rows", M)
            part = torch.empty(rows * 2 * Cc, dtype=torch.float32, device=dy.device)
            call("nk_layernorm_bwd_rows", dy.data_ptr(), x.data_ptr(), weight.data_ptr(), mean.data_ptr(), rstd.data_ptr(), _p(dx_add),
                 dx.data_ptr(), part.data_ptr(), M, Cc, _stream())
            entry = (part, grad_flat(weight), grad_flat(bias), rows, Cc, bool(acc))
            if _wgrad_queue is not None:
                _wgrad_queue.add_colpart(*entry)
            else:
                on_wgrad_stream(lambda: colpart_reduce([entry]), part, owner=weight)
            return dx
        ws = _ws(query("nk_layernorm_ws_floats", M, Cc), dy.device)
        call("nk_layernorm_bwd_dx", dy.data_ptr(), x.data_ptr(), weight.data_ptr(), mean.data_ptr(), rstd.data_ptr(), _p(dx_add),
             dx.data_ptr(), M, Cc, _stream())

        def params():
            call("nk_layernorm_bwd_params", dy.data_ptr(), x.data_ptr(), mean.data_ptr(), rstd.data_ptr(),
                 grad_flat(weight).data_ptr(), grad_flat(bias).data_ptr(), ws.data_ptr(), M, Cc, int(acc), _stream())

        st_ = state_of(weight)
        if st_.norm_params_on_side_stream if st_.norm_params_on_side_stream is not None else st_.deferred is not None:
            on_wgrad_stream(params, dy, x, mean, rstd, ws, owner=weight)
        else:
            params()
        return dx

    return y, bwd


def geglu_fwd(u: Tensor):
    _check2d(u, "u")
    M, I2 = u.shape
    inner = I2 // 2
    y = torch.empty(M, inner, dtype=BF16, device=u.device)
    call("nk_geglu_fwd", u.data_ptr(), y.data_ptr(), M, inner, _stream())

    def bwd(dy: Tensor):
        du = torch.empty_like(u)
        call("nk_geglu_bwd", dy.data_ptr(), u.data_ptr(), du.data_ptr(), M, inner, _stream())
        return du

    return y, bwd


def gelu(x: Tensor, quick: bool = False) -> Tensor:
    y = torch.empty_like(x)
    call("nk_gelu_fwd", x.data_ptr(), y.data_ptr(), x.numel(), int(quick), _stream())
    return y


def gelu_fwd(x: Tensor, quick: bool = False):
    if not x.is_contiguous():
        raise ValueError("gelu_fwd: x must be dense")
    y = gelu(x, quick)

    def bwd(dy: Tensor) -> Tensor:
        if dy.shape != x.shape or dy.dtype != BF16 or not dy.is_contiguous():
            raise ValueError("gelu bwd: dy must be a dense bf16 tensor of x's shape")
        dx = torch.empty_like(x)
        call("nk_gelu_bwd", dy.data_ptr(), x.data_ptr(), dx.data_ptr(), x.numel(), int(quick), _stream())
        return dx

    return y, bwd


def embedding_bwd(ids: Tensor, dx: Tensor, table: Tensor, positions: Tensor) -> None:
    _check2d(dx, "dx")
    B, L = ids.shape
    V, Cc = table.shape
    P = positions.shape[0]
    if ids.dtype != torch.int64 or not ids.is_contiguous() or dx.shape != (B * L, Cc) or positions.shape[1] != Cc:
        raise ValueError(f"embedding_bwd: ids [B, L] int64 and dx [B * L, {Cc}] expected, got {tuple(ids.shape)} {ids.dtype}, {tuple(dx.shape)}")
    call("nk_embedding_bwd", ids.data_ptr(), dx.data_ptr(), dx.stride(0), grad_flat(table).data_ptr(), grad_flat(positions).data_ptr(), B, L, V, P,
         Cc, wgrad_mode(table), _stream())


def gather_rows_bwd(dsel: Tensor, idx: Tensor, L: int) -> Tensor:
    _check2d(dsel, "dsel")
    B, Cc = dsel.shape
    if idx.shape != (B,) or idx.dtype != torch.int64 or not idx.is_contiguous():
        raise ValueError("gather_rows_bwd: idx must be a dense int64 [B] tensor")
    dx = torch.empty(B * L, Cc, dtype=BF16, device=dsel.device)
    call("nk_gather_rows_bwd", dsel.data_ptr(), dsel.stride(0), idx.data_ptr(), dx.data_ptr(), B, L, Cc, _stream())
    return dx


def wgrad_few_rows(x: Tensor, dy: Tensor, dw: Tensor, accumulate: bool) -> None:
    _check2d(x, "x")
# ... 278 lines not shown
```

Measured before the change: 26.39.

## Replace split-K atomic accumulation with scratch slabs and a reduction kernel

Split-K weight-gradient GEMMs and the conv wgrad halo kernel now write each non-first split into a separate fp32 scratch slab instead of atomically adding into a pre-zeroed output. A follow-up kernel sums the slabs into the destination. This removes the zero-fill launches and the atomic contention, and makes the result deterministic. It costs extra scratch memory and traffic, an additional reduction launch, and a per-call scratch-size query and allocation from Python, with a cap that can limit the split count.

Result: no change. 26.37 (-0.1%).

```diff
diff --git a/include/neurosis_hip.h b/include/neurosis_hip.h
--- a/include/neurosis_hip.h
+++ b/include/neurosis_hip.h
@@ -25,6 +25,9 @@
                     long lddw, int accumulate, void* stream);
 int nk_linear_wgrad_bias(const void* dy, const void* x, float* dw, float* dbias, int M, int N, int K, long lddy, long ldx, long lddw,
                          int accumulate, void* stream);
+long nk_linear_wgrad_scratch_bytes(int M, int N, int K, long lddy, long ldx, long lddw, int has_bias, int count);
+int nk_linear_wgrad_ws(const void* dy, const void* x, float* dw, float* dbias, int M, int N, int K, long lddy, long ldx, long lddw,
+                       int accumulate, float* scratch, long scratch_bytes, void* stream);
 
 int nk_gemm_sk_status(void);
 
@@ -44,6 +47,8 @@
 
 int nk_linear_wgrad_batched(const void* const* dy, const void* const* x, float* const* dw, float* const* dbias, int count, int M, int N,
                             int K, long lddy, long ldx, long lddw, int accumulate, void* stream);
+int nk_linear_wgrad_batched_ws(const void* const* dy, const void* const* x, float* const* dw, float* const* dbias, int count, int M, int N,
+                               int K, long lddy, long ldx, long lddw, int accumulate, float* scratch, long scratch_bytes, void* stream);
 
 typedef struct NkConvDesc {
   int N, H, W, Cin;
@@ -66,6 +71,9 @@
 int nk_conv2d_dgrad(const NkConvDesc* d, const void* dy, const void* w, void* dx, void* stream);
 int nk_conv2d_wgrad(const NkConvDesc* d, const void* dy, const void* x, float* dw, int accumulate, void* stream);
 int nk_conv2d_wgrad_bias(const NkConvDesc* d, const void* dy, const void* x, float* dw, float* dbias, int accumulate, void* stream);
+long nk_conv2d_wgrad_scratch_bytes(const NkConvDesc* d, int has_bias);
+int nk_conv2d_wgrad_ws(const NkConvDesc* d, const void* dy, const void* x, float* dw, float* dbias, int accumulate, float* scratch,
+                       long scratch_bytes, void* stream);
 
 typedef struct NkAttnDesc {
   int B, H, Lq, Lk, D;
diff --git a/neurosis_amd/csrc/conv_wgrad_halo.h b/neurosis_amd/csrc/conv_wgrad_halo.h
--- a/neurosis_amd/csrc/conv_wgrad_halo.h
+++ b/neurosis_amd/csrc/conv_wgrad_halo.h
@@ -138,10 +138,11 @@
     }
   }
 
-  float* dw = (float*)p.C;
+  float* dw = split ? nk_split_slab(p, split, gridDim.x / nblk, 0) : (float*)p.C;
+  float* db = split ? nk_split_bias_slab(p, split, gridDim.x / nblk, 0, 1) : p.dbias;
   const int ci = ib * WH_BCI + is * 32 + (lane & 31);
   const int co_base = cb * WH_BCO + cs * 32 + 4 * h;
-  const bool atomic = gridDim.x > (unsigned)nblk || p.accumulate == 1;
+  const bool add = !split && p.accumulate == 1;
 #pragma unroll
   for (int t = 0; t < 9; ++t)
 #pragma unroll
@@ -150,8 +151,7 @@
       if (co < Cout) {
         float* dst = dw + (long)co * p.ldc + t * Cin + ci;
         const float v = acc[t][r] * p.alpha;
-        if (atomic) unsafeAtomicAdd(dst, v);
-        else *dst = v;
+        *dst = add ? *dst + v : v;
       }
     }
   if constexpr (BIAS) {
@@ -159,8 +159,7 @@
       bsum += __shfl_xor(bsum, 32);
       const int co = cb * WH_BCO + cs * 32 + (lane & 31);
       if (lane < 32 && co < Cout) {
-        if (atomic) unsafeAtomicAdd(p.dbias + co, bsum * p.alpha);
-        else p.dbias[co] = bsum * p.alpha;
+        db[co] = add ? db[co] + bsum * p.alpha : bsum * p.alpha;
       }
     }
   }
@@ -184,6 +183,7 @@
   for (int s = 1; s <= 64 && s <= T; ++s) {
     const long tiles = (T + s - 1) / s;
     const long rounds = (nblk * s + 255) / 256;
+    if (split_scratch_bytes(p, s) > NK_SPLIT_WS_CAP) break;
     const double cost = (double)rounds * (tiles * 3.0e-6 + 4.0e-6) + (s > 1 ? s * dw_bytes / 1.3e12 : dw_bytes / 4.0e12);
     if (cost < best * 0.97) { best = cost; best_s = s; }
   }
@@ -204,17 +204,13 @@
   int per = 0;
   const int S = wgrad_halo_splits(p, per);
   const long nblk = (long)((p.M + WH_BCO - 1) / WH_BCO) * (p.gb.C / WH_BCI);
-  if (S > 1 && p.accumulate == 0) {
-    const size_t n = (size_t)p.M * p.N;
-    const unsigned blocks = (unsigned)((n / 4 + 255) / 256 > 2048 ? 2048 : (n / 4 + 255) / 256);
-    hipLaunchKernelGGL(nk_zero_f32_kernel, dim3(blocks ? blocks : 1), dim3(256), 0, stream, (float*)p.C, n);
-    if (p.dbias) hipLaunchKernelGGL(nk_zero_f32_kernel, dim3(1), dim3(256), 0, stream, p.dbias, (size_t)p.M);
-    if (hipGetLastError() != hipSuccess) return NK_ERR_LAUNCH;
-  }
+  if (p.plan_only) { p.split_ws_bytes = split_scratch_bytes(p, S); return NK_OK; }
   p.accumulate = p.accumulate == 1 ? 1 : 0;
+  if (int rc = split_prepare(p, S, stream)) return rc;
   p.ksplit_len = per;
   auto kern = p.dbias ? nk_conv3x3_wgrad_halo_kernel<1> : nk_conv3x3_wgrad_halo_kernel<0>;
   nk_optin_lds((const void*)kern, WH_SMEM);
   hipLaunchKernelGGL(kern, dim3((unsigned)(nblk * S)), dim3(512), WH_SMEM, stream, p);
-  return nk_check_launch(p.dbias ? "nk_conv3x3_wgrad_halo_kernel<bias=1>" : "nk_conv3x3_wgrad_halo_kernel<bias=0>");
-}
+  if (int rc = nk_check_launch(p.dbias ? "nk_conv3x3_wgrad_halo_kernel<bias=1>" : "nk_conv3x3_wgrad_halo_kernel<bias=0>")) return rc;
+  return split_sum_launch(p, S, stream);
+}
diff --git a/neurosis_amd/csrc/gemm.hip b/neurosis_amd/csrc/gemm.hip
--- a/neurosis_amd/csrc/gemm.hip
+++ b/neurosis_amd/csrc/gemm.hip
@@ -34,6 +34,12 @@
   return (((long)n * g.H + h) * g.W + w) * g.C + c;
 }
 
+__device__ __forceinline__ float* nk_split_slab(const NkGemmParams& p, int split, int S, int z) {
+  return p.split_ws + ((long)z * (S - 1) + (split - 1)) * ((long)p.M * p.N);
+}
+__device__ __forceinline__ float* nk_split_bias_slab(const NkGemmParams& p, int split, int S, int z, int nz) {
+  return p.split_ws + (long)nz * (S - 1) * ((long)p.M * p.N) + ((long)z * (S - 1) + (split - 1)) * p.M;
+}
 template <int OUT_F32, int TBM = BM, int TNT = NTHREADS, int NJ = 4>
 __device__ __forceinline__ void nk_gemm_epilogue(const NkGemmParams& p, char* smem, float4_t (&acc)[4][NJ], int m0, int n0, int tid,
                                                  int lane, int wm, int wn) {
@@ -105,8 +111,11 @@
   }
 
   if constexpr (OUT_F32) {
-    float* C = (float*)(p.nbatch ? p.Cb[blockIdx.z] : p.C);
-    if (!p.accumulate && (p.N & 3) == 0 && (p.ldc & 3) == 0) {
+    const int split = blockIdx.y;
+    float* C = split ? nk_split_slab(p, split, gridDim.y, blockIdx.z) : (float*)(p.nbatch ? p.Cb[blockIdx.z] : p.C);
+    const long ldc = split ? p.N : p.ldc;
+    const bool add = !split && p.accumulate;
+    if ((p.N & 3) == 0 && (ldc & 3) == 0) {
       for (int it = 0; it < (TBM * BN / 4) / TNT; ++it) {
         int idx = tid + it * TNT;
         int row = idx >> 5, c4 = (idx & 31) * 4;
@@ -114,7 +123,9 @@
         if (m < p.M && n < p.N) {
           float4_t v = *(const float4_t*)(cs + row * CS_LD + c4);
           v *= p.alpha;
-          *(float4_t*)(C + (long)m * p.ldc + n) = v;
+          float4_t* dst = (float4_t*)(C + (long)m * ldc + n);
+          if (add) v += *dst;
+          *dst = v;
         }
       }
       return;
@@ -125,9 +136,8 @@
       int m = m0 + row, n = n0 + col;
       if (m < p.M && n < p.N) {
         float v = cs[row * CS_LD + col] * p.alpha;
-        float* dst = C + (long)m * p.ldc + n;
-        if (p.accumulate) unsafeAtomicAdd(dst, v);
-        else *dst = v;
+        float* dst = C + (long)m * ldc + n;
+        *dst = add ? *dst + v : v;
       }
     }
   } else {
@@ -468,15 +478,14 @@
   const short8_t o = {0x3F80, 0x3F80, 0x3F80, 0x3F80, 0x3F80, 0x3F80, 0x3F80, 0x3F80};
   return __builtin_bit_cast(bf16x8_t, o);
 }
-__device__ __forceinline__ void nk_store_bias_rows(float* db, const float4_t& a, int row0, int M, float alpha, int mode, int lane) {
+__device__ __forceinline__ void nk_store_bias_rows(float* db, const float4_t& a, int row0, int M, float alpha, bool add, int lane) {
   if (lane & 15) return;
 #pragma unroll
   for (int r = 0; r < 4; ++r) {
     const int m = row0 + (lane >> 4) * 4 + r;
     if (m < M) {
       const float v = a[r] * alpha;
-      if (mode == 2) unsafeAtomicAdd(db + m, v);
-      else db[m] = mode == 1 ? db[m] + v : v;
+      db[m] = add ? db[m] + v : v;
     }
   }
 }
@@ -587,9 +596,10 @@
   }
   if constexpr (CAN_BIAS) {
     if (do_bias) {
-      const int mode = gridDim.y > 1 ? 2 : (p.accumulate ? 1 : 0);
-#pragma unroll
-      for (int u = 0; u < BPW; ++u) nk_store_bias_rows(dbias, accb[u], m0 + wm * 64 + (wn * BPW + u) * 16, p.M, p.alpha, mode, lane);
+      const int split = blockIdx.y;
+      float* db = split ? nk_split_bias_slab(p, split, gridDim.y, blockIdx.z, gridDim.z) : dbias;
+#pragma unroll
+      for (int u = 0; u < BPW; ++u) nk_store_bias_rows(db, accb[u], m0 + wm * 64 + (wn * BPW + u) * 16, p.M, p.alpha, !split && p.accumulate, lane);
     }
   }
   __syncthreads();
@@ -722,7 +732,10 @@
     if (++cur_stage == RING_NS) cur_stage = 0;
   }
   if constexpr (CAN_BIAS) {
-    if (do_bias) nk_store_bias_rows(p.dbias, accb, m0 + wm * 64 + wn * 16, p.M, p.alpha, gridDim.y > 1 ? 2 : (p.accumulate ? 1 : 0), lane);
+    if (do_bias) {
+      const int split = blockIdx.y;
+      nk_store_bias_rows(split ? nk_split_bias_slab(p, split, gridDim.y, 0, 1) : p.dbias, accb, m0 + wm * 64 + wn * 16, p.M, p.alpha, !split && p.accumulate, lane);
+    }
   }
   __syncthreads();
   nk_gemm_epilogue<OUT_F32, BM, 512, NJ>(p, smem, acc, m0, n0, tid, lane, wm, wn);
@@ -1420,7 +1433,9 @@
 }
 
 static bool use_xl(const NkGemmParams& p, int amode, int bmode, int out_f32, int splitk);
-__global__ void nk_zero_f32_kernel(float* __restrict__ dst, size_t n);
+#include <mutex>
+#include <unordered_map>
+#include "split_sum.h"
 #include "gemm_g2.h"
 #include "gemm_w160.h"
 #include "conv_halo.h"
@@ -1485,8 +1500,6 @@
 }
 
 
-#include <mutex>
-#include <unordered_map>
 struct SkWorkspace {
   unsigned* counter = nullptr;
   unsigned* flags = nullptr;
@@ -1576,13 +1589,6 @@
   return nk_check_launch("nk_gemm_sk_kernel");
 }
 
-__global__ __launch_bounds__(256) void nk_zero_f32_kernel(float* __restrict__ dst, size_t n) {
-  const size_t n4 = n / 4, stride = (size_t)gridDim.x * 256;
-  float4_t* d4 = (float4_t*)dst;
-  for (size_t i = (size_t)blockIdx.x * 256 + threadIdx.x; i < n4; i += stride) d4[i] = (float4_t){0.f, 0.f, 0.f, 0.f};
-  if (blockIdx.x == 0 && threadIdx.x < (n & 3)) dst[n4 * 4 + threadIdx.x] = 0.f;
-}
-
 static int pick_splitk(int M, int N, int K, int max_split) {
   int tiles = ((M + BM - 1) / BM) * ((N + BN - 1) / BN);
   int nk = (K + BK - 1) / BK;
@@ -1598,18 +1604,6 @@
   int nk = (p.K + BK - 1) / BK;
   int per = (nk + splitk - 1) / splitk;
   p.ksplit_len = per * BK;
-}
-
-static int zero_split_outputs(const NkGemmParams& p, hipStream_t stream) {
-  for (int z = 0; z < (p.nbatch ? p.nbatch : 1); ++z) {
-    const size_t n = (size_t)p.M * p.N;
-    float* dst = (float*)(p.nbatch ? p.Cb[z] : p.C);
-    const unsigned blocks = (unsigned)((n / 4 + 255) / 256 > 2048 ? 2048 : (n / 4 + 255) / 256);
-    hipLaunchKernelGGL(nk_zero_f32_kernel, dim3(blocks ? blocks : 1), dim3(256), 0, stream, dst, n);
-    float* db = p.nbatch ? p.dbias_b[z] : p.dbias;
-    if (db) hipLaunchKernelGGL(nk_zero_f32_kernel, dim3(1), dim3(256), 0, stream, db, (size_t)p.M);
-  }
-  return hipGetLastError() != hipSuccess ? NK_ERR_LAUNCH : NK_OK;
 }
 
 int nk_gemm_dispatch(NkGemmParams& p, int amode, int bmode, int out_f32, int allow_splitk,
@@ -1644,7 +1638,7 @@
     set_split(p, 1);
     return launch<OP_KC, OP_MC, 0>(p, 1, stream);
   }
-  if (use_halo(p, amode, bmode, out_f32)) return launch_halo(p, stream);
+  if (use_halo(p, amode, bmode, out_f32)) return p.plan_only ? NK_OK : launch_halo(p, stream);
   if (use_wgrad_halo(p, amode, bmode, out_f32)) return launch_wgrad_halo(p, stream);
   if (p.stats_part) {
     nk_set_error(__FILE__, __LINE__, "statistics epilogue on a convolution the halo-tile kernel does not take (ask nk_conv2d_stats_tiles first)");
@@ -1654,20 +1648,18 @@
   {
     const W160Plan wp = w160_plan(p, amode, bmode, out_f32, allow_splitk);
     if (wp.bn) {
+      if (p.plan_only) { p.split_ws_bytes = split_scratch_bytes(p, wp.splitk); return NK_OK; }
       set_split(p, wp.splitk);
-      if (wp.splitk > 1 && p.accumulate == 0) {
-        NK_CHECK_ARG(p.ldc == p.N);
-        if (int rc = zero_split_outputs(p, stream)) return rc;
-        p.accumulate = 1;
-      } else if (p.accumulate == 2) {
-        p.accumulate = wp.splitk > 1 ? 1 : 0;
-      }
+      if (int rc = split_prepare(p, wp.splitk, stream)) return rc;
+      if (p.accumulate == 2) p.accumulate = 0;
       p.k_rotate = k_rotate_on(wp.splitk > 1 ? p.ksplit_len : p.K) ? 1 : 0;
-      return wp.bn == 160 ? launch_w160_as<160>(p, wp.splitk, stream) : launch_w160_as<128>(p, wp.splitk, stream);
-    }
-  }
-  if (use_ring64(p, amode, bmode, out_f32)) return launch_ring64(p, stream);
+      if (int rc = wp.bn == 160 ? launch_w160_as<160>(p, wp.splitk, stream) : launch_w160_as<128>(p, wp.splitk, stream)) return rc;
+      return split_sum_launch(p, wp.splitk, stream);
+    }
+  }
+  if (use_ring64(p, amode, bmode, out_f32)) return p.plan_only ? NK_OK : launch_ring64(p, stream);
   if ((!p.nbatch || p.nbatch <= NK_MAX_BATCH) && use_g2(p, amode, bmode, out_f32, 1) && (g2_mode() == 2 || !use_xl(p, amode, bmode, out_f32, 1))) {
+    if (p.plan_only) return NK_OK;
     if (p.accumulate == 2) p.accumulate = 0;
     if (amode == OP_KC && bmode == OP_KC) return out_f32 ? launch_g2<OP_KC, OP_KC, 1>(p, stream) : launch_g2<OP_KC, OP_KC, 0>(p, stream);
     if (amode == OP_KC && bmode == OP_MC) return out_f32 ? launch_g2<OP_KC, OP_MC, 1>(p, stream) : launch_g2<OP_KC, OP_MC, 0>(p, stream);
@@ -1681,6 +1673,7 @@
   if (!has_dbias && use_sk(p, out_f32)) {
     const long ntm_ = (p.M + BM - 1) / BM, ntn_ = (p.N + BN - 1) / BN, nk_ = (p.K + BK - 1) / BK;
     if (ntm_ * ntn_ * (p.nbatch ? p.nbatch : 1) * nk_ < (1l << 22)) {
+      if (p.plan_only) return NK_OK;
       if (p.accumulate == 2) p.accumulate = 0;
 #define NK_SK_CASE(A_, B_)                                                        \
       if (amode == A_ && bmode == B_) return out_f32 ? launch_sk<A_, B_, 1>(p, stream) : launch_sk<A_, B_, 0>(p, stream);
@@ -1694,23 +1687,20 @@
     }
   }
   int splitk = 1;
-  if (out_f32 && allow_splitk) splitk = pick_splitk(p.M * (p.nbatch ? p.nbatch : 1), p.N, p.K, 32);
   if (p.nbatch) NK_CHECK_ARG(p.nbatch <= NK_MAX_BATCH);
+  if (out_f32 && allow_splitk) splitk = split_cap(p, pick_splitk(p.M * (p.nbatch ? p.nbatch : 1), p.N, p.K, 32));
+  if (p.plan_only) { p.split_ws_bytes = split_scratch_bytes(p, splitk); return NK_OK; }
   set_split(p, splitk);
-  if (out_f32 && splitk > 1 && p.accumulate == 0) {
-    NK_CHECK_ARG(p.ldc == p.N);
-    if (int rc = zero_split_outputs(p, stream)) return rc;
-    p.accumulate = 1;
-  } else if (p.accumulate == 2) {
-    p.accumulate = splitk > 1 ? 1 : 0;
-  }
+  if (p.accumulate == 2) p.accumulate = 0;
+  if (int rc = split_prepare(p, splitk, stream)) return rc;
 
   if (use_xl(p, amode, bmode, out_f32, splitk))
     return amode == OP_KC ? launch_xl<OP_KC>(p, stream) : launch_xl<OP_KCG>(p, stream);
 
 #define NK_CASE(A_, B_)                                                          \
   if (amode == A_ && bmode == B_) {                                              \
-    return out_f32 ? launch<A_, B_, 1>(p, splitk, stream) : launch<A_, B_, 0>(p, splitk, stream); \
+    if (int rc = out_f32 ? launch<A_, B_, 1>(p, splitk, stream) : launch<A_, B_, 0>(p, splitk, stream)) return rc; \
+    return split_sum_launch(p, splitk, stream);                                  \
   }
   NK_CASE(OP_KC, OP_KC)
   NK_CASE(OP_KC, OP_MC)
diff --git a/neurosis_amd/csrc/gemm_w160.h b/neurosis_amd/csrc/gemm_w160.h
--- a/neurosis_amd/csrc/gemm_w160.h
+++ b/neurosis_amd/csrc/gemm_w160.h
@@ -291,24 +291,25 @@
   W160_STAMP(2); W160_STAMP_RT(5);
 
   const int mb = m0 + wr * 80, nb = n0 + wc * (BN_ / 2);
-  const int mode = gridDim.y > 1 ? 2 : (p.accumulate ? 1 : 0);
+  const int split = blockIdx.y;
+  const bool add = !split && p.accumulate;
   if (dbias != nullptr && bmask) {
+    float* const db = split ? nk_split_bias_slab(p, split, gridDim.y, blockIdx.z, gridDim.z) : dbias;
 #pragma unroll
     for (int i = 0; i < 5; ++i) {
       if ((bmask & (1u << i)) && lane < 16) {
         const int m = mb + i * 16 + lane;
         if (m < p.M) {
           const float v = accb[i][0] * p.alpha;
-          if (mode == 2) unsafeAtomicAdd(dbias + m, v);
-          else dbias[m] = mode == 1 ? dbias[m] + v : v;
+          db[m] = add ? db[m] + v : v;
         }
       }
     }
   }
-  float* const Cp = (float*)(p.nbatch ? p.Cb[blockIdx.z] : p.C);
-  if (mode == 2) {
+  float* const Cp = split ? nk_split_slab(p, split, gridDim.y, blockIdx.z) : (float*)(p.nbatch ? p.Cb[blockIdx.z] : p.C);
+  if (gridDim.y > 1) {
     W160_BAR();
-    constexpr int BW = BN_ / 2, LDW = BW + 4;
+    constexpr int BW = BN_ / 2, LDW = BW + 4, BW4 = BW / 4;
     static_assert(4 * 80 * LDW * 4 <= Cfg::SMEM, "the four waves' staging images fit the ring");
     float* img = (float*)smem + wave * (80 * LDW);
 #pragma unroll
@@ -319,9 +320,14 @@
         v *= p.alpha;
         *(float4_t*)(img + (i * 16 + (lane & 15)) * LDW + j * 16 + (lane >> 4) * 4) = v;
       }
-    for (int e = lane; e < 80 * BW; e += 64) {
-      const int m = e / BW, n = e - m * BW;
-      if (mb + m < p.M && nb + n < p.N) unsafeAtomicAdd(Cp + (long)(mb + m) * p.ldc + nb + n, img[m * LDW + n]);
+    for (int e = lane; e < 80 * BW4; e += 64) {
+      const int m = e / BW4, n = (e - m * BW4) * 4;
+      if (mb + m < p.M && nb + n < p.N) {
+        float4_t v = *(const float4_t*)(img + m * LDW + n);
+        float4_t* dst = (float4_t*)(Cp + (long)(mb + m) * p.N + nb + n);
+        if (add) v += *dst;
+        *dst = v;
+      }
     }
     return;
   }
@@ -365,6 +371,7 @@
     int sk = 1;
     if (const char* e = getenv("NK_GEMM_W160_SPLIT")) sk = atoi(e);
     if (sk < 1 || !allow_splitk || nk < 2 * sk) sk = 1;
+    sk = split_cap(p, sk);
     return {p.N % 160 == 0 || p.N % 128 != 0 ? 160 : 128, sk};
   }
   if (p.M % W160_BM) return {0, 0};
@@ -379,6 +386,7 @@
       if (sk > 1 && (!allow_splitk || nk / sk < 32)) break;
       const long wgs = tiles * sk, rounds = (wgs + 255) / 256;
       if ((double)wgs < 0.85 * (double)(rounds * 256)) continue;
+      if (split_scratch_bytes(p, sk) > NK_SPLIT_WS_CAP) continue;
       const double us = (double)rounds * (double)((nk + sk - 1) / sk) * 0.66 * bn / 160.0 + (sk > 1 ? sk * (double)p.M * p.N * nb * 4.0 / 0.6e6 : 0.0);
       if (us < best_us) { best_us = us; best = {bn, sk}; }
     }
diff --git a/neurosis_amd/csrc/nk_gemm.h b/neurosis_amd/csrc/nk_gemm.h
--- a/neurosis_amd/csrc/nk_gemm.h
+++ b/neurosis_amd/csrc/nk_gemm.h
@@ -36,6 +36,9 @@
   int ksplit_len;
   int group_m;
   int accumulate;
+  float* split_ws;
+  size_t split_ws_bytes;
+  int plan_only;
   int lean_src;
   int k_rotate;
   int nbatch;
diff --git a/neurosis_amd/csrc/ops_gemm.hip b/neurosis_amd/csrc/ops_gemm.hip
--- a/neurosis_amd/csrc/ops_gemm.hip
+++ b/neurosis_amd/csrc/ops_gemm.hip
@@ -108,8 +108,10 @@
   return dgrad_geglu(dy, w, u, du, M, N, I, lddy, ldw, ldu, lddu, 0, stream);
 }
 
+static float plan_bias;
+
 static int linear_wgrad(const void* dy, const void* x, float* dw, float* dbias, int M, int N, int K, long lddy, long ldx, long lddw,
-                        int accumulate, void* stream) {
+                        int accumulate, float* scratch, size_t scratch_bytes, int plan, size_t* need, void* stream) {
   NkGemmParams p = zero_params();
   p.A = (const bf16_t*)dy; p.lda = lddy;
   p.B = (const bf16_t*)x; p.ldb = ldx;
@@ -117,20 +119,28 @@
   p.C = dw; p.ldc = lddw;
   p.accumulate = accumulate;
   p.dbias = dbias;
-  return nk_gemm_dispatch(p, NK_OP_MC, NK_OP_MC, 1, lddw == K, (hipStream_t)stream);
+  p.split_ws = scratch; p.split_ws_bytes = plan ? 0 : scratch_bytes; p.plan_only = plan;
+  const int rc = nk_gemm_dispatch(p, NK_OP_MC, NK_OP_MC, 1, lddw == K, (hipStream_t)stream);
+  if (plan && need) *need = p.split_ws_bytes;
+  return rc;
 }
 extern "C" int nk_linear_wgrad(const void* dy, const void* x, float* dw, int M, int N, int K, long lddy,
                                long ldx, long lddw, int accumulate, void* stream) {
-  return linear_wgrad(dy, x, dw, nullptr, M, N, K, lddy, ldx, lddw, accumulate, stream);
+  return linear_wgrad(dy, x, dw, nullptr, M, N, K, lddy, ldx, lddw, accumulate, nullptr, 0, 0, nullptr, stream);
 }
 extern "C" int nk_linear_wgrad_bias(const void* dy, const void* x, float* dw, float* dbias, int M, int N, int K, long lddy,
                                     long ldx, long lddw, int accumulate, void* stream) {
   NK_CHECK_ARG(dbias != nullptr);
-  return linear_wgrad(dy, x, dw, dbias, M, N, K, lddy, ldx, lddw, accumulate, stream);
-}
-
-extern "C" int nk_linear_wgrad_batched(const void* const* dy, const void* const* x, float* const* dw, float* const* dbias, int count, int M,
-                                       int N, int K, long lddy, long ldx, long lddw, int accumulate, void* stream) {
+  return linear_wgrad(dy, x, dw, dbias, M, N, K, lddy, ldx, lddw, accumulate, nullptr, 0, 0, nullptr, stream);
+}
+extern "C" int nk_linear_wgrad_ws(const void* dy, const void* x, float* dw, float* dbias, int M, int N, int K, long lddy, long ldx, long lddw,
+                                  int accumulate, float* scratch, long scratch_bytes, void* stream) {
+  NK_CHECK_ARG(scratch_bytes >= 0 && (scratch != nullptr || scratch_bytes == 0));
+  return linear_wgrad(dy, x, dw, dbias, M, N, K, lddy, ldx, lddw, accumulate, scratch, (size_t)scratch_bytes, 0, nullptr, stream);
+}
+
+static int linear_wgrad_batched(const void* const* dy, const void* const* x, float* const* dw, float* const* dbias, int count, int M, int N, int K,
+                                long lddy, long ldx, long lddw, int accumulate, float* scratch, size_t scratch_bytes, void* stream) {
   NK_CHECK_ARG(dy && x && dw && count >= 1 && count <= NK_MAX_BATCH);
   NkGemmParams p = zero_params();
   p.lda = lddy; p.ldb = ldx;
@@ -145,7 +155,35 @@
     p.dbias_b[i] = dbias ? dbias[i] : nullptr;
   }
   p.A = p.Ab[0]; p.B = p.Bb[0]; p.C = p.Cb[0];
+  p.split_ws = scratch; p.split_ws_bytes = scratch_bytes;
   return nk_gemm_dispatch(p, NK_OP_MC, NK_OP_MC, 1, lddw == K, (hipStream_t)stream);
+}
+extern "C" int nk_linear_wgrad_batched(const void* const* dy, const void* const* x, float* const* dw, float* const* dbias, int count, int M,
+                                       int N, int K, long lddy, long ldx, long lddw, int accumulate, void* stream) {
+  return linear_wgrad_batched(dy, x, dw, dbias, count, M, N, K, lddy, ldx, lddw, accumulate, nullptr, 0, stream);
+}
+extern "C" int nk_linear_wgrad_batched_ws(const void* const* dy, const void* const* x, float* const* dw, float* const* dbias, int count, int M,
+                                          int N, int K, long lddy, long ldx, long lddw, int accumulate, float* scratch, long scratch_bytes,
+                                          void* stream) {
+  NK_CHECK_ARG(scratch_bytes >= 0 && (scratch != nullptr || scratch_bytes == 0));
+  return linear_wgrad_batched(dy, x, dw, dbias, count, M, N, K, lddy, ldx, lddw, accumulate, scratch, (size_t)scratch_bytes, stream);
+}
+extern "C" long nk_linear_wgrad_scratch_bytes(int M, int N, int K, long lddy, long ldx, long lddw, int has_bias, int count) {
+  if (count < 1 || count > NK_MAX_BATCH) return -1;
+  size_t need = 0;
+  if (count == 1) {
+    if (linear_wgrad(nullptr, nullptr, nullptr, has_bias ? &plan_bias : nullptr, M, N, K, lddy, ldx, lddw, 0, nullptr, 0, 1, &need, nullptr)) return -1;
+    return (long)need;
+  }
+  NkGemmParams p = zero_params();
+  p.lda = lddy; p.ldb = ldx;
+  p.M = N; p.N = K; p.K = M;
+  p.ldc = lddw;
+  p.nbatch = count;
+  for (int i = 0; i < count; ++i) p.dbias_b[i] = has_bias ? &plan_bias : nullptr;
+  p.plan_only = 1;
+  if (nk_gemm_dispatch(p, NK_OP_MC, NK_OP_MC, 1, lddw == K, nullptr)) return -1;
+  return (long)p.split_ws_bytes;
 }
 
 static int check_conv(const NkConvDesc* d) {
@@ -262,7 +300,8 @@
   return nk_gemm_dispatch(p, NK_OP_KCG, NK_OP_KC, 0, 0, (hipStream_t)stream);
 }
 
-static int conv_wgrad(const NkConvDesc* d, const void* dy, const void* x, float* dw, float* dbias, int accumulate, void* stream) {
+static int conv_wgrad(const NkConvDesc* d, const void* dy, const void* x, float* dw, float* dbias, int accumulate, float* scratch,
+                      size_t scratch_bytes, int plan, size_t* need, void* stream) {
   if (int e = check_conv(d)) return e;
   NkGemmParams p = zero_params();
   p.A = (const bf16_t*)dy; p.lda = d->Cout;
@@ -272,14 +311,27 @@
   p.accumulate = accumulate;
   p.dbias = dbias;
   p.halo_nb = (d->KH == 3 && d->KW == 3) ? d->N : 0;
-  return nk_gemm_dispatch(p, NK_OP_MC, NK_OP_MCG, 1, 1, (hipStream_t)stream);
+  p.split_ws = scratch; p.split_ws_bytes = plan ? 0 : scratch_bytes; p.plan_only = plan;
+  const int rc = nk_gemm_dispatch(p, NK_OP_MC, NK_OP_MCG, 1, 1, (hipStream_t)stream);
+  if (plan && need) *need = p.split_ws_bytes;
+  return rc;
 }
 extern "C" int nk_conv2d_wgrad(const NkConvDesc* d, const void* dy, const void* x, float* dw, int accumulate,
                                void* stream) {
-  return conv_wgrad(d, dy, x, dw, nullptr, accumulate, stream);
+  return conv_wgrad(d, dy, x, dw, nullptr, accumulate, nullptr, 0, 0, nullptr, stream);
 }
 extern "C" int nk_conv2d_wgrad_bias(const NkConvDesc* d, const void* dy, const void* x, float* dw, float* dbias, int accumulate,
                                     void* stream) {
   NK_CHECK_ARG(dbias != nullptr);
-  return conv_wgrad(d, dy, x, dw, dbias, accumulate, stream);
-}
+  return conv_wgrad(d, dy, x, dw, dbias, accumulate, nullptr, 0, 0, nullptr, stream);
+}
+extern "C" int nk_conv2d_wgrad_ws(const NkConvDesc* d, const void* dy, const void* x, float* dw, float* dbias, int accumulate, float* scratch,
+                                  long scratch_bytes, void* stream) {
+  NK_CHECK_ARG(scratch_bytes >= 0 && (scratch != nullptr || scratch_bytes == 0));
+  return conv_wgrad(d, dy, x, dw, dbias, accumulate, scratch, (size_t)scratch_bytes, 0, nullptr, stream);
+}
+extern "C" long nk_conv2d_wgrad_scratch_bytes(const NkConvDesc* d, int has_bias) {
+  size_t need = 0;
+  if (conv_wgrad(d, nullptr, nullptr, nullptr, has_bias ? &plan_bias : nullptr, 0, nullptr, 0, 1, &need, nullptr)) return -1;
+  return (long)need;
+}
diff --git a/neurosis_amd/csrc/split_sum.h b/neurosis_amd/csrc/split_sum.h
--- /dev/null
+++ b/neurosis_amd/csrc/split_sum.h
@@ -0,0 +1,103 @@
+#pragma once
+
+#define NK_SPLIT_WS_CAP ((size_t)128 << 20)
+
+struct NkSplitSum {
+  float* dst[NK_MAX_BATCH];
+  float* dbias[NK_MAX_BATCH];
+  const float* ws;
+  long MN;
+  int M;
+  int S, nz;
+};
+
+__global__ __launch_bounds__(256) void nk_split_sum_kernel(const NkSplitSum a) {
+  const int z = blockIdx.y, ns = a.S - 1;
+  const long i = (long)blockIdx.x * 256 + threadIdx.x, n4 = a.MN >> 2;
+  if (i < n4) {
+    float4_t* dst = (float4_t*)a.dst[z] + i;
+    const float4_t* src = (const float4_t*)(a.ws + (long)z * ns * a.MN) + i;
+    float4_t v = *dst;
+#pragma unroll 4
+    for (int s = 0; s < ns; ++s) v += src[(long)s * n4];
+    *dst = v;
+  } else if (i - n4 < a.M && a.dbias[z]) {
+    const long m = i - n4;
+    const float* src = a.ws + (long)a.nz * ns * a.MN + (long)z * ns * a.M + m;
+    float v = a.dbias[z][m];
+    for (int s = 0; s < ns; ++s) v += src[(long)s * a.M];
+    a.dbias[z][m] = v;
+  }
+}
+
+static bool split_has_bias(const NkGemmParams& p) {
+  bool b = p.dbias != nullptr;
+  for (int z = 0; z < p.nbatch && z < NK_MAX_BATCH; ++z) b = b || p.dbias_b[z] != nullptr;
+  return b;
+}
+static size_t split_scratch_bytes(const NkGemmParams& p, int S) {
+  if (S <= 1) return 0;
+  return (size_t)(S - 1) * (p.nbatch ? p.nbatch : 1) * ((size_t)p.M * p.N + (split_has_bias(p) ? p.M : 0)) * sizeof(float);
+}
+static int split_cap(const NkGemmParams& p, int S) {
+  while (S > 1 && split_scratch_bytes(p, S) > NK_SPLIT_WS_CAP) --S;
+  return S;
+}
+
+struct SplitBlock {
+  float* ptr = nullptr;
+  size_t bytes = 0;
+};
+static std::mutex split_mutex;
+static std::unordered_map<void*, SplitBlock> split_blocks;
+
+static int split_prepare(NkGemmParams& p, int S, hipStream_t stream) {
+  const size_t need = split_scratch_bytes(p, S);
+  if (!need) { p.split_ws = nullptr; p.split_ws_bytes = 0; return NK_OK; }
+  NK_CHECK_ARG(p.ldc == p.N && (p.N & 3) == 0 && need <= NK_SPLIT_WS_CAP);
+  if (p.split_ws) {
+    if (p.split_ws_bytes < need || ((uintptr_t)p.split_ws & 15)) {
+      nk_set_error(__FILE__, __LINE__, "split weight gradient: the scratch block passed is smaller than nk_*_wgrad_scratch_bytes reports, or not 16-byte aligned");
+      return NK_ERR_ARG;
+    }
+    return NK_OK;
+  }
+  std::lock_guard<std::mutex> lock(split_mutex);
+  SplitBlock& b = split_blocks[(void*)stream];
+  if (b.bytes < need) {
+    hipStreamCaptureStatus capturing = hipStreamCaptureStatusNone;
+    if (hipStreamIsCapturing(stream, &capturing) == hipSuccess && capturing != hipStreamCaptureStatusNone) {
+      nk_set_error(__FILE__, __LINE__, "split weight gradient needs a larger scratch block than this stream holds while the stream is capturing: run the launch once on this stream before capturing it, or pass a block to the *_ws entry point");
+      return NK_ERR_LAUNCH;
+    }
+    size_t want = need > 2 * b.bytes ? need : 2 * b.bytes;
+    if (want > NK_SPLIT_WS_CAP) want = NK_SPLIT_WS_CAP;
+    float* raw = nullptr;
+    if (hipMalloc((void**)&raw, want) != hipSuccess) {
+      nk_set_error(__FILE__, __LINE__, "hipMalloc of the split weight-gradient scratch failed");
+      return NK_ERR_LAUNCH;
+    }
+    b.ptr = raw;
+    b.bytes = want;
+  }
+  p.split_ws = b.ptr;
+  p.split_ws_bytes = b.bytes;
+  return NK_OK;
+}
+
+static int split_sum_launch(const NkGemmParams& p, int S, hipStream_t stream) {
+  if (S <= 1) return NK_OK;
+  NkSplitSum a = {};
+  a.nz = p.nbatch ? p.nbatch : 1;
+  for (int z = 0; z < a.nz; ++z) {
+    a.dst[z] = (float*)(p.nbatch ? p.Cb[z] : p.C);
+    a.dbias[z] = p.nbatch ? p.dbias_b[z] : p.dbias;
+  }
+  a.ws = p.split_ws;
+  a.MN = (long)p.M * p.N;
+  a.M = split_has_bias(p) ? p.M : 0;
+  a.S = S;
+  const long elems = (a.MN >> 2) + a.M;
+  hipLaunchKernelGGL(nk_split_sum_kernel, dim3((unsigned)((elems + 255) / 256), a.nz), dim3(256), 0, stream, a);
+  return nk_check_launch("nk_split_sum_kernel");
+}
diff --git a/neurosis_amd/lib.py b/neurosis_amd/lib.py
--- a/neurosis_amd/lib.py
+++ b/neurosis_amd/lib.py
@@ -46,6 +46,9 @@
     "nk_linear_wgrad_batched": [C.POINTER(vp), C.POINTER(vp), C.POINTER(vp), C.POINTER(vp), i32, i32, i32, i32, i64, i64, i64, i32, vp],
     "nk_linear_wgrad_bias": [vp, vp, vp, vp, i32, i32, i32, i64, i64, i64, i32, vp],
     "nk_conv2d_wgrad_bias": [cdp, vp, vp, vp, vp, i32, vp],
+    "nk_linear_wgrad_ws": [vp, vp, vp, vp, i32, i32, i32, i64, i64, i64, i32, vp, i64, vp],
+    "nk_linear_wgrad_batched_ws": [C.POINTER(vp), C.POINTER(vp), C.POINTER(vp), C.POINTER(vp), i32, i32, i32, i32, i64, i64, i64, i32, vp, i64, vp],
+    "nk_conv2d_wgrad_ws": [cdp, vp, vp, vp, vp, i32, vp, i64, vp],
     "nk_conv2d_fwd": [cdp, vp, vp, vp, vp, vp, vp, vp],
     "nk_conv2d_fwd_stats": [cdp, vp, vp, vp, vp, vp, vp, vp, i32, vp],
     "nk_conv_weight_flip": [vp, vp, i32, i32, i32, vp],
@@ -130,6 +133,8 @@
     "nk_layernorm_ws_floats": [i32, i32],
     "nk_layernorm_part_rows": [i32],
     "nk_colsum_ws_floats": [i64, i32],
+    "nk_linear_wgrad_scratch_bytes": [i32, i32, i32, i64, i64, i64, i32, i32],
+    "nk_conv2d_wgrad_scratch_bytes": [cdp, i32],
     "nk_batchnorm_ws_floats": [i64, i32],
     "nk_lpips_layer_ws_floats": [i32, i32],
     "nk_attention_bwd_ws_floats": [adp],
diff --git a/neurosis_amd/ops.py b/neurosis_amd/ops.py
--- a/neurosis_amd/ops.py
+++ b/neurosis_amd/ops.py
@@ -148,9 +148,11 @@
                         continue
                     n = len(chunk)
                     arr = C.c_void_p * n
-                    call("nk_linear_wgrad_batched", arr(*[c[0].data_ptr() for c in chunk]), arr(*[c[1].data_ptr() for c in chunk]),
+                    ws, nbytes = _split_ws(query("nk_linear_wgrad_scratch_bytes", M, N, K, lddy, ldx, lddw, int(any(c[3] is not None for c in chunk)), n),
+                                           chunk[0][0].device)
+                    call("nk_linear_wgrad_batched_ws", arr(*[c[0].data_ptr() for c in chunk]), arr(*[c[1].data_ptr() for c in chunk]),
                          arr(*[c[2].data_ptr() for c in chunk]), arr(*[None if c[3] is None else c[3].data_ptr() for c in chunk]), n, M, N, K,
-                         lddy, ldx, lddw, mode, _stream())
+                         lddy, ldx, lddw, mode, _p(ws), nbytes, _stream())
 
         on_wgrad_stream(run, *[t for it in items for t in it[:2]], owner=self.owner)
 
@@ -205,6 +207,14 @@
 
 def _ws(n_floats: int, device) -> Tensor:
     return torch.empty(n_floats, dtype=torch.float32, device=device)
+
+
+def _split_ws(nbytes: int, device):
+    if nbytes < 0:
+        raise ValueError(f"weight-gradient scratch query failed: {lib.load().nk_last_error().decode()}")
+    if nbytes == 0:
+        return None, 0
+    return torch.empty((nbytes + 3) // 4, dtype=torch.float32, device=device), nbytes
 
 
 def _p(t: Optional[Tensor]):
@@ -406,13 +416,11 @@
     K = x.shape[1]
     if x.shape[0] != M or dw.shape != (N, K) or dw.dtype != torch.float32 or dw.stride(1) != 1:
         raise ValueError(f"gemm_tn_f32: bad shapes {dy.shape} {x.shape} {dw.shape}")
-    if dbias is None:
-        call("nk_linear_wgrad", dy.data_ptr(), x.data_ptr(), dw.data_ptr(), M, N, K, dy.stride(0), x.stride(0), dw.stride(0), int(accumulate), _stream())
-        return
-    if dbias.shape != (N,) or dbias.dtype != torch.float32 or not dbias.is_contiguous():
+    if dbias is not None and (dbias.shape != (N,) or dbias.dtype != torch.float32 or not dbias.is_contiguous()):
         raise ValueError(f"gemm_tn_f32: dbias must be a dense fp32 [{N}] tensor")
-    call("nk_linear_wgrad_bias", dy.data_ptr(), x.data_ptr(), dw.data_ptr(), dbias.data_ptr(), M, N, K, dy.stride(0), x.stride(0), dw.stride(0),
-         int(accumulate), _stream())
+    ws, nbytes = _split_ws(query("nk_linear_wgrad_scratch_bytes", M, N, K, dy.stride(0), x.stride(0), dw.stride(0), int(dbias is not None), 1), dy.device)
+    call("nk_linear_wgrad_ws", dy.data_ptr(), x.data_ptr(), dw.data_ptr(), _p(dbias), M, N, K, dy.stride(0), x.stride(0), dw.stride(0),
+         int(accumulate), _p(ws), nbytes, _stream())
 
 
 def colsum(dy: Tensor, out: Tensor, accumulate: bool) -> None:
@@ -543,12 +551,12 @@
         acc = state_of(weight).grad_accumulate
 
         if weight.requires_grad:
-            if bias is not None:
-                on_wgrad_stream(lambda: call("nk_conv2d_wgrad_bias", C.byref(d), dy.data_ptr(), x.t.data_ptr(), g2d(weight).data_ptr(), grad_flat(bias).data_ptr(),
-                                             wgrad_mode(weight), _stream()), dy, x.t, owner=weight)
-            else:
-                on_wgrad_stream(lambda: call("nk_conv2d_wgrad", C.byref(d), dy.data_ptr(), x.t.data_ptr(), g2d(weight).data_ptr(), wgrad_mode(weight), _stream()),
-                                dy, x.t, owner=weight)
+            def wgrad():
+                ws, nbytes = _split_ws(query("nk_conv2d_wgrad_scratch_bytes", C.byref(d), int(bias is not None)), dy.device)
+                call("nk_conv2d_wgrad_ws", C.byref(d), dy.data_ptr(), x.t.data_ptr(), g2d(weight).data_ptr(),
+                     None if bias is None else grad_flat(bias).data_ptr(), wgrad_mode(weight), _p(ws), nbytes, _stream())
+
+            on_wgrad_stream(wgrad, dy, x.t, owner=weight)
         drow = None
         if rowvec is not None:
             drow32 = torch.empty(x.N, Cout, dtype=torch.float32, device=dy.device)
```
